# yuhuishi-convect/mojo-bm25

Hardware: AMD Instinct MI355X
Metric: queries/sec + achieved HBM GB/s, 10M-doc CSC index, batch=1024, k=100 (higher is better)
Workload: dtype f32; 1 GPU; c3: 10M docs / 200k vocab, batch=1024, k=100, 8 terms per query; segments=dense, n_docs=10000000, n_terms=200000, nnz=639994696, batch=1024, terms_per_query=8, k=100, tile_docs=2048, parallelism=doc-shard x1, term_lanes=8

## Files before the change

### mojo-bm25_amd/bm25mi/index.py

```python
from __future__ import annotations

import ctypes
from typing import Optional, Tuple

import numpy as np

from . import _capi
from ._capi import check, lib


def _ptr(a: Optional[np.ndarray]):
    return None if a is None else a.ctypes.data_as(ctypes.c_void_p)


def pack_mask(allow) -> np.ndarray:
    a = np.asarray(allow)
    if a.ndim == 1:
        a = a[None, :]
    if a.ndim != 2:
        raise ValueError("allow must be a bool [n_docs] or [M, n_docs] array")
    a = a.astype(bool)
    M, n = a.shape
    W = (n + 31) // 32
    bits = np.zeros((M, W * 32), np.uint8)
# ... 812 lines not shown
        if (d_values.dim() not in (1, 2) or d_values.shape[-1] != self.n_docs
                or not d_values.is_contiguous()):
            raise ValueError(f"d_values must be a contiguous [{self.n_docs}] or "
                             f"[F, {self.n_docs}] tensor (one entry per document)")
        F = 1 if d_values.dim() == 1 else d_values.shape[0]
        if (d_out.dim() != 2 or d_out.shape[1] != W or d_out.element_size() != 4
                or not d_out.is_contiguous()):
            raise ValueError(f"d_out must be a contiguous packed [M, {W}] tensor of 32-bit words")
        M = d_out.shape[0]
        if (d_fields.dim() != 2 or d_fields.shape[0] != M or d_fields.dtype != torch.int32
                or not d_fields.is_contiguous()):
            raise ValueError(f"d_fields must be a contiguous int32 [{M}, C] tensor (one row per "
                             "mask)")
        C = d_fields.shape[1]
        for name, t in (("d_lo", d_lo), ("d_hi", d_hi)):
            if (t.dtype != d_values.dtype or tuple(t.shape) != (M, C) or not t.is_contiguous()):
                raise ValueError(f"{name} must be a contiguous {d_values.dtype} [{M}, {C}] tensor "
                                 "(the values' dtype, the shape of d_fields)")
        Mb = 0
        if d_base is not None:
            if (d_base.dim() != 2 or d_base.shape[1] != W or d_base.element_size() != 4
                    or not d_base.is_contiguous()):
                raise ValueError(f"d_base must be a contiguous packed [1 or M, {W}] tensor of "
                                 "32-bit words")
            Mb = d_base.shape[0]
            if Mb not in (1, M):
                raise ValueError(f"d_base has {Mb} rows, expected 1 or {M}")
        s = getattr(stream, "cuda_stream", stream) or 0
        p = lambda t, n: ctypes.c_void_p(t.data_ptr()) if n else None
        check(lib.bm25_range_masks_device(
            self._h, p(d_values, F and self.n_docs), kinds[d_values.dtype], F, p(d_fields, M * C),
            p(d_lo, M * C), p(d_hi, M * C), C, M, p(d_base, Mb and W), Mb, p(d_out, M and W),
            ctypes.c_void_p(s)))

    def search_boolean(self, queries: np.ndarray, k: int, must=None, any=None, must_not=None,
                       base=None, *, min_match=None, total_hits: bool = False, facets=None,
                       ranges=None):
        q = np.ascontiguousarray(queries, dtype=np.int32)
        if q.ndim != 2:
            raise ValueError("queries must be a 2-D [Q, T] int32 array")
        Q, T = q.shape
        mu, an, mn, _, b, Mb = self._clauses_arg(must, any, must_not, base, rows=Q)
        mm = None if min_match is None else min_match_rows(an, min_match, "query")
        if facets is not None:
            if not isinstance(facets, (tuple, list)) or len(facets) != 2:
                raise ValueError("facets must be a pair (groups, n_groups)")
            fg, G = _facet_groups(facets[0], facets[1], self.n_docs)
        if ranges is not None:
            rv, kind, rf, rlo, rhi = _range_args(*_ranges_arg(ranges), self.n_docs, rows=Q,
                                                 what="query")
        k = int(k)
        docs = np.zeros((Q, max(k, 0)), np.int32)
        scores = np.zeros((Q, max(k, 0)), np.float32)
        if ranges is not None:
            totals = np.zeros(Q, np.int64) if total_hits else None
            counts = np.zeros((Q, G), np.int64) if facets is not None else None
            give = bool(counts is not None and G and fg.size)
            ranged = bool(rv.size and rf.size)
            check(lib.bm25_search_boolean_ranges(
                self._h, _ptr(q), Q, T, k, _ptr(mu), mu.shape[1], _ptr(an), an.shape[1], _ptr(mn),
                mn.shape[1], _ptr(mm), _ptr(b) if Mb else None, Mb, _ptr(fg) if give else None,
                G if give else 0, _ptr(rv) if ranged else None, kind, rv.shape[0] if ranged else 0,
                _ptr(rf) if ranged else None, _ptr(rlo) if ranged else None,
                _ptr(rhi) if ranged else None, rf.shape[1] if ranged else 0, _ptr(docs),
                _ptr(scores), _ptr(totals), _ptr(counts) if give else None))
            out = (docs, scores)
            if total_hits:
                out += (totals,)
            if facets is not None:
                out += (counts,)
            return out
        if facets is not None:
            totals = np.zeros(Q, np.int64) if total_hits else None
            counts = np.zeros((Q, G), np.int64)
            give = bool(G and fg.size)
            check(lib.bm25_search_boolean_facets(
                self._h, _ptr(q), Q, T, k, _ptr(mu), mu.shape[1], _ptr(an), an.shape[1], _ptr(mn),
                mn.shape[1], _ptr(mm), _ptr(b) if Mb else None, Mb, _ptr(fg) if give else None,
                G if give else 0, _ptr(docs), _ptr(scores), _ptr(totals),
                _ptr(counts) if give else None))
            return (docs, scores, totals, counts) if total_hits else (docs, scores, counts)
        if mm is None and not total_hits:
            check(lib.bm25_search_boolean(self._h, _ptr(q), Q, T, k, _ptr(mu), mu.shape[1],
                                          _ptr(an), an.shape[1], _ptr(mn), mn.shape[1],
                                          _ptr(b) if Mb else None, Mb, _ptr(docs), _ptr(scores)))
            return docs, scores
        totals = np.zeros(Q, np.int64) if total_hits else None
        check(lib.bm25_search_boolean_min_match(
            self._h, _ptr(q), Q, T, k, _ptr(mu), mu.shape[1], _ptr(an), an.shape[1], _ptr(mn),
            mn.shape[1], _ptr(mm), _ptr(b) if Mb else None, Mb, _ptr(docs), _ptr(scores),
            _ptr(totals)))
        return (docs, scores, totals) if total_hits else (docs, scores)

    def set_values_f64(self, data64) -> None:
        d = np.ascontiguousarray(data64, dtype=np.float64)
        if d.size < self.nnz:
            raise ValueError("data64 shorter than nnz")
        check(lib.bm25_index_set_values_f64(self._h, _ptr(d)))

    def scores_dense_f64(self, query) -> np.ndarray:
        q = np.ascontiguousarray(np.asarray(query).ravel(), dtype=np.int32)
        out = np.zeros(self.n_docs, np.float64)
        check(lib.bm25_scores_dense_f64(self._h, _ptr(q), q.size, _ptr(out)))
        return out

    def topn_f64(self, query, n: int) -> Tuple[np.ndarray, np.ndarray]:
        q = np.ascontiguousarray(np.asarray(query).ravel(), dtype=np.int32)
        docs = np.zeros(max(int(n), 0), np.int32)
        scores = np.zeros(max(int(n), 0), np.float64)
        check(lib.bm25_topn_f64(self._h, _ptr(q), q.size, int(n), _ptr(docs), _ptr(scores)))
        return docs, scores

    def profile_enable(self, on: bool = True) -> None:
        check(lib.bm25_profile_enable(self._h, int(on)))

    def profile_read(self) -> dict:
        sm = ctypes.c_double()
        sl = ctypes.c_int64()
        tm = ctypes.c_double()
        ns = ctypes.c_int64()
        rs = ctypes.c_int64()
        check(lib.bm25_profile_read(self._h, ctypes.byref(sm), ctypes.byref(sl), ctypes.byref(tm),
                                    ctypes.byref(ns), ctypes.byref(rs)))
        return {"score_ms": sm.value, "score_launches": sl.value, "total_ms": tm.value,
                "searches": ns.value, "rescored_tiles_last": rs.value}

    def set_option(self, name: str, value: int) -> None:
        check(lib.bm25_index_set_option(self._h, name.encode(), int(value)))
        self.__dict__.pop("_bm25_width_ok", None)
        for f in self.__dict__.get("_bm25_forks", []):
            f.set_option(name, value)

    def get_option(self, name: str) -> int:
        v = ctypes.c_int64()
        check(lib.bm25_index_get_option(self._h, name.encode(), ctypes.byref(v)))
        return v.value

    KERNELS = {1: "flat_sample", 2: "flat_rest", 4: "flat_all", 8: "wave_sample",
               16: "wave_rest", 32: "wave_all", 64: "large_k", 128: "bound_keys",
               256: "bound_off", 512: "count_skips", 1024: "rest_split",
               2048: "bound_pool", 4096: "filtered", 8192: "weighted",
               16384: "after"}

    def last_dispatch(self) -> dict:
        km = ctypes.c_uint32()
        tl = ctypes.c_int32()
        bt = (ctypes.c_int32 * 3)()
        sp_ = ctypes.c_int32()
        check(lib.bm25_search_dispatch(self._h, ctypes.byref(km), ctypes.byref(tl), bt,
                                       ctypes.byref(sp_)))
        return {"kernels": {n for b, n in self.KERNELS.items() if km.value & b},
                "tile_skip": bool(km.value & 32768),
                "seg_skip": bool(km.value & 65536),
                "term_lanes": tl.value,
                "band_tiles": {"all": bt[0], "sample": bt[1], "rest": bt[2]},
                "sample_p": sp_.value}

    def search_stats(self) -> dict:
        v = (ctypes.c_int64 * 8)()
        check(lib.bm25_search_counters(self._h, v, 8))
        return {"rescored_tiles": v[0], "fallback_queries": v[1],
                "bound_skipped_tiles": v[2], "bound_skipped_postings": v[3],
                "block_merge_queries": v[4], "large_dense_queries": v[5],
                "bound_dropped_segments": v[6], "bound_dropped_postings": v[7]}


def merge_topk_device(device: int, d_docs, d_scores, W: int, Q: int, k: int, d_out_docs,
                      d_out_scores, stream=None) -> None:
    s = getattr(stream, "cuda_stream", stream) or 0
    check(lib.bm25_merge_topk_device(int(device), ctypes.c_void_p(d_docs.data_ptr()),
                                     ctypes.c_void_p(d_scores.data_ptr()), int(W), int(Q), int(k),
                                     ctypes.c_void_p(d_out_docs.data_ptr()),
                                     ctypes.c_void_p(d_out_scores.data_ptr()),
                                     ctypes.c_void_p(s)))


def merge_sorted_device(device: int, d_docs, d_scores, W: int, Q: int, k: int, rank_stride: int,
                        d_out_docs, d_out_scores, stream=None) -> None:
    s = getattr(stream, "cuda_stream", stream) or 0
    check(lib.bm25_merge_sorted_device(int(device), ctypes.c_void_p(d_docs.data_ptr()),
                                       ctypes.c_void_p(d_scores.data_ptr()), int(W), int(Q),
                                       int(k), int(rank_stride),
                                       ctypes.c_void_p(d_out_docs.data_ptr()),
                                       ctypes.c_void_p(d_out_scores.data_ptr()),
                                       ctypes.c_void_p(s)))


class ShardedIndex:

    def __init__(self, indptr, indices, data, n_docs: int, devices):
        devices = [int(d) for d in devices]
        if not devices:
            raise ValueError("need at least one device")
        indptr = np.asarray(indptr)
        ip_i64 = indptr.dtype == np.int64 or indptr[-1] > np.iinfo(np.int32).max
        ip = np.ascontiguousarray(indptr, dtype=np.int64 if ip_i64 else np.int32)
        ix = np.ascontiguousarray(indices, dtype=np.int32)
        dt = np.ascontiguousarray(data, dtype=np.float32)
        devs = np.asarray(devices, np.int32)
        self.n_docs = int(n_docs)
        self.n_terms = int(ip.size - 1)
        self._h = None
        h = ctypes.c_void_p()
        check(lib.bm25_sharded_create(len(devices), _ptr(devs), self.n_docs, self.n_terms,
                                      int(ip[-1]), _ptr(ip), int(ip_i64), _ptr(ix), _ptr(dt),
                                      ctypes.byref(h)))
        self._h = h

    def shards(self):
        n = ctypes.c_int64()
        check(lib.bm25_sharded_info(self._h, ctypes.byref(n), None, None))
        lo = np.zeros(n.value, np.int64)
        hi = np.zeros(n.value, np.int64)
        check(lib.bm25_sharded_info(self._h, ctypes.byref(n), _ptr(lo), _ptr(hi)))
        return list(zip(lo.tolist(), hi.tolist()))

    def search(self, queries: np.ndarray, k: int) -> Tuple[np.ndarray, np.ndarray]:
        q = np.ascontiguousarray(queries, dtype=np.int32)
        if q.ndim != 2:
            raise ValueError("queries must be a 2-D [Q, T] int32 array")
        Q, T = q.shape
        k = int(k)
        docs = np.zeros((Q, max(k, 0)), np.int32)
        scores = np.zeros((Q, max(k, 0)), np.float32)
        check(lib.bm25_sharded_search(self._h, _ptr(q), Q, T, k, _ptr(docs), _ptr(scores)))
        return docs, scores

    def close(self) -> None:
        if self._h is not None:
            lib.bm25_sharded_destroy(self._h)
            self._h = None

    def __del__(self):
        try:
            self.close()
        except Exception:
            pass


def device_count() -> int:
    return _capi.device_count()
```

### mojo-bm25_amd/csrc/bm25mi_capi.cpp

```cpp
#include "../../include/bm25mi.h"

#include <hip/hip_runtime.h>

#include <algorithm>
#include <cmath>
#include <cstdarg>
#include <cstdio>
#include <cstring>
#include <memory>
#include <mutex>
#include <string>
#include <vector>

#include "bm25mi_host.h"
#include "bm25mi_internal.h"

using namespace bm25mi;

namespace {
thread_local std::string g_err;
}

int bm25mi::fail(int code, const char* fmt, ...) {
  char buf[1024];
// ... 33 lines not shown
  std::vector<void*> p;
  ~IndexArrays() {
    hipSetDevice(device);
    for (void* x : p) hipFree(x);
  }
};

}

struct bm25_index {
  DevIndex ix;
  std::shared_ptr<IndexArrays> arrays;
  hipStream_t stream = nullptr;
  Workspace ws;
  int32_t* d_q = nullptr;
  int32_t* d_docs = nullptr;
  float* d_scores = nullptr;
  int64_t cap_q_elems = 0, cap_out_elems = 0;
  std::mutex mu;
  int prof = 0;
  std::vector<EventPair> ev_pool;
  size_t ev_used = 0;
  double score_ms = 0.0, total_ms = 0.0;
  int64_t score_launches = 0, searches = 0, rescored = 0;
  int64_t device_bytes = 0;
  EventPair* split_ev = nullptr;
  hipEvent_t ws_done = nullptr;
  hipEvent_t ev_split[2] = {nullptr, nullptr};
  hipStream_t ws_stream = nullptr;
  int32_t* d_maxtok = nullptr;
  bool sampled = false;
  int32_t* report_host = nullptr;
  int32_t* report_dev = nullptr;
  int32_t seq = 0, last_bound_seq = -1, seen_seq = -1, weak_until = 0, backoff = 64;
  int64_t last_bound_q = 0;
  int64_t large_fallback = 0;
  LargeArena arena;
  int64_t filtered_dense = 0;
};

static const OptDesc* find_opt(const char* name) {
  for (const OptDesc& d : kOpts)
    if (!strcmp(d.name, name)) return &d;
  for (const OptDesc& d : kOptsMore)
    if (!strcmp(d.name, name)) return &d;
  fail(BM25_EINVAL, "unknown option '%s'", name);
  return nullptr;
}

int bm25mi::set_opt(SearchOpts& o, const char* name, int64_t v) {
  if (!name) return fail(BM25_EINVAL, "NULL option name");
  const OptDesc* d = find_opt(name);
  if (!d) return BM25_EINVAL;
  if (v < d->lo || v > d->hi || (d->kind == kOptPow2 && (v & (v - 1)) != 0)) {
    if (d->msg) return fail(BM25_EINVAL, "%s", d->msg);
    if (d->kind == kOptBool) return fail(BM25_EINVAL, "%s must be 0 or 1", name);
    return fail(BM25_EINVAL, d->kind == kOptPow2 ? "%s must be a power of two in %d..%d"
                                                  : "%s must be in %d..%d", name, d->lo, d->hi);
  }
  o.*d->field = (int)v;
  return BM25_OK;
}

int bm25mi::get_opt(const SearchOpts& o, const char* name, int64_t* v) {
  if (!name || !v) return fail(BM25_EINVAL, "NULL argument");
  const OptDesc* d = find_opt(name);
  if (!d) return BM25_EINVAL;
  *v = o.*d->field;
  return BM25_OK;
}

namespace {

void free_ws(Workspace& ws) {
  hipFree(ws.cand);
  hipFree(ws.theta);
  hipFree(ws.list);
  hipFree(ws.list_cnt);
  hipFree(ws.fb);
  hipFree(ws.cand2);
  hipFree(ws.flag_tiles);
  hipFree(ws.nflag);
  hipFree(ws.queue);
  hipFree(ws.counters);
  hipFree(ws.slow);
  hipFree(ws.wctr);
  hipFree(ws.seg);
  hipFree(ws.qw);
  hipFree(ws.sub);
  hipFree(ws.sub_ipb);
  hipFree(ws.sub_done);
  hipFree(ws.tskip);
  ws = Workspace{};
}

int32_t list_cap_for(const SearchOpts& o, int64_t k) {
  if (o.list_cap > 0) return o.list_cap;
  return (int32_t)std::min<int64_t>(65536, std::max<int64_t>(2048, 64 * k));
}

SearchOpts env_opts() {
  SearchOpts o;
  auto read = [&o](const OptDesc& d) {
    int v = env_int(d.env, o.*d.field);
    if (d.kind == kOptBool) v = v != 0;
    if (d.env_clamp >= 1) v = std::max(d.lo, v);
    if (d.env_clamp >= 2) v = std::min(d.hi, v);
    o.*d.field = v;
  };
  for (const OptDesc& d : kOpts) read(d);
  for (const OptDesc& d : kOptsMore) read(d);
  return o;
}

int ensure_ws(bm25_index* h, int64_t Q, int64_t T, int k, hipStream_t st) {
  Workspace& ws = h->ws;
  const int64_t need_seg = seg_entries(h->ix, std::max(Q, ws.cap_q), T);
  if (Q <= ws.cap_q && k <= ws.cap_k) {
    if (need_seg <= ws.cap_seg) return BM25_OK;
    hipFree(ws.seg);
    ws.seg = nullptr;
    ws.cap_seg = 0;
    HIP_TRY(hipMalloc(&ws.seg, sizeof(uint64_t) * need_seg), "hipMalloc(seg)");
    ws.cap_seg = need_seg;
    return BM25_OK;
  }
  const int64_t q = std::max(Q, ws.cap_q);
  const int64_t kk = std::max<int64_t>(k, ws.cap_k);
  free_ws(ws);
  const int64_t nt = h->ix.ntiles;
  const int64_t mf = maxflag_for((int)kk, nt);
  const int32_t C = list_cap_for(h->ix.opt, kk);
  HIP_TRY(hipMalloc(&ws.cand, sizeof(uint64_t) * q * nt * kTileM), "hipMalloc(cand)");
  HIP_TRY(hipMalloc(&ws.theta, sizeof(uint64_t) * q), "hipMalloc(theta)");
  HIP_TRY(hipMalloc(&ws.list, sizeof(uint64_t) * q * C), "hipMalloc(list)");
  HIP_TRY(hipMalloc(&ws.list_cnt, sizeof(int32_t) * q), "hipMalloc(list_cnt)");
  HIP_TRY(hipMalloc(&ws.fb, sizeof(int32_t) * q), "hipMalloc(fb)");
  HIP_TRY(hipMalloc(&ws.cand2, sizeof(uint64_t) * q * mf * kk), "hipMalloc(cand2)");
  HIP_TRY(hipMalloc(&ws.flag_tiles, sizeof(int32_t) * q * mf), "hipMalloc(flag_tiles)");
  HIP_TRY(hipMalloc(&ws.nflag, sizeof(int32_t) * q), "hipMalloc(nflag)");
  HIP_TRY(hipMalloc(&ws.queue, sizeof(int32_t) * q * mf), "hipMalloc(queue)");
  HIP_TRY(hipMalloc(&ws.counters, sizeof(int32_t) * kCounters), "hipMalloc(counters)");
  HIP_TRY(hipMemsetAsync(ws.counters, 0, sizeof(int32_t) * kCounters, st), "hipMemsetAsync(counters)");
  HIP_TRY(hipMalloc(&ws.slow, sizeof(int32_t) * q), "hipMalloc(slow)");
  HIP_TRY(hipMalloc(&ws.wctr, sizeof(int32_t) * kWctrRegions * kWctrInts), "hipMalloc(wctr)");
  HIP_TRY(hipMemsetAsync(ws.wctr, 0, sizeof(int32_t) * kWctrRegions * kWctrInts, st),
          "hipMemsetAsync(wctr)");
  HIP_TRY(hipMalloc(&ws.qw, sizeof(uint32_t) * q), "hipMalloc(qw)");
  HIP_TRY(hipMalloc(&ws.sub, sizeof(uint32_t) * q * 8), "hipMalloc(sub)");
  HIP_TRY(hipMalloc(&ws.sub_ipb, sizeof(int32_t)), "hipMalloc(sub_ipb)");
  HIP_TRY(hipMalloc(&ws.sub_done, sizeof(int32_t)), "hipMalloc(sub_done)");
  HIP_TRY(hipMemsetAsync(ws.sub_done, 0, sizeof(int32_t), st), "hipMemsetAsync(sub_done)");
  if (h->ix.bmax)
    HIP_TRY(hipMalloc(&ws.tskip, (size_t)std::max<int64_t>(q * tskip_stride(nt), 4)), "hipMalloc(tskip)");
  ws.cap_seg = need_seg;
  if (ws.cap_seg > 0) HIP_TRY(hipMalloc(&ws.seg, sizeof(uint64_t) * ws.cap_seg), "hipMalloc(seg)");
  ws.list_cap = C;
  ws.cap_q = q;
  ws.cap_k = kk;
  return BM25_OK;
}

int ensure_io(bm25_index* h, int64_t q_elems, int64_t out_elems) {
  if (q_elems > h->cap_q_elems) {
    hipFree(h->d_q);
    h->d_q = nullptr;
    h->cap_q_elems = 0;
    HIP_TRY(hipMalloc(&h->d_q, sizeof(int32_t) * std::max<int64_t>(q_elems, 1)), "hipMalloc(queries)");
    h->cap_q_elems = q_elems;
  }
  if (out_elems > h->cap_out_elems) {
    hipFree(h->d_docs);
    hipFree(h->d_scores);
    h->d_docs = nullptr;
    h->d_scores = nullptr;
    h->cap_out_elems = 0;
    HIP_TRY(hipMalloc(&h->d_docs, sizeof(int32_t) * std::max<int64_t>(out_elems, 1)), "hipMalloc(docs)");
    HIP_TRY(hipMalloc(&h->d_scores, sizeof(float) * std::max<int64_t>(out_elems, 1)), "hipMalloc(scores)");
    h->cap_out_elems = out_elems;
  }
  return BM25_OK;
}

void harvest_events(bm25_index* h) {
  if (h->ev_used == 0) return;
  for (size_t i = 0; i < h->ev_used; ++i) {
    float ms1 = 0.f, ms2 = 0.f;
    const bool tot = h->ev_pool[i].with_c;
    hipEventSynchronize(tot ? h->ev_pool[i].c : h->ev_pool[i].b);
    hipEventElapsedTime(&ms1, h->ev_pool[i].a, h->ev_pool[i].b);
    if (tot) hipEventElapsedTime(&ms2, h->ev_pool[i].a, h->ev_pool[i].c);
    h->score_ms += ms1;
    h->total_ms += tot ? ms2 : ms1;
  }
  h->ev_used = 0;
}

EventPair* next_events(bm25_index* h) {
  if (!h->prof) return nullptr;
  if (h->ev_used == h->ev_pool.size()) {
    if (h->ev_pool.size() < 512) {
      EventPair p;
      hipEventCreate(&p.a);
      hipEventCreate(&p.b);
      hipEventCreate(&p.c);
      h->ev_pool.push_back(p);
    } else {
      harvest_events(h);
    }
  }
  EventPair* e = &h->ev_pool[h->ev_used++];
  e->with_c = h->prof >= 2;
  return e;
}

hipError_t record_end(bm25_index* h, EventPair* ev, hipStream_t st) {
  return (ev && ev->with_c) ? hipEventRecord(ev->c, st) : hipSuccess;
}

hipError_t order_ws(bm25_index* h, hipStream_t st) {
  if (h->ws_stream == nullptr || st == h->ws_stream) {
    h->ws_stream = st;
    return hipSuccess;
  }
  if (!h->ws_done) {
    const hipError_t e = hipEventCreateWithFlags(&h->ws_done, hipEventDisableTiming);
    if (e != hipSuccess) return e;
  }
  hipError_t e = hipEventRecord(h->ws_done, h->ws_stream);
  if (e == hipSuccess) e = hipStreamWaitEvent(st, h->ws_done, 0);
  h->ws_stream = st;
  return e;
}

void ws_wait_host(bm25_index* h) {
  if (h->ws_stream) hipStreamSynchronize(h->ws_stream);
}

void choose_theta_source(bm25_index* h) {
  ++h->seq;
  if (h->report_host && h->last_bound_seq >= 0 && h->seen_seq != h->last_bound_seq) {
    const int32_t r = __atomic_load_n(h->report_host + 1, __ATOMIC_ACQUIRE);
    if (r == h->last_bound_seq) {
      h->seen_seq = r;
      const int64_t nf = __atomic_load_n(h->report_host, __ATOMIC_RELAXED);
      if (nf * 16 > h->last_bound_q) {
        h->weak_until = h->seq + h->backoff;
        h->backoff = std::min(2 * h->backoff, 4096);
      } else {
        h->backoff = 64;
      }
    }
  }
  h->ix.bound_weak = h->seq < h->weak_until;
}

void arm_report(bm25_index* h, int P, int64_t Q) {
  h->ws.report = h->report_dev;
  h->ws.seq = h->seq;
  if (h->ix.bound_weak) h->ix.disp.kernels |= kKBoundOff;
  if (P == 0) {
    h->last_bound_seq = h->seq;
    h->last_bound_q = Q;
  }
}

void alloc_report(bm25_index* h) {
  if (hipHostMalloc((void**)&h->report_host, 2 * sizeof(int32_t), hipHostMallocMapped) !=
      hipSuccess) {
    (void)hipGetLastError();
    h->report_host = nullptr;
    return;
  }
  h->report_host[0] = 0;
  h->report_host[1] = -1;
  if (hipHostGetDevicePointer((void**)&h->report_dev, h->report_host, 0) != hipSuccess) {
    (void)hipGetLastError();
    hipHostFree(h->report_host);
    h->report_host = h->report_dev = nullptr;
  }
}

int run_search(bm25_index* h, const int32_t* d_queries, int64_t Q, int64_t T, int k,
               int32_t* d_docs, float* d_scores, hipStream_t st, bool shard = false) {
  if (Q == 0 || k == 0) return BM25_OK;
  if (k > kMaxK) {
    const bool lists = h->ix.opt.large_lists && k <= kLargeListMaxK && k <= h->ix.n_docs &&
                       large_list_supported(h->ix, T, Q) && large_geom(h->ix, k).P > 0;
    if (lists) {
      const int rc = ensure_ws(h, Q, T, 1, st);
      if (rc) return rc;
    }
    if (h->arena.need > h->arena.bytes) {
      if (h->ws_stream) HIP_TRY(hipStreamSynchronize(h->ws_stream), "hipStreamSynchronize");
      hipFree(h->arena.base);
      h->arena.base = nullptr;
      h->arena.bytes = 0;
      HIP_TRY(hipMalloc((void**)&h->arena.base, h->arena.need), "hipMalloc(large-k scratch)");
      h->arena.bytes = h->arena.need;
    }
    h->arena.used = 0;
    h->ws.arena = &h->arena;
    HIP_TRY(order_ws(h, st), "workspace order");
    if (h->ws.counters)
      HIP_TRY(hipMemsetAsync(h->ws.counters, 0, sizeof(int32_t) * kCounters, st), "hipMemsetAsync");
    h->ix.disp = Dispatch{};
    h->ix.disp.sample_p = 1;
// ... 55 lines not shown
    hipFree(h->arena.base);
    h->arena.base = nullptr;
    h->arena.bytes = 0;
    HIP_TRY(hipMalloc((void**)&h->arena.base, h->arena.need), "hipMalloc(filtered scratch)");
    h->arena.bytes = h->arena.need;
  }
  h->arena.used = 0;
  h->ws.arena = &h->arena;
  HIP_TRY(order_ws(h, st), "workspace order");
  h->large_fallback = 0;
  h->ix.disp = Dispatch{};
  h->ix.disp.sample_p = 1;
  h->ws.report = nullptr;
  EventPair* ev = next_events(h);
  if (ev) HIP_TRY(hipEventRecord(ev->a, st), "hipEventRecord");
  int64_t nd = 0;
  if (after) h->ix.disp.kernels |= kKAfter;
  HIP_TRY(launch_search_filtered(h->ix, d_queries, Q, T, k, d_masks, M, d_query_mask, h->ws,
                                 d_docs, d_scores, &nd, st, d_weights, d_after_scores,
                                 d_after_docs),
          after ? "cursor search" : d_weights ? "weighted search" : "filtered search");
  h->filtered_dense = nd;
  if (ev) {
    HIP_TRY(hipEventRecord(ev->b, st), "hipEventRecord");
    HIP_TRY(record_end(h, ev, st), "hipEventRecord");
  }
  if (h->prof) {
    h->score_launches += 1;
    h->searches += 1;
  }
  return BM25_OK;
}

void read_counters(bm25_index* h, int32_t (&cnt)[kCounters]) {
  if (!h->ws.counters) return;
  ws_wait_host(h);
  hipMemcpyAsync(cnt, h->ws.counters, sizeof cnt, hipMemcpyDeviceToHost, h->stream);
  hipStreamSynchronize(h->stream);
}

int check_k(const bm25_index* h, int64_t k, bool shard = false) {
  if (k < 0) return fail(BM25_EINVAL, "negative dimensions are not allowed (top_k=%lld)", (long long)k);
  if (!shard && k > h->ix.n_docs)
    return fail(BM25_EINVAL, "kth(=%lld) out of bounds (%lld)", (long long)(h->ix.n_docs - k),
                (long long)h->ix.n_docs);
  return BM25_OK;
}

int64_t max_token(int64_t mx, const int32_t* ids, int64_t n) {
  for (int64_t i = 0; i < n; ++i) mx = std::max<int64_t>(mx, ids[i]);
  return mx;
}

int check_token_ids(int64_t n_terms, int64_t mx0, const int32_t* ids, int64_t n) {
  const int64_t mx = max_token(mx0, ids, n);
  if (mx >= n_terms)
    return fail(BM25_EINVAL,
                "The maximum token ID in the query (%lld) is higher than the number of tokens in "
                "the index.",
                (long long)mx);
  return BM25_OK;
}

int check_weights(const int32_t* ids, const float* w, int64_t Q, int64_t T) {
  for (int64_t i = 0; i < Q * T; ++i)
    if (ids[i] >= 0 && !std::isfinite(w[i]))
      return fail(BM25_EINVAL, "weights[%lld][%lld] = %g is not finite", (long long)(i / T),
                  (long long)(i % T), (double)w[i]);
  return BM25_OK;
}

struct Enter {
  std::lock_guard<std::mutex> lk;
  int rc;
  explicit Enter(bm25_index* h) : lk(h->mu), rc(BM25_OK) {
    const hipError_t e = hipSetDevice(h->ix.device);
    if (e != hipSuccess) rc = hip_fail(e, "hipSetDevice");
  }
};

struct OwnStream {
  hipStream_t s = nullptr;
  ~OwnStream() {
    if (s) hipStreamDestroy(s);
  }
};

}

extern "C" {

int bm25_abi_version(void) { return BM25MI_ABI_VERSION; }

const char* bm25_last_error(void) { return g_err.c_str(); }

int bm25_device_count(void) {
  int n = 0;
  if (hipGetDeviceCount(&n) != hipSuccess) return 0;
  return n;
}

static int build_index(bm25_index* h, const std::vector<int64_t>& ip, const int32_t* indices,
                       const float* data);

int bm25_index_create(int device, int64_t n_docs, int64_t n_terms, int64_t nnz,
                      const void* indptr, int indptr_is_i64, const int32_t* indices,
                      const float* data, int64_t doc_offset, bm25_index** out) {
  if (!out) return fail(BM25_EINVAL, "out is NULL");
  *out = nullptr;
  if (n_docs < 0 || n_terms < 0 || nnz < 0)
    return fail(BM25_EINVAL, "negative size (n_docs=%lld n_terms=%lld nnz=%lld)",
                (long long)n_docs, (long long)n_terms, (long long)nnz);
  if (n_docs > INT32_MAX) return fail(BM25_EINVAL, "n_docs=%lld exceeds int32 doc ids", (long long)n_docs);
  if (doc_offset < 0 || doc_offset + n_docs > (int64_t)INT32_MAX + 1)
    return fail(BM25_EINVAL, "doc_offset=%lld out of int32 range", (long long)doc_offset);
  if (!indptr || (nnz > 0 && (!indices || !data)))
    return fail(BM25_EINVAL, "NULL CSC array");
  std::vector<int64_t> ip(n_terms + 1);
  for (int64_t t = 0; t <= n_terms; ++t)
    ip[t] = indptr_is_i64 ? ((const int64_t*)indptr)[t] : (int64_t)((const int32_t*)indptr)[t];
  if (ip[0] != 0 || ip[n_terms] != nnz)
    return fail(BM25_EINVAL, "indptr must start at 0 and end at nnz (got %lld..%lld, nnz=%lld)",
                (long long)ip[0], (long long)ip[n_terms], (long long)nnz);
  for (int64_t t = 0; t < n_terms; ++t) {
    if (ip[t + 1] < ip[t]) return fail(BM25_EINVAL, "indptr decreases at column %lld", (long long)t);
    if (ip[t + 1] - ip[t] > n_docs)
      return fail(BM25_EINVAL, "column %lld has more entries than n_docs", (long long)t);
  }
  const int shift = build_tile_shift();
  const int64_t ntiles = (n_docs + (1LL << shift) - 1) >> shift;
  if (ntiles > 65536) return fail(BM25_EINVAL, "n_docs=%lld needs %lld tiles (> 65536)", (long long)n_docs, (long long)ntiles);

  int ndev = 0;
  if (hipGetDeviceCount(&ndev) != hipSuccess || ndev == 0)
    return fail(BM25_EHIP, "no HIP device available");
  if (device < 0 || device >= ndev) return fail(BM25_EINVAL, "device %d out of range (%d visible)", device, ndev);
  HIP_TRY(hipSetDevice(device), "hipSetDevice");

  bm25_index* h = new bm25_index();
  DevIndex& ix = h->ix;
  ix.opt = env_opts();
  ix.device = device;
  ix.n_docs = n_docs;
  ix.n_terms = n_terms;
  ix.nnz = nnz;
  ix.doc_offset = doc_offset;
  ix.tile_shift = shift;
  ix.ntiles = ntiles;
  const int rc = build_index(h, ip, indices, data);
  if (rc == BM25_OK) {
    h->arrays = std::make_shared<IndexArrays>();
    h->arrays->device = device;
    h->arrays->p = {ix.indptr, ix.rel, ix.tl_ptr, ix.tl_tile, ix.tl_start, ix.ldoc, ix.val, ix.bmax,
                    ix.bpool, ix.tmask};
    *out = h;
  } else {
    bm25_index_destroy(h);
  }
  return rc;
}

static int build_index(bm25_index* h, const std::vector<int64_t>& ip, const int32_t* indices,
                       const float* data) {
  DevIndex& ix = h->ix;
  const int64_t n_terms = ix.n_terms, nnz = ix.nnz, ntiles = ix.ntiles;
  HIP_TRY(hipStreamCreateWithFlags(&h->stream, hipStreamNonBlocking), "hipStreamCreate");
  std::vector<int64_t> cnt;
  HostCall c(h->stream);
  auto own = [&c](auto** p, int64_t bytes, const char* what) {
    if (c.ok()) c.run(hipMalloc(p, (size_t)bytes), what);
  };
  alloc_report(h);
  const int64_t rel_elems = n_terms * (ntiles + 1);
  {
    const char* m = getenv("BM25_SEGMENTS");
    size_t free_b = 0, total_b = 0;
    if (hipMemGetInfo(&free_b, &total_b) != hipSuccess) total_b = 0;
    const int64_t rel_bytes = rel_elems * 4;
    if (m && !strcmp(m, "sparse")) ix.sparse = true;
    else if (m && !strcmp(m, "dense")) ix.sparse = false;
    else ix.sparse = rel_bytes > 2 * 6 * std::max<int64_t>(nnz, 1) &&
                     rel_bytes > (int64_t)(total_b / 8);
  }
  own(&ix.indptr, sizeof(int64_t) * (n_terms + 1), "hipMalloc(indptr)");
  if (!ix.sparse) own(&ix.rel, sizeof(uint32_t) * std::max<int64_t>(rel_elems, 1), "hipMalloc(rel)");
  own(&ix.ldoc, sizeof(uint16_t) * (nnz + kPostingPad), "hipMalloc(ldoc)");
  own(&ix.val, sizeof(float) * (nnz + kPostingPad), "hipMalloc(val)");
  if (c.ok()) c.run(hipMemsetAsync(ix.ldoc + nnz, 0, sizeof(uint16_t) * kPostingPad, h->stream), "hipMemset");
  if (c.ok()) c.run(hipMemsetAsync(ix.val + nnz, 0, sizeof(float) * kPostingPad, h->stream), "hipMemset");
  int32_t* d_indices = c.alloc<int32_t>(nnz, "hipMalloc(indices)");
  int32_t* d_err = c.alloc<int32_t>(1, "hipMalloc(err)");
  h->device_bytes = (int64_t)(sizeof(int64_t) * (n_terms + 1) +
                              (ix.sparse ? 0 : sizeof(uint32_t) * rel_elems) +
                              (sizeof(uint16_t) + sizeof(float)) * nnz);
  if (c.ok()) c.run(hipMemsetAsync(d_err, 0, sizeof(int32_t), h->stream), "hipMemset");
  c.upload_to(ix.indptr, ip.data(), n_terms + 1, "H2D indptr");
  c.upload_to(d_indices, indices, nnz, "H2D indices");
  c.upload_to(ix.val, data, nnz, "H2D data");
  if (!ix.sparse) {
    if (c.ok()) c.run(launch_build_tables(ix, d_indices, d_err, h->stream), "build_tables launch");
  } else {
    int64_t* d_cnt = c.alloc<int64_t>(n_terms, "hipMalloc(cnt)");
    cnt.assign(n_terms + 1, 0);
    if (c.ok()) c.run(launch_count_tiles(ix, d_indices, d_cnt, d_err, h->stream), "count_tiles");
    c.download(cnt.data() + 1, d_cnt, n_terms, "count_tiles");
    if (c.ok()) c.run(hipStreamSynchronize(h->stream), "count_tiles");
    for (int64_t t = 0; t < n_terms; ++t) cnt[t + 1] += cnt[t];
    ix.n_pairs = cnt[n_terms];
    own(&ix.tl_ptr, sizeof(int64_t) * (n_terms + 1), "hipMalloc(tl_ptr)");
    own(&ix.tl_tile, sizeof(uint16_t) * std::max<int64_t>(ix.n_pairs, 1), "hipMalloc(tl_tile)");
    own(&ix.tl_start, sizeof(uint32_t) * std::max<int64_t>(ix.n_pairs, 1), "hipMalloc(tl_start)");
    c.upload_to(ix.tl_ptr, cnt.data(), n_terms + 1, "H2D tl_ptr");
    if (c.ok()) c.run(launch_fill_tiles(ix, d_indices, h->stream), "fill_tiles launch");
    if (c.ok()) c.run(hipStreamSynchronize(h->stream), "fill_tiles");
    h->device_bytes += (int64_t)(sizeof(int64_t) * (n_terms + 1) +
                                 (sizeof(uint16_t) + sizeof(uint32_t)) * ix.n_pairs);
  }
  ix.nonneg = true;
  for (int64_t p = 0; p < nnz && ix.nonneg; ++p)
    ix.nonneg = data[p] == 0.0f || data[p] >= 1.17549435e-38f;
  if (c.ok() && !ix.sparse && ix.nonneg && n_terms > 0 && ntiles > 0) {
    if (hipMalloc(&ix.bmax, sizeof(uint16_t) * n_terms * bmax_stride(ntiles)) == hipSuccess) {
      c.run(launch_build_bmax(ix, h->stream), "build_bmax launch");
      h->device_bytes += (int64_t)(sizeof(uint16_t) * n_terms * bmax_stride(ntiles));
      const int64_t ps = bmax_stride((ntiles + kPool - 1) / kPool);
      if (c.ok() && hipMalloc(&ix.bpool, sizeof(uint16_t) * n_terms * ps) == hipSuccess) {
        ix.pstride = ps;
        c.run(launch_pool_bounds(ix.bmax, n_terms, bmax_stride(ntiles), ix.bpool, ps, h->stream),
              "pool_bounds launch");
        h->device_bytes += (int64_t)(sizeof(uint16_t) * n_terms * ps);
      } else {
        (void)hipGetLastError();
        ix.bpool = nullptr;
      }
      if (c.ok() && ix.opt.tile_mask &&
          hipMalloc(&ix.tmask, sizeof(uint32_t) * n_terms * bmax_stride(ntiles)) == hipSuccess) {
        c.run(launch_build_tmask(ix, h->stream), "build_tmask launch");
        h->device_bytes += (int64_t)(sizeof(uint32_t) * n_terms * bmax_stride(ntiles));
      } else {
        (void)hipGetLastError();
        ix.tmask = nullptr;
      }
    } else {
      (void)hipGetLastError();
      ix.bmax = nullptr;
    }
  }
  int32_t herr = 0;
  c.download(&herr, d_err, 1, "D2H err");
  const int rc = c.finish("build sync");
  if (rc) return rc;
  if (herr)
    return fail(BM25_EINVAL,
                "indices must be sorted, unique and in [0, n_docs) within every column "
                "(canonical CSC)");
  return BM25_OK;
}

int bm25_index_destroy(bm25_index* h) {
  if (!h) return BM25_OK;
  hipSetDevice(h->ix.device);
  if (h->stream) hipStreamSynchronize(h->stream);
  if (h->ws_stream) hipDeviceSynchronize();
  for (auto& p : h->ev_pool) {
    hipEventDestroy(p.a);
    hipEventDestroy(p.b);
    hipEventDestroy(p.c);
  }
  if (h->ws_done) hipEventDestroy(h->ws_done);
  for (hipEvent_t e : h->ev_split)
    if (e) hipEventDestroy(e);
  free_ws(h->ws);
  hipFree(h->arena.base);
  hipFree(h->d_q);
  hipFree(h->d_docs);
  hipFree(h->d_scores);
  hipFree(h->d_maxtok);
  if (h->report_host) hipHostFree(h->report_host);
  if (h->arrays) {
    h->arrays.reset();
  } else {
    for (void* x : {(void*)h->ix.indptr, (void*)h->ix.rel, (void*)h->ix.tl_ptr,
                    (void*)h->ix.tl_tile, (void*)h->ix.tl_start, (void*)h->ix.ldoc,
                    (void*)h->ix.val, (void*)h->ix.bmax, (void*)h->ix.bpool,
                    (void*)h->ix.tmask})
      hipFree(x);
  }
  hipFree(h->ix.wbpool);
  if (h->stream) hipStreamDestroy(h->stream);
  delete h;
  return BM25_OK;
}

static int pool_world(bm25_index* h);

int bm25_index_fork(bm25_index* base, bm25_index** out) {
  if (!out) return fail(BM25_EINVAL, "out is NULL");
  *out = nullptr;
  if (!base || !base->arrays) return fail(BM25_EINVAL, "NULL or unbuilt index");
  std::lock_guard<std::mutex> lk(base->mu);
  HIP_TRY(hipSetDevice(base->ix.device), "hipSetDevice");
  bm25_index* h = new bm25_index();
  h->ix = base->ix;
  h->ix.disp = Dispatch{};
  h->ix.wbpool = nullptr;
  h->arrays = base->arrays;
  h->device_bytes = base->device_bytes;
  const hipError_t e = hipStreamCreateWithFlags(&h->stream, hipStreamNonBlocking);
  if (e != hipSuccess) {
    bm25_index_destroy(h);
    return hip_fail(e, "hipStreamCreate");
  }
  alloc_report(h);
  if (h->ix.wbmax) {
    const int rc = pool_world(h);
    if (rc) {
      bm25_index_destroy(h);
      return rc;
    }
  }
  *out = h;
  return BM25_OK;
}

int bm25_index_info(const bm25_index* h, int64_t* n_docs, int64_t* n_terms, int64_t* nnz,
                    int32_t* tile_docs, int64_t* n_tiles, int64_t* device_bytes) {
  if (!h) return fail(BM25_EINVAL, "NULL index");
  if (n_docs) *n_docs = h->ix.n_docs;
  if (n_terms) *n_terms = h->ix.n_terms;
  if (nnz) *nnz = h->ix.nnz;
  if (tile_docs) *tile_docs = 1 << h->ix.tile_shift;
  if (n_tiles) *n_tiles = h->ix.ntiles;
  if (device_bytes) *device_bytes = h->device_bytes;
  return BM25_OK;
}

int bm25_index_segments(const bm25_index* h, int32_t* sparse, int64_t* n_pairs) {
  if (!h) return fail(BM25_EINVAL, "NULL index");
  if (sparse) *sparse = h->ix.sparse ? 1 : 0;
  if (n_pairs) *n_pairs = h->ix.n_pairs;
  return BM25_OK;
}

int bm25_index_bounds(const bm25_index* h, int32_t* has_bounds, int64_t* bytes) {
  if (!h) return fail(BM25_EINVAL, "NULL index");
  const bool on = h->ix.bmax != nullptr;
  if (has_bounds) *has_bounds = on ? 1 : 0;
  if (bytes) *bytes = on ? (int64_t)sizeof(uint16_t) * h->ix.n_terms * bmax_stride(h->ix.ntiles) : 0;
  return BM25_OK;
}

int bm25_search(bm25_index* h, const int32_t* queries, int64_t Q, int64_t T, int32_t k,
                int32_t* out_docs, float* out_scores) {
  if (!h) return fail(BM25_EINVAL, "NULL index");
  if (Q < 0 || T < 0) return fail(BM25_EINVAL, "negative query shape");
  int rc = check_k(h, k);
  if (rc) return rc;
  if (Q == 0 || k == 0) return BM25_OK;
  if (T > 0 && !queries) return fail(BM25_EINVAL, "NULL queries");
  if (!out_docs || !out_scores) return fail(BM25_EINVAL, "NULL output");
  rc = check_token_ids(h->ix.n_terms, 0, queries, Q * T);
  if (rc) return rc;
  Enter in(h);
  if (in.rc) return in.rc;
  rc = ensure_io(h, Q * T, Q * (int64_t)k);
  if (rc) return rc;
  HostCall c(h->stream);
  c.upload_to(h->d_q, queries, Q * T, "H2D queries");
  if (c.ok()) c.hold(run_search(h, h->d_q, Q, T, k, h->d_docs, h->d_scores, h->stream));
  c.download(out_docs, h->d_docs, Q * k, "D2H docs");
  c.download(out_scores, h->d_scores, Q * k, "D2H scores");
  return c.finish("search sync");
}

int bm25_search_device(bm25_index* h, const int32_t* d_queries, int64_t Q, int64_t T, int32_t k,
                       int32_t* d_docs, float* d_scores, void* stream) {
  if (!h) return fail(BM25_EINVAL, "NULL index");
  if (Q < 0 || T < 0) return fail(BM25_EINVAL, "negative query shape");
  int rc = check_k(h, k);
  if (rc) return rc;
  if (Q == 0 || k == 0) return BM25_OK;
  Enter in(h);
  if (in.rc) return in.rc;
  return run_search(h, d_queries, Q, T, k, d_docs, d_scores, (hipStream_t)stream);
}

int bm25_search_filtered(bm25_index* h, const int32_t* queries, int64_t Q, int64_t T, int32_t k,
                         const uint32_t* masks, int64_t M, const int32_t* query_mask,
                         int32_t* out_docs, float* out_scores) {
  if (!h) return fail(BM25_EINVAL, "NULL index");
  if (Q < 0 || T < 0 || M < 0) return fail(BM25_EINVAL, "negative query or mask shape");
  int rc = check_k(h, k);
  if (rc) return rc;
  if (Q == 0 || k == 0) return BM25_OK;
  if (T > 0 && !queries) return fail(BM25_EINVAL, "NULL queries");
  if (M > 0 && !masks) return fail(BM25_EINVAL, "NULL masks");
  if (M == 0 && !query_mask)
    return fail(BM25_EINVAL, "no masks: query_mask must name -1 (no filter) for every query");
  if (!out_docs || !out_scores) return fail(BM25_EINVAL, "NULL output");
  rc = check_token_ids(h->ix.n_terms, 0, queries, Q * T);
  if (rc) return rc;
  if (query_mask)
    for (int64_t i = 0; i < Q; ++i)
      if (query_mask[i] < -1 || query_mask[i] >= M)
        return fail(BM25_EINVAL, "query_mask[%lld] = %d is outside [-1, %lld)", (long long)i,
                    query_mask[i], (long long)M);
  Enter in(h);
  if (in.rc) return in.rc;
  rc = ensure_io(h, Q * T, Q * (int64_t)k);
  if (rc) return rc;
  const int64_t W = (h->ix.n_docs + 31) >> 5;
  HostCall c(h->stream);
  uint32_t* d_masks = M > 0 ? c.alloc<uint32_t>(M * W) : nullptr;
  int32_t* d_qm = query_mask ? c.alloc<int32_t>(Q) : nullptr;
  c.upload_to(d_masks, masks, M * W);
  if (query_mask) c.upload_to(d_qm, query_mask, Q);
  c.upload_to(h->d_q, queries, Q * T);
  if (!c.ok()) return c.finish("filtered search staging");
  c.hold(run_filtered(h, h->d_q, Q, T, k, d_masks, M, d_qm, h->d_docs, h->d_scores, h->stream));
  c.download(out_docs, h->d_docs, Q * k);
  c.download(out_scores, h->d_scores, Q * k);
  return c.finish("filtered search");
}

int bm25_search_filtered_device(bm25_index* h, const int32_t* d_queries, int64_t Q, int64_t T,
                                int32_t k, const uint32_t* d_masks, int64_t M,
                                const int32_t* d_query_mask, int32_t* d_docs, float* d_scores,
                                void* stream) {
  if (!h) return fail(BM25_EINVAL, "NULL index");
  if (Q < 0 || T < 0 || M < 0) return fail(BM25_EINVAL, "negative query or mask shape");
  int rc = check_k(h, k);
  if (rc) return rc;
  if (Q == 0 || k == 0) return BM25_OK;
  Enter in(h);
  if (in.rc) return in.rc;
  return run_filtered(h, d_queries, Q, T, k, d_masks, M, d_query_mask, d_docs, d_scores,
                      (hipStream_t)stream);
}
// ... 951 lines not shown
  c.upload_to(d_qq, queries, Q * T);
  c.upload_to(d_ww, weights, Q * T);
  c.upload_to(d_dd, docs, Q * C);
  if (c.ok()) c.run(launch_score_docs(h->ix, d_qq, Q, T, d_dd, C, d_out, h->stream, d_ww));
  c.download(out_scores, d_out, Q * C);
  return c.finish("score_docs_weighted");
}

int bm25_score_docs_weighted_device(bm25_index* h, const int32_t* d_queries,
                                    const float* d_weights, int64_t Q, int64_t T,
                                    const int32_t* d_docs, int64_t C, float* d_scores,
                                    void* stream) {
  if (!h) return fail(BM25_EINVAL, "NULL index");
  if (Q < 0 || T < 0 || C < 0) return fail(BM25_EINVAL, "negative query or candidate shape");
  if (Q == 0 || C == 0) return BM25_OK;
  if (T > 0 && (!d_queries || !d_weights)) return fail(BM25_EINVAL, "NULL queries or weights");
  if (!d_docs || !d_scores) return fail(BM25_EINVAL, "NULL docs or output");
  Enter in(h);
  if (in.rc) return in.rc;
  HIP_TRY(launch_score_docs(h->ix, d_queries, Q, T, d_docs, C, d_scores, (hipStream_t)stream,
                            T > 0 ? d_weights : nullptr),
          "score_docs_weighted launch");
  return BM25_OK;
}

int bm25_index_set_values_f64(bm25_index* h, const double* data64) {
  if (!h || (h->ix.nnz > 0 && !data64)) return fail(BM25_EINVAL, "NULL argument");
  if (!h->arrays) return fail(BM25_EINVAL, "unbuilt index");
  Enter in(h);
  if (in.rc) return in.rc;
  if (!h->ix.val64) {
    HIP_TRY(hipMalloc(&h->ix.val64, sizeof(double) * std::max<int64_t>(h->ix.nnz, 1)),
            "hipMalloc(val64)");
    h->arrays->p.push_back(h->ix.val64);
  }
  HostCall c(h->stream);
  c.upload_to(h->ix.val64, data64, h->ix.nnz, "H2D val64");
  return c.finish("val64 sync");
}

static double* dense_f64_query(bm25_index* h, HostCall& c, const int32_t* query, int64_t T) {
  if (T < 0) c.hold(fail(BM25_EINVAL, "negative query length"));
  else if (T > 0 && !query) c.hold(fail(BM25_EINVAL, "NULL query"));
  else if (!h->ix.val64)
    c.hold(fail(BM25_EINVAL, "no float64 values: bm25_index_set_values_f64 first"));
  else c.hold(check_token_ids(h->ix.n_terms, 0, query, T));
  int32_t* d_q = c.alloc<int32_t>(T, "hipMalloc(query)");
  double* d_out = c.alloc<double>(h->ix.n_docs, "hipMalloc(dense)");
  c.upload_to(d_q, query, T, "H2D query");
  if (c.ok())
    c.run(launch_dense_f64(h->ix, h->ix.val64, d_q, T, d_out, h->stream), "dense f64 launch");
  return d_out;
}

int bm25_scores_dense_f64(bm25_index* h, const int32_t* query, int64_t T, double* out_scores) {
  if (!h || !out_scores) return fail(BM25_EINVAL, "NULL argument");
  Enter in(h);
  if (in.rc) return in.rc;
  HostCall c(h->stream);
  const double* d_out = dense_f64_query(h, c, query, T);
  c.download(out_scores, d_out, h->ix.n_docs);
  return c.finish("scores_dense_f64");
}

int bm25_topn_f64(bm25_index* h, const int32_t* query, int64_t T, int64_t n, int32_t* out_docs,
                  double* out_scores) {
  if (!h) return fail(BM25_EINVAL, "NULL index");
  if (n < 0 || n > h->ix.n_docs)
    return fail(BM25_EINVAL, "n=%lld must be in 0..n_docs (%lld)", (long long)n,
                (long long)h->ix.n_docs);
  if (n > 0 && (!out_docs || !out_scores)) return fail(BM25_EINVAL, "NULL output");
  if (n == 0) return BM25_OK;
  Enter in(h);
  if (in.rc) return in.rc;
  HostCall c(h->stream);
  const double* d_out = dense_f64_query(h, c, query, T);
  void* scratch = c.alloc<char>((int64_t)topn_f64_scratch_bytes(h->ix.n_docs));
  int32_t* d_docs = c.alloc<int32_t>(n);
  double* d_sc = c.alloc<double>(n);
  if (c.ok()) c.run(launch_topn_f64(d_out, h->ix.n_docs, n, scratch, d_docs, d_sc, h->stream));
  c.download(out_docs, d_docs, n);
  c.download(out_scores, d_sc, n);
  return c.finish("topn_f64");
}

int bm25_merge_topk_device(int device, const int32_t* d_docs, const float* d_scores, int64_t W,
                           int64_t Q, int32_t k, int32_t* d_out_docs, float* d_out_scores,
                           void* stream) {
  if (W < 1 || Q < 0 || k < 0) return fail(BM25_EINVAL, "bad merge shape W=%lld Q=%lld k=%d", (long long)W, (long long)Q, k);
  HIP_TRY(hipSetDevice(device), "hipSetDevice");
  HIP_TRY(launch_merge_lists(d_docs, d_scores, W, Q, k, Q * (int64_t)k, false, d_out_docs, d_out_scores, (hipStream_t)stream), "merge_lists launch");
  return BM25_OK;
}

int bm25_merge_sorted_device(int device, const int32_t* d_docs, const float* d_scores, int64_t W,
                             int64_t Q, int32_t k, int64_t rank_stride, int32_t* d_out_docs,
                             float* d_out_scores, void* stream) {
  if (W < 1 || Q < 0 || k < 0 || rank_stride < Q * (int64_t)k)
    return fail(BM25_EINVAL, "bad merge shape W=%lld Q=%lld k=%d stride=%lld", (long long)W,
                (long long)Q, k, (long long)rank_stride);
  HIP_TRY(hipSetDevice(device), "hipSetDevice");
  HIP_TRY(launch_merge_lists(d_docs, d_scores, W, Q, k, rank_stride, true, d_out_docs,
                             d_out_scores, (hipStream_t)stream),
          "merge_sorted launch");
  return BM25_OK;
}

int bm25_profile_enable(bm25_index* h, int on) {
  if (!h) return fail(BM25_EINVAL, "NULL index");
  std::lock_guard<std::mutex> lk(h->mu);
  hipSetDevice(h->ix.device);
  harvest_events(h);
  h->prof = on < 0 ? 0 : (on > 2 ? 2 : on);
  h->score_ms = h->total_ms = 0.0;
  h->score_launches = h->searches = h->rescored = 0;
  return BM25_OK;
}

int bm25_profile_read(bm25_index* h, double* score_ms_total, int64_t* score_launches,
                      double* total_ms, int64_t* searches, int64_t* rescored_tiles) {
  if (!h) return fail(BM25_EINVAL, "NULL index");
  std::lock_guard<std::mutex> lk(h->mu);
  hipSetDevice(h->ix.device);
  harvest_events(h);
  int32_t cnt[kCounters] = {};
  read_counters(h, cnt);
  if (score_ms_total) *score_ms_total = h->score_ms;
  if (score_launches) *score_launches = h->score_launches;
  if (total_ms) *total_ms = h->total_ms;
  if (searches) *searches = h->searches;
  if (rescored_tiles) *rescored_tiles = cnt[3];
  return BM25_OK;
}

int bm25_search_stats(bm25_index* h, int64_t* rescored_tiles, int64_t* fallback_queries) {
  return bm25_search_stats_ex(h, rescored_tiles, fallback_queries, nullptr);
}

int bm25_search_stats_ex(bm25_index* h, int64_t* rescored_tiles, int64_t* fallback_queries,
                         int64_t* bound_skipped) {
  if (!h) return fail(BM25_EINVAL, "NULL index");
  Enter in(h);
  if (in.rc) return in.rc;
  int32_t cnt[kCounters] = {};
  read_counters(h, cnt);
  if (rescored_tiles) *rescored_tiles = cnt[3];
  if (fallback_queries) *fallback_queries = cnt[2];
  if (bound_skipped) *bound_skipped = (h->ix.disp.kernels & kKCountSkips) ? cnt[5] : -1;
  return BM25_OK;
}

int bm25_search_counters(bm25_index* h, int64_t* out, int32_t n) {
  if (!h || !out) return fail(BM25_EINVAL, "NULL argument");
  if (n < 1 || n > 8) return fail(BM25_EINVAL, "n=%d must be in 1..8", n);
  Enter in(h);
  if (in.rc) return in.rc;
  int32_t cnt[kCounters] = {};
  read_counters(h, cnt);
  uint64_t post = 0;
  std::memcpy(&post, cnt + 6, sizeof post);
  const bool counted = (h->ix.disp.kernels & kKCountSkips) != 0;
  uint64_t dpost = 0;
  std::memcpy(&dpost, cnt + 10, sizeof dpost);
  const int64_t v[8] = {cnt[3], cnt[2], counted ? cnt[5] : -1, counted ? (int64_t)post : -1,
                        cnt[4], h->large_fallback, counted ? cnt[8] : -1,
                        counted ? (int64_t)dpost : -1};
  for (int i = 0; i < n; ++i) out[i] = v[i];
  return BM25_OK;
}

int bm25_index_set_option(bm25_index* h, const char* name, int64_t value) {
  if (!h) return fail(BM25_EINVAL, "NULL index");
  std::lock_guard<std::mutex> lk(h->mu);
  const int old_cap = h->ix.opt.list_cap;
  const int rc = set_opt(h->ix.opt, name, value);
  if (rc) return rc;
  if (h->ix.opt.list_cap != old_cap && h->ws.cap_q > 0) {
    hipSetDevice(h->ix.device);
    ws_wait_host(h);
    free_ws(h->ws);
  }
  return BM25_OK;
}

int bm25_index_get_option(const bm25_index* h, const char* name, int64_t* value) {
  if (!h) return fail(BM25_EINVAL, "NULL index");
  bm25_index* m = const_cast<bm25_index*>(h);
  std::lock_guard<std::mutex> lk(m->mu);
  return get_opt(h->ix.opt, name, value);
}

int bm25_search_dispatch(bm25_index* h, uint32_t* kernels, int32_t* term_lanes,
                         int32_t* band_tiles, int32_t* sample_p) {
  if (!h) return fail(BM25_EINVAL, "NULL index");
  std::lock_guard<std::mutex> lk(h->mu);
  const Dispatch& d = h->ix.disp;
  if (kernels) *kernels = d.kernels;
  if (term_lanes) *term_lanes = d.term_lanes;
  if (band_tiles)
    for (int i = 0; i < 3; ++i) band_tiles[i] = d.band_tiles[i];
  if (sample_p) *sample_p = d.sample_p;
  return BM25_OK;
}

}

struct bm25_sharded {
  std::vector<bm25_index*> shards;
  std::vector<int64_t> lo, hi;
  std::vector<hipEvent_t> sampled;
  std::vector<hipEvent_t> keyed;
  std::vector<hipEvent_t> done;
  std::vector<uint64_t*> keys;
  std::vector<uint64_t*> all_keys;
  int64_t cap_keys = 0;
  int64_t n_docs = 0, n_terms = 0, shard_docs_max = 0;
  int32_t* g_docs = nullptr;
  float* g_scores = nullptr;
  int32_t* m_docs = nullptr;
  float* m_scores = nullptr;
  int64_t cap_g = 0, cap_m = 0;
  std::mutex mu;
};

namespace {

int sharded_free(bm25_sharded* s) {
  if (!s) return BM25_OK;
  if (!s->shards.empty() && s->shards[0]) {
    hipSetDevice(s->shards[0]->ix.device);
    hipFree(s->g_docs);
    hipFree(s->g_scores);
    hipFree(s->m_docs);
    hipFree(s->m_scores);
  }
  for (size_t i = 0; i < s->shards.size(); ++i) {
    if (!s->shards[i]) continue;
    hipSetDevice(s->shards[i]->ix.device);
    hipStreamSynchronize(s->shards[i]->stream);
    for (auto* v : {&s->sampled, &s->keyed, &s->done})
      if (i < v->size() && (*v)[i]) hipEventDestroy((*v)[i]);
    if (i < s->keys.size()) hipFree(s->keys[i]);
    if (i < s->all_keys.size()) hipFree(s->all_keys[i]);
    bm25_index_destroy(s->shards[i]);
  }
  delete s;
  return BM25_OK;
}

struct DrainShards {
  bm25_sharded* s;
  ~DrainShards() {
    for (size_t r = 0; s && r < s->shards.size(); ++r) {
      hipSetDevice(s->shards[r]->ix.device);
      hipStreamSynchronize(s->shards[r]->stream);
    }
  }
};

}

extern "C" {

int bm25_sharded_create(int n_dev, const int* devices, int64_t n_docs, int64_t n_terms,
                        int64_t nnz, const void* indptr, int indptr_is_i64,
                        const int32_t* indices, const float* data, bm25_sharded** out) {
  if (!out) return fail(BM25_EINVAL, "out is NULL");
  *out = nullptr;
  if (n_dev < 1 || !devices) return fail(BM25_EINVAL, "need at least one device");
  if (n_docs < 0 || n_terms < 0 || nnz < 0) return fail(BM25_EINVAL, "negative size");
  if (!indptr || (nnz > 0 && (!indices || !data))) return fail(BM25_EINVAL, "NULL CSC array");
  std::vector<int64_t> ip(n_terms + 1);
  for (int64_t t = 0; t <= n_terms; ++t)
    ip[t] = indptr_is_i64 ? ((const int64_t*)indptr)[t] : (int64_t)((const int32_t*)indptr)[t];
  if (ip[0] != 0 || ip[n_terms] != nnz)
    return fail(BM25_EINVAL, "indptr must start at 0 and end at nnz");
  for (int64_t t = 0; t < n_terms; ++t)
    if (ip[t + 1] < ip[t]) return fail(BM25_EINVAL, "indptr decreases at column %lld", (long long)t);
  bm25_sharded* s = new bm25_sharded();
  s->n_docs = n_docs;
  s->n_terms = n_terms;
  const int64_t align = 2048;
  auto bound = [&](int64_t r) -> int64_t {
    if (r >= n_dev) return n_docs;
    const int64_t x = n_docs * r / n_dev;
    return std::min(n_docs, (x + align / 2) / align * align);
  };
  std::vector<int64_t> sip(n_terms + 1);
  std::vector<int32_t> six;
  std::vector<float> sdt;
  for (int r = 0; r < n_dev; ++r) {
    const int64_t lo = bound(r), hi = bound(r + 1);
    sip[0] = 0;
    for (int64_t t = 0; t < n_terms; ++t) {
      const int32_t* b = indices + ip[t];
      const int32_t* e = indices + ip[t + 1];
      const int32_t* p0 = std::lower_bound(b, e, (int32_t)std::min<int64_t>(lo, INT32_MAX));
      const int32_t* p1 = std::lower_bound(p0, e, (int32_t)std::min<int64_t>(hi, INT32_MAX));
      sip[t + 1] = sip[t] + (p1 - p0);
    }
    six.resize(std::max<int64_t>(sip[n_terms], 1));
    sdt.resize(std::max<int64_t>(sip[n_terms], 1));
    for (int64_t t = 0; t < n_terms; ++t) {
      const int32_t* b = indices + ip[t];
      const int32_t* e = indices + ip[t + 1];
      const int32_t* p0 = std::lower_bound(b, e, (int32_t)std::min<int64_t>(lo, INT32_MAX));
      for (int64_t i = 0; i < sip[t + 1] - sip[t]; ++i) {
        six[sip[t] + i] = p0[i] - (int32_t)lo;
        sdt[sip[t] + i] = data[(p0 - indices) + i];
      }
    }
    bm25_index* h = nullptr;
    const int rc = bm25_index_create(devices[r], hi - lo, n_terms, sip[n_terms], sip.data(), 1,
                                     six.data(), sdt.data(), lo, &h);
    if (rc) {
      const std::string msg = g_err;
      sharded_free(s);
      return fail(rc, "shard %d (device %d): %s", r, devices[r], msg.c_str());
    }
// ... 155 lines not shown
```

### mojo-bm25_amd/csrc/bm25mi_host.h

```cpp
#pragma once
#include <hip/hip_runtime.h>

#include <algorithm>
#include <cstdint>
#include <vector>

#include "../../include/bm25mi.h"
#include "bm25mi_internal.h"

namespace bm25mi {

int fail(int code, const char* fmt, ...);
int hip_fail(hipError_t e, const char* what);

class HostCall {
 public:
  explicit HostCall(hipStream_t st) : st_(st) {}
  HostCall(const HostCall&) = delete;
  HostCall& operator=(const HostCall&) = delete;
  ~HostCall() {
    if (!finished_) hipStreamSynchronize(st_);
    for (void* p : bufs_) hipFree(p);
  }

  bool ok() const { return rc_ == BM25_OK && err_ == hipSuccess; }
  void run(hipError_t e, const char* what = nullptr) {
    if (ok() && e != hipSuccess) {
      err_ = e;
      what_ = what;
    }
  }
  void hold(int rc) {
    if (rc_ == BM25_OK) rc_ = rc;
  }
  template <class T>
  T* alloc(int64_t n, const char* what = nullptr) {
    void* p = nullptr;
    if (ok()) run(hipMalloc(&p, sizeof(T) * (size_t)std::max<int64_t>(n, 1)), what);
    if (p) bufs_.push_back(p);
    return (T*)p;
  }
  template <class T>
  void upload_to(T* dst, const T* src, int64_t n, const char* what = nullptr) {
    if (ok() && n > 0)
      run(hipMemcpyAsync(dst, src, sizeof(T) * (size_t)n, hipMemcpyHostToDevice, st_), what);
  }
  template <class T>
  T* upload(const T* src, int64_t n, const char* what = nullptr) {
    if (n <= 0) return nullptr;
    T* d = alloc<T>(n, what);
    upload_to(d, src, n, what);
    return d;
  }
  template <class T>
  void download(T* dst, const T* src, int64_t n, const char* what = nullptr) {
    if (ok() && n > 0)
      run(hipMemcpyAsync(dst, src, sizeof(T) * (size_t)n, hipMemcpyDeviceToHost, st_), what);
  }
  int finish(const char* what) {
    const hipError_t es = hipStreamSynchronize(st_);
    finished_ = true;
    if (rc_) return rc_;
    run(es);
    return err_ == hipSuccess ? BM25_OK : hip_fail(err_, what_ ? what_ : what);
  }

 private:
  hipStream_t st_;
  std::vector<void*> bufs_;
  hipError_t err_ = hipSuccess;
  const char* what_ = nullptr;
  int rc_ = BM25_OK;
  bool finished_ = false;
};

enum OptKind { kOptBool, kOptRange, kOptPow2 };
struct OptDesc {
  const char* name;
  const char* env;
  int SearchOpts::*field;
  OptKind kind;
  int lo, hi;
  int env_clamp;
  const char* msg;
};
inline constexpr OptDesc kOpts[] = {
    {"flat", "BM25_FLAT", &SearchOpts::flat, kOptBool, 0, 1, 0, nullptr},
    {"flat_bw", "BM25_FLAT_BW", &SearchOpts::flat_bw, kOptPow2, 0, 8, 0,
     "flat_bw must be 0, 1, 2, 4 or 8"},
    {"items_per_wave", "BM25_ITEMS_PER_WAVE", &SearchOpts::items_per_wave, kOptRange, 1, 1024, 0,
     nullptr},
    {"sample_p", "BM25_SAMPLE_P", &SearchOpts::sample_p, kOptPow2, 1, 64, 0, nullptr},
    {"list_cap", "BM25_LIST_CAP", &SearchOpts::list_cap, kOptRange, 0, 1 << 20, 0,
     "list_cap must be in 0..2^20"},
    {"claim_ch", "BM25_CLAIM_CH", &SearchOpts::claim_ch, kOptRange, 1, 64, 0, nullptr},
    {"claim_m", "BM25_CLAIM_M", &SearchOpts::claim_m, kOptRange, 1, kClaimM, 0, nullptr},
    {"tile_bound", "BM25_TILE_BOUND", &SearchOpts::tile_bound, kOptBool, 0, 1, 0, nullptr},
    {"theta_bound", "BM25_THETA_BOUND", &SearchOpts::theta_bound, kOptBool, 0, 1, 0, nullptr},
    {"grid_pct", "BM25_GRID_PCT", &SearchOpts::grid_pct, kOptRange, 1, 100, 2, nullptr},
    {"count_skips", "BM25_COUNT_SKIPS", &SearchOpts::count_skips, kOptBool, 0, 1, 0, nullptr},
    {"large_lists", "BM25_LARGE_LISTS", &SearchOpts::large_lists, kOptBool, 0, 1, 0, nullptr},
    {"rest_split", "BM25_REST_SPLIT", &SearchOpts::rest_split, kOptBool, 0, 1, 0, nullptr},
    {"bound_pool", "BM25_BOUND_POOL", &SearchOpts::bound_pool, kOptBool, 0, 1, 0, nullptr},
    {"filter_tiles", "BM25_FILTER_TILES", &SearchOpts::filter_tiles, kOptBool, 0, 1, 0, nullptr},
    {"bool_chunk", "BM25_BOOL_CHUNK", &SearchOpts::bool_chunk, kOptRange, 0, 1 << 30, 1,
     "bool_chunk must be in 0..2^30"},
};
inline constexpr OptDesc kOptsMore[] = {
    {"tile_mask", "BM25_TILE_MASK", &SearchOpts::tile_mask, kOptBool, 0, 1, 0, nullptr},
    {"seg_skip", "BM25_SEG_SKIP", &SearchOpts::seg_skip, kOptBool, 0, 1, 0, nullptr},
};

int set_opt(SearchOpts& o, const char* name, int64_t v);
int get_opt(const SearchOpts& o, const char* name, int64_t* v);

}
```

### mojo-bm25_amd/csrc/bm25mi_internal.h

```cpp
#pragma once
#include <stdint.h>
#include <hip/hip_runtime.h>

#include <algorithm>
#include <vector>

namespace bm25mi {

__host__ __device__ inline uint32_t score_key(float s) {
  uint32_t u;
  __builtin_memcpy(&u, &s, 4);
  return (u & 0x80000000u) ? ~u : (u | 0x80000000u);
}
__host__ __device__ inline float key_score(uint32_t k) {
  uint32_t u = (k & 0x80000000u) ? (k & 0x7FFFFFFFu) : ~k;
  float s;
  __builtin_memcpy(&s, &u, 4);
  return s;
}
__host__ __device__ inline uint64_t make_key(float s, uint32_t doc) {
  return ((uint64_t)score_key(s) << 32) | (uint64_t)(0xFFFFFFFFu - doc);
}

constexpr int kTileM = 4;
constexpr int kLargeM = 8;
constexpr int kSplitM = 3;
constexpr int kSplitItemsPerWave = 48;
constexpr int kMaxK = 4096;
constexpr int kMergeP = 8192;
constexpr int64_t kPostingPad = 64;
constexpr int kDefaultTileShift = 11;

constexpr int kClaimM = 8;
constexpr int kCtrStride = 64;
constexpr int kSampleGroup = 8;
constexpr int kWctrInts = 8 * kClaimM * kCtrStride;
constexpr int kDoneOff = 32;
constexpr int kWctrRegions = 3;

struct SearchOpts {
  int flat = 1;
  int flat_bw = 0;
  int items_per_wave = 4;
  int sample_p = 8;
  int list_cap = 0;
  int claim_ch = 1;
  int claim_m = 4;
  int tile_bound = 1;
  int theta_bound = 1;
  int count_skips = 0;
  int grid_pct = 100;
  int large_lists = 1;
  int rest_split = 0;
  int bound_pool = 1;
  int filter_tiles = 1;
  int bool_chunk = 0;
  int tile_mask = 1;
  int seg_skip = 1;
};

enum {
  kKFlatSample = 1, kKFlatRest = 2, kKFlatAll = 4,
  kKWaveSample = 8, kKWaveRest = 16, kKWaveAll = 32,
  kKLarge = 64,
  kKBound = 128,
  kKBoundOff = 256,
  kKCountSkips = 512,
  kKRestSplit = 1024,
  kKBoundPool = 2048,
  kKFiltered = 4096,
  kKWeighted = 8192,
  kKAfter = 16384,
  kKTileSkip = 32768,
  kKSegSkip = 65536,
};
struct Dispatch {
  uint32_t kernels = 0;
  int32_t term_lanes = 0;
  int32_t band_tiles[3] = {0, 0, 0};
  int32_t sample_p = 0;
};

__host__ __device__ inline int64_t bmax_stride(int64_t ntiles) { return (ntiles + 3) & ~(int64_t)3; }

__host__ __device__ inline int64_t tskip_stride(int64_t ntiles) { return (ntiles + 3) & ~(int64_t)3; }

struct DevIndex {
  int device = 0;
  int64_t n_docs = 0, n_terms = 0, nnz = 0, doc_offset = 0;
  int tile_shift = kDefaultTileShift;
  bool nonneg = false;
  int64_t ntiles = 0;
  int64_t* indptr = nullptr;
  bool sparse = false;
  uint32_t* rel = nullptr;
  int64_t* tl_ptr = nullptr;
  uint16_t* tl_tile = nullptr;
  uint32_t* tl_start = nullptr;
  int64_t n_pairs = 0;
  uint16_t* ldoc = nullptr;
  float* val = nullptr;
  double* val64 = nullptr;
  uint16_t* bmax = nullptr;
  uint32_t* tmask = nullptr;
  uint16_t* bpool = nullptr;
  int64_t pstride = 0;
  bool bound_weak = false;
  const uint16_t* wbmax = nullptr;
  int32_t wW = 0;
  int64_t wstride = 0;
  int64_t wtiles = 0;
  uint16_t* wbpool = nullptr;
  int64_t wpstride = 0;
  int64_t wgroups = 0;
  SearchOpts opt;
  mutable Dispatch disp;
};

constexpr int kCounters = 12;

struct LargeArena {
  char* base = nullptr;
  size_t bytes = 0;
  size_t used = 0;
  size_t need = 0;
  int64_t budget = 0;
};

struct Scratch {
  hipStream_t st;
  std::vector<void*> ptrs;
  LargeArena* ar;
  size_t start, total = 0;
  explicit Scratch(hipStream_t s, LargeArena* a = nullptr)
      : st(s), ar(a), start(a ? a->used : 0) {}
  template <class T>
  hipError_t get(T** p, int64_t n) {
    *p = nullptr;
    const size_t size = (sizeof(T) * (size_t)std::max<int64_t>(n, 1) + 255) & ~(size_t)255;
    total += size;
    if (ar && ar->base && ar->used + size <= ar->bytes) {
      *p = reinterpret_cast<T*>(ar->base + ar->used);
      ar->used += size;
      return hipSuccess;
    }
    const hipError_t e = hipMallocAsync((void**)p, size, st);
    if (e == hipSuccess) ptrs.push_back((void*)*p);
    return e;
  }
  ~Scratch() {
    if (ar) {
      ar->need = std::max(ar->need, start + total);
      ar->used = start;
    }
    for (void* p : ptrs) hipFreeAsync(p, st);
  }
};

struct Workspace {
  int64_t cap_q = 0, cap_k = 0;
  LargeArena* arena = nullptr;
  uint64_t* cand = nullptr;
  uint64_t* theta = nullptr;
  uint64_t* list = nullptr;
  int32_t* list_cnt = nullptr;
  int32_t list_cap = 0;
  int32_t* fb = nullptr;
  uint64_t* cand2 = nullptr;
  int32_t* flag_tiles = nullptr;
  int32_t* nflag = nullptr;
  int32_t* queue = nullptr;
  int32_t* counters = nullptr;
  int32_t* slow = nullptr;
  uint64_t* slots = nullptr;
  int32_t* slot_cnt = nullptr;
  int32_t slot_cap = 0;
  int32_t* wctr = nullptr;
  int32_t* report = nullptr;
  int32_t seq = 0;
  uint32_t* qw = nullptr;
  uint32_t* sub = nullptr;
  int32_t* sub_ipb = nullptr;
  int32_t* sub_done = nullptr;
  uint8_t* tskip = nullptr;
  uint64_t* seg = nullptr;
  int64_t cap_seg = 0;
};

inline int64_t maxflag_for(int k, int64_t ntiles) {
  const int64_t m = (k + kTileM - 1) / kTileM;
  return m < ntiles ? m : (ntiles > 0 ? ntiles : 1);
}

struct SampleGeom {
  int P, m;
  int64_t S;
  int G;
};
SampleGeom sample_geom(int64_t ntiles, int k, int W, int pmax);
SampleGeom search_geom(const DevIndex& ix, int64_t ntiles, int k, int W, int64_t T);
constexpr int64_t kBoundMaxTiles = 30720;
constexpr int64_t kBoundTilesPerK = 16;
constexpr int64_t kPool = 4;
constexpr int64_t kPoolGroupsPerK = 8;
#ifndef BM25_BOUND_TERMS
#define BM25_BOUND_TERMS 16
#endif
constexpr int64_t kBoundMaxTerms = BM25_BOUND_TERMS;

hipError_t launch_build_tables(const DevIndex& ix, const int32_t* d_indices,
                               int32_t* d_err, hipStream_t stream);
hipError_t launch_build_bmax(const DevIndex& ix, hipStream_t stream);
hipError_t launch_build_tmask(const DevIndex& ix, hipStream_t stream);
hipError_t launch_pool_bounds(const uint16_t* in, int64_t rows, int64_t in_stride, uint16_t* out,
                              int64_t out_stride, hipStream_t stream);
hipError_t launch_count_tiles(const DevIndex& ix, const int32_t* d_indices, int64_t* d_cnt,
                              int32_t* d_err, hipStream_t stream);
hipError_t launch_fill_tiles(const DevIndex& ix, const int32_t* d_indices, hipStream_t stream);
int64_t seg_entries(const DevIndex& ix, int64_t Q, int64_t T);
SampleGeom shard_geom_world(const DevIndex& ix, int k, int64_t T, bool world);
hipError_t launch_score(const DevIndex& ix, const int32_t* d_queries, int64_t Q, int64_t T,
                        int k, const Workspace& ws, hipStream_t stream, bool world = false);
hipError_t launch_sample(const DevIndex& ix, const int32_t* d_queries, int64_t Q, int64_t T,
                         const SampleGeom& g, uint64_t* keys, const Workspace& ws,
                         hipStream_t stream);
hipError_t launch_finish(const DevIndex& ix, const int32_t* d_queries, int64_t Q, int64_t T,
                         int k, const SampleGeom& g, int W, const uint64_t* all_keys,
                         const Workspace& ws, hipStream_t stream,
                         hipStream_t rest_stream = nullptr, hipEvent_t join = nullptr,
                         hipEvent_t rest_timing = nullptr);
hipError_t launch_select(const DevIndex& ix, const int32_t* d_queries,
                         int64_t Q, int64_t T, int k, int P, const Workspace& ws,
                         int32_t* d_docs, float* d_scores, hipStream_t stream, bool unsorted = false);
hipError_t launch_scores_dense(const DevIndex& ix, const int32_t* d_query,
                               int64_t T, float* d_out, hipStream_t stream);
hipError_t launch_score_docs(const DevIndex& ix, const int32_t* d_queries, int64_t Q, int64_t T,
                             const int32_t* d_docs, int64_t C, float* d_out, hipStream_t stream,
                             const float* d_weights = nullptr);
hipError_t launch_merge_lists(const int32_t* d_docs, const float* d_scores,
                              int64_t W, int64_t Q, int k, int64_t rank_stride, bool sorted,
                              int32_t* d_out_docs, float* d_out_scores, hipStream_t stream);

hipError_t launch_scores_batch(const DevIndex& ix, const int32_t* d_queries, int64_t G, int64_t T,
                               int64_t stride, float* d_out, hipStream_t stream,
                               const float* d_weights = nullptr);

hipError_t launch_search_large(const DevIndex& ix, const int32_t* d_queries, int64_t Q, int64_t T,
                               int k, int32_t* d_docs, float* d_scores, hipStream_t stream,
                               LargeArena* arena = nullptr, int64_t budget = 0);
hipError_t launch_sample_large(const DevIndex& ix, const int32_t* d_queries, int64_t Q, int64_t T,
                               const SampleGeom& g, uint64_t* keys, const Workspace& ws,
                               hipStream_t stream);
hipError_t launch_rest_lists(const DevIndex& ix, const int32_t* d_queries, int64_t Q, int64_t T,
                             const SampleGeom& g, const Workspace& ws, hipStream_t stream);
bool large_list_supported(const DevIndex& ix, int64_t T, int64_t Q);

constexpr int64_t kLargeListMaxK = 131072;
SampleGeom large_geom(const DevIndex& ix, int64_t k);
hipError_t launch_search_large_lists(const DevIndex& ix, const int32_t* d_queries, int64_t Q,
                                     int64_t T, int k, const Workspace& ws, int32_t* d_docs,
                                     float* d_scores, int64_t* n_fallback, hipStream_t stream);

hipError_t launch_merge_large(const int32_t* d_docs, const float* d_scores, int64_t W, int64_t Q,
                              int k, int64_t rank_stride, int32_t* d_out_docs,
                              float* d_out_scores, hipStream_t stream);

hipError_t launch_filter_census(const DevIndex& ix, const uint32_t* d_masks, int64_t M,
                                int32_t* d_census, uint32_t* d_total, hipStream_t stream);
hipError_t launch_filter_pass_a(const DevIndex& ix, const int32_t* d_queries, int64_t Q, int64_t T,
                                const uint32_t* d_masks, const int32_t* d_query_mask,
                                const int32_t* d_census, uint64_t* d_cand, int32_t* d_skipped,
                                hipStream_t stream, const float* d_weights = nullptr,
                                const uint64_t* d_ckey = nullptr);
hipError_t launch_filter_pass_b(const DevIndex& ix, const int32_t* d_queries, int64_t Q, int64_t T,
                                const uint32_t* d_masks, const int32_t* d_query_mask,
                                const uint64_t* d_cand, const uint64_t* d_theta, uint64_t* d_list,
                                int32_t* d_list_cnt, int32_t C, int32_t* d_rescored,
                                hipStream_t stream, const float* d_weights = nullptr,
                                const uint64_t* d_ckey = nullptr);
hipError_t launch_search_filtered_dense(const DevIndex& ix, const int32_t* d_queries, int64_t T,
                                        int k, const uint32_t* d_masks,
                                        const int32_t* d_query_mask, const uint32_t* d_total,
                                        const int32_t* d_ids, int64_t nq, int32_t* d_docs,
                                        float* d_scores, hipStream_t stream, LargeArena* arena,
                                        const float* d_weights = nullptr,
                                        const uint64_t* d_ckey = nullptr);
hipError_t launch_search_filtered(const DevIndex& ix, const int32_t* d_queries, int64_t Q,
                                  int64_t T, int k, const uint32_t* d_masks, int64_t M,
                                  const int32_t* d_query_mask, const Workspace& ws,
                                  int32_t* d_docs, float* d_scores, int64_t* n_dense,
                                  hipStream_t stream, const float* d_weights = nullptr,
                                  const float* d_after_scores = nullptr,
                                  const int32_t* d_after_docs = nullptr);

hipError_t launch_term_masks(const DevIndex& ix, const int32_t* d_must, int64_t A,
                             const int32_t* d_any, int64_t B, const int32_t* d_must_not, int64_t N,
                             int64_t M, const uint32_t* d_base, int64_t Mb, uint32_t* d_out,
                             hipStream_t stream, const int32_t* d_min_match = nullptr);

hipError_t launch_mask_count(const DevIndex& ix, const uint32_t* d_masks, int64_t M,
                             int64_t* d_counts, hipStream_t stream);

constexpr int64_t kFacetBins = 8192;
constexpr int64_t kFacetMaxRows = 64;
constexpr int64_t kFacetMinChunk = 8192;
constexpr int64_t kFacetMaxChunk = 65536;
constexpr int64_t kFacetChunkStep = 1024;
constexpr int64_t kFacetGlobalChunk = 16384;
int64_t facet_rows(int64_t G);
int64_t facet_chunk_docs(int64_t G, int64_t M);
hipError_t launch_mask_facets(const DevIndex& ix, const uint32_t* d_masks, int64_t M,
                              const int32_t* d_groups, int64_t G, int64_t* d_counts,
                              hipStream_t stream);

enum { kFieldI32 = 0, kFieldF32 = 1, kFieldI64 = 2 };
constexpr int64_t kRangeRows = 64;
constexpr int64_t kRangeSpanDocs = 256;
constexpr int64_t kRangeChunkDocs = 4096;
constexpr int64_t kRangeRegClauses = 8;
hipError_t launch_range_masks(const DevIndex& ix, const void* d_values, int kind, int64_t F,
                              const int32_t* d_fields, const void* d_lo, const void* d_hi,
                              int64_t C, int64_t M, const uint32_t* d_base, int64_t Mb,
                              uint32_t* d_out, hipStream_t stream);

hipError_t launch_max_token(const int32_t* d_queries, int64_t n, int32_t* d_out,
                            hipStream_t stream);

bool tile_shift_supported(int s);
int build_tile_shift();

size_t radix_sort_scratch_bytes(int64_t n);
hipError_t radix_sort_pairs(uint64_t* keys, uint32_t* vals, uint64_t* keys_alt, uint32_t* vals_alt,
                            int64_t n, int key_bits_lo, int key_bits_hi, bool descending,
                            int val_bits_hi, void* scratch, bool* result_in_alt, hipStream_t st);
hipError_t radix_sort_rows_desc(uint64_t* keys, uint64_t* keys_alt, uint32_t* rows,
                                uint32_t* rows_alt, int64_t G, int64_t n, void* scratch,
                                bool* result_in_alt, hipStream_t st);
size_t exclusive_scan_scratch_bytes(int64_t n);
hipError_t exclusive_scan_u64(const unsigned long long* in, int64_t* out, int64_t n, void* scratch,
                              hipStream_t st);

hipError_t launch_dense_f64(const DevIndex& ix, const double* val64, const int32_t* d_query,
                            int64_t T, double* d_out, hipStream_t st);
size_t topn_f64_scratch_bytes(int64_t n_docs);
hipError_t launch_topn_f64(const double* d_scores, int64_t n_docs, int64_t n, void* scratch,
                           int32_t* d_docs, double* d_out_scores, hipStream_t st);

enum { kLucene = 0, kBm25Py = 1 };
hipError_t build_scores(int64_t n_docs, int64_t n_terms, int64_t n, const int32_t* d_docs,
                        const int32_t* d_terms, const float* d_tfs, const int32_t* d_doc_len,
                        double avgdl, double k1, double b, int method, const float* d_idf,
                        int64_t* d_indptr, int32_t* d_indices, float* d_data, double* d_data64,
                        int32_t* d_err, hipStream_t stream);

}
```

### mojo-bm25_amd/csrc/bm25mi_kernels.hip

```cpp
#include "bm25mi_internal.h"

#include <map>
#include <mutex>
#include <cstdio>
#include <cstdlib>
#include <vector>

namespace bm25mi {

enum Phase { kAll = 0, kSample = 1, kRest = 2 };

constexpr int kJ = 8;
constexpr int kWaves = 4;
constexpr int kGroup = 64;

struct IndexArgs {
  const int64_t* indptr;
  const uint32_t* rel;
  const uint16_t* ldoc;
  const float* val;
  int64_t V, ntiles, n_docs, nnz;
  int64_t doc_offset;
  int32_t nonneg;
  int32_t sparse;
  const int64_t* tl_ptr;
  const uint16_t* tl_tile;
  const uint32_t* tl_start;
  const uint64_t* seg;
  int64_t seg_zero;
  const uint8_t* tskip;
  int64_t tskip_stride;
};

static IndexArgs args_of(const DevIndex& ix) {
  return IndexArgs{ix.indptr, ix.rel, ix.ldoc, ix.val, ix.n_terms, ix.ntiles, ix.n_docs,
                   ix.nnz, ix.doc_offset, ix.nonneg ? 1 : 0, ix.sparse ? 1 : 0, ix.tl_ptr,
                   ix.tl_tile, ix.tl_start, nullptr, 0, nullptr, 0};
}

__device__ __forceinline__ void segment(const IndexArgs& a, int64_t term, int64_t tile,
                                        uint32_t& r0, uint32_t& r1) {
  if (!a.sparse) {
    const uint32_t* r = a.rel + term * (a.ntiles + 1) + tile;
    r0 = r[0];
    r1 = r[1];
    return;
  }
  const int64_t b = a.tl_ptr[term], e = a.tl_ptr[term + 1];
  int64_t lo = b, hi = e;
  while (lo < hi) {
    const int64_t mid = (lo + hi) >> 1;
    if ((int64_t)a.tl_tile[mid] < tile) lo = mid + 1;
    else hi = mid;
  }
  const uint32_t df = (uint32_t)(a.indptr[term + 1] - a.indptr[term]);
  const uint32_t at = lo < e ? a.tl_start[lo] : df;
  r0 = r1 = at;
  if (lo < e && (int64_t)a.tl_tile[lo] == tile) r1 = lo + 1 < e ? a.tl_start[lo + 1] : df;
}

__host__ __device__ inline int64_t sample_tile(int64_t si, int64_t P, int64_t G) {
  return (si / G) * G * P + si % G;
}
__host__ __device__ inline int64_t sample_count(int64_t ntiles, int64_t P, int64_t G) {
  const int64_t r = ntiles % (G * P);
  return (ntiles / (G * P)) * G + (r < G ? r : G);
}

struct Stage {
  const uint64_t* cand;
  uint64_t* cand_out;
  int64_t cstride;
  int64_t nt;
  int32_t P;
  int32_t G;
  int32_t M;
  const uint64_t* theta;
  const uint64_t* list;
  const int32_t* list_cnt;
  int32_t C;
  const uint64_t* sample_keys;
  uint64_t* cand_mirror;
  int64_t sample_stride;
  const int32_t* qmap;
  const int32_t* nq_dev;
  int32_t nq_host;
  int32_t* fb;
  int32_t* fb_cnt;
  int32_t ctr_region;
  bool remap;
  bool unsorted;
  bool split;
};

__device__ __forceinline__ int lane_id() { return (int)(threadIdx.x & 63); }

__device__ __forceinline__ uint32_t lane_u32(uint32_t v, int l) {
  return (uint32_t)__builtin_amdgcn_readlane((int)v, l);
}
__device__ __forceinline__ int64_t lane_i64(int64_t v, int l) {
  const uint32_t lo = lane_u32((uint32_t)v, l), hi = lane_u32((uint32_t)((uint64_t)v >> 32), l);
  return (int64_t)(((uint64_t)hi << 32) | lo);
}
__device__ __forceinline__ int uniform(int v) { return __builtin_amdgcn_readfirstlane(v); }
__device__ __forceinline__ float lane_f32(float v, int l) {
  return __uint_as_float(lane_u32(__float_as_uint(v), l));
}

__device__ __forceinline__ uint32_t wave_max_u32(uint32_t v) {
  v = max(v, (uint32_t)__builtin_amdgcn_mov_dpp((int)v, 0xB1, 0xF, 0xF, false));
  v = max(v, (uint32_t)__builtin_amdgcn_mov_dpp((int)v, 0x4E, 0xF, 0xF, false));
  v = max(v, (uint32_t)__builtin_amdgcn_mov_dpp((int)v, 0x141, 0xF, 0xF, false));
  v = max(v, (uint32_t)__builtin_amdgcn_mov_dpp((int)v, 0x140, 0xF, 0xF, false));
  const uint32_t a = __builtin_amdgcn_readlane(v, 0), b = __builtin_amdgcn_readlane(v, 16);
  const uint32_t c = __builtin_amdgcn_readlane(v, 32), d = __builtin_amdgcn_readlane(v, 48);
  return max(max(a, b), max(c, d));
}

__device__ __forceinline__ uint32_t wave_sum_u32(uint32_t v) {
  v += (uint32_t)__builtin_amdgcn_mov_dpp((int)v, 0xB1, 0xF, 0xF, false);
  v += (uint32_t)__builtin_amdgcn_mov_dpp((int)v, 0x4E, 0xF, 0xF, false);
  v += (uint32_t)__builtin_amdgcn_mov_dpp((int)v, 0x141, 0xF, 0xF, false);
  v += (uint32_t)__builtin_amdgcn_mov_dpp((int)v, 0x140, 0xF, 0xF, false);
  return (uint32_t)__builtin_amdgcn_readlane((int)v, 0) + (uint32_t)__builtin_amdgcn_readlane((int)v, 16) +
         (uint32_t)__builtin_amdgcn_readlane((int)v, 32) + (uint32_t)__builtin_amdgcn_readlane((int)v, 48);
}

template <int TL>
__device__ __forceinline__ uint32_t seg_sum_u32(uint32_t v) {
  if (TL >= 1) v += (uint32_t)__builtin_amdgcn_mov_dpp((int)v, 0xB1, 0xF, 0xF, false);
  if (TL >= 2) v += (uint32_t)__builtin_amdgcn_mov_dpp((int)v, 0x4E, 0xF, 0xF, false);
  if (TL >= 3) v += (uint32_t)__builtin_amdgcn_mov_dpp((int)v, 0x141, 0xF, 0xF, false);
  if (TL >= 4) v += (uint32_t)__builtin_amdgcn_mov_dpp((int)v, 0x140, 0xF, 0xF, false);
  if (TL >= 5) v += (uint32_t)__shfl_xor((int)v, 16, 64);
  if (TL >= 6) v += (uint32_t)__shfl_xor((int)v, 32, 64);
  return v;
}
template <int TL>
__device__ __forceinline__ float seg_sum_f32(float v) {
  if (TL >= 1) v += __int_as_float(__builtin_amdgcn_mov_dpp(__float_as_int(v), 0xB1, 0xF, 0xF, false));
  if (TL >= 2) v += __int_as_float(__builtin_amdgcn_mov_dpp(__float_as_int(v), 0x4E, 0xF, 0xF, false));
  if (TL >= 3) v += __int_as_float(__builtin_amdgcn_mov_dpp(__float_as_int(v), 0x141, 0xF, 0xF, false));
  if (TL >= 4) v += __int_as_float(__builtin_amdgcn_mov_dpp(__float_as_int(v), 0x140, 0xF, 0xF, false));
  if (TL >= 5) v += __shfl_xor(v, 16, 64);
  if (TL >= 6) v += __shfl_xor(v, 32, 64);
  return v;
}

__device__ __forceinline__ uint32_t wave_or_u32(uint32_t v) {
  v |= (uint32_t)__builtin_amdgcn_mov_dpp((int)v, 0xB1, 0xF, 0xF, false);
  v |= (uint32_t)__builtin_amdgcn_mov_dpp((int)v, 0x4E, 0xF, 0xF, false);
  v |= (uint32_t)__builtin_amdgcn_mov_dpp((int)v, 0x141, 0xF, 0xF, false);
  v |= (uint32_t)__builtin_amdgcn_mov_dpp((int)v, 0x140, 0xF, 0xF, false);
  return (uint32_t)__builtin_amdgcn_readlane((int)v, 0) | (uint32_t)__builtin_amdgcn_readlane((int)v, 16) |
         (uint32_t)__builtin_amdgcn_readlane((int)v, 32) | (uint32_t)__builtin_amdgcn_readlane((int)v, 48);
}

__device__ __forceinline__ uint32_t wave_incl_scan(uint32_t x) {
  const int lane = lane_id();
#pragma unroll
  for (int o = 1; o < 64; o <<= 1) {
    const uint32_t y = (uint32_t)__shfl_up((int)x, o, 64);
    if (lane >= o) x += y;
  }
  return x;
}

__device__ __forceinline__ void lds_add(float* p, float v) {
  __hip_atomic_fetch_add(p, v, __ATOMIC_RELAXED, __HIP_MEMORY_SCOPE_WORKGROUP);
}

__device__ __forceinline__ float mul_rn(float w, float v) {
#pragma clang fp contract(off)
  return w * v;
}

template <int S, bool WT = false>
__device__ __forceinline__ void add_group(const IndexArgs& a, int64_t beg, uint32_t len, float wt,
                                          int ng, float* acc) {
  const int lane = lane_id();
  const uint32_t incl = wave_incl_scan(len);
  const uint32_t start = incl - len;
  const int64_t delta = beg - (int64_t)start;
// ... 527 lines not shown
    }
    const uint32_t wm = wave_max_u32(__float_as_uint(m));
    const int64_t last = min<int64_t>(base + (int64_t)(i + 1) * per * 256 - 1, n_docs - 1);
    const uint64_t key = wm == 0u ? 0ull
                         : ((uint64_t)score_key(__uint_as_float(wm)) << 32) |
                               (uint64_t)(0xFFFFFFFFu - (uint32_t)last - idoff);
    if (lane == (uint32_t)i) out[i] = key;
  }
  zero_acc<S>(acc);
}

template <int S>
__device__ __forceinline__ void best1_pos(float* acc, int64_t tile, uint32_t idoff,
                                          uint64_t* __restrict__ out, uint64_t* mirror) {
  constexpr int E4 = (1 << S) / 256;
  float4* a4 = reinterpret_cast<float4*>(acc);
  const uint32_t lane = lane_id();
  float m = 0.f;
#pragma unroll
  for (int j = 0; j < E4; ++j) {
    const float4 f = a4[j * 64 + lane];
    m = fmaxf(m, fmaxf(fmaxf(f.x, f.y), fmaxf(f.z, f.w)));
  }
  const uint32_t wm = wave_max_u32(__float_as_uint(m));
  uint64_t key = 0ull;
  if (wm != 0u) {
    const float fm = __uint_as_float(wm);
    uint32_t bd = 0xFFFFFFFFu;
#pragma unroll
    for (int j = E4 - 1; j >= 0; --j) {
      const float4 f = a4[j * 64 + lane];
      bd = f.w == fm ? entry_doc(4 * j + 3, lane) : bd;
      bd = f.z == fm ? entry_doc(4 * j + 2, lane) : bd;
      bd = f.y == fm ? entry_doc(4 * j + 1, lane) : bd;
      bd = f.x == fm ? entry_doc(4 * j + 0, lane) : bd;
    }
    const uint32_t doc = 0xFFFFFFFFu - wave_max_u32(0xFFFFFFFFu - bd);
    key = ((uint64_t)score_key(fm) << 32) |
          (uint64_t)(0xFFFFFFFFu - (uint32_t)((tile << S) + doc) - idoff);
  }
  zero_acc<S>(acc);
  if (lane == 0) *out = key;
  if (lane == 1 && mirror) *mirror = key;
}
template <int S, int PH>
__global__ __launch_bounds__(64 * kWaves) void score_wave_kernel(
    IndexArgs a, const int32_t* __restrict__ queries, int32_t T, Stage sg,
    const uint64_t* __restrict__ theta, uint64_t* __restrict__ cand, uint64_t* __restrict__ list,
    int32_t* __restrict__ list_cnt, int32_t C) {
  constexpr int D = 1 << S;
  __shared__ __attribute__((aligned(16))) float acc_all[kWaves * D];
  const int wave = uniform((int)(threadIdx.x >> 6));
  float* acc = acc_all + wave * D;
  const int64_t nq = sg.nq_dev ? (int64_t)*sg.nq_dev : (int64_t)sg.nq_host;
  const int P = sg.P;
  const int64_t nt = PH == kSample ? sample_count(a.ntiles, P, sg.G) : a.ntiles;
  const int64_t nitems = nt * nq;
  const int64_t per = (nitems + 7) >> 3;
  const int64_t grp = blockIdx.x & 7;
  const int64_t lo = grp * per;
  const int64_t hi = min(nitems, lo + per);
  const int64_t stride = (int64_t)(gridDim.x >> 3) * kWaves;
  int64_t it = lo + (int64_t)(blockIdx.x >> 3) * kWaves + wave;
  if (it >= hi) return;
  zero_acc<S>(acc);
  for (; it < hi; it += stride) {
    const int64_t ti = it / nq;
    const int64_t qi = it - ti * nq;
    const int64_t q = sg.qmap ? (int64_t)sg.qmap[qi] : qi;
    const int64_t tile = tile_of<PH>(ti, P, sg.G);
    add_item<S>(a, tile, queries + q * T, T, acc);
    float fv[D / 64];
    take_entries<S>(acc, fv);
    if (PH == kRest)
      emit_above<S>(fv, tile, a.n_docs, theta[qi], list + qi * C, list_cnt + qi, C);
    else
      select_top<S>(fv, tile, a.n_docs, PH == kSample ? sg.M : kTileM,
                    PH == kSample ? (uint32_t)a.doc_offset : 0u,
                    sg.cand_out + qi * sg.cstride + ti * (PH == kSample ? sg.M : kTileM));
  }
}
#ifndef BM25_QW
#define BM25_QW 4
#endif
constexpr int kQW = BM25_QW;
#ifndef BM25_FR
#define BM25_FR 10
#endif
#ifndef BM25_FR_S
#define BM25_FR_S 8
#endif

#ifndef BM25_FLAT_WPE
#define BM25_FLAT_WPE 5
#endif

#ifndef BM25_CLAMP
#define BM25_CLAMP 2
#endif

#ifndef BM25_TRACE
#define BM25_TRACE 0
#endif
#if BM25_TRACE
constexpr int kTraceWaves = 1 << 14;
__device__ uint64_t g_bm25_trace[4 * kTraceWaves];
#endif

__device__ __forceinline__ uint32_t scan64(uint32_t x) {
  x += (uint32_t)__builtin_amdgcn_update_dpp(0, (int)x, 0x111, 0xF, 0xF, true);
  x += (uint32_t)__builtin_amdgcn_update_dpp(0, (int)x, 0x112, 0xF, 0xF, true);
  x += (uint32_t)__builtin_amdgcn_update_dpp(0, (int)x, 0x114, 0xF, 0xF, true);
  x += (uint32_t)__builtin_amdgcn_update_dpp(0, (int)x, 0x118, 0xF, 0xF, true);
  x += (uint32_t)__builtin_amdgcn_update_dpp(0, (int)x, 0x142, 0xA, 0xF, false);
  x += (uint32_t)__builtin_amdgcn_update_dpp(0, (int)x, 0x143, 0xC, 0xF, false);
  return x;
}

struct FlatCur {
  int32_t rit, end, b, q, qb, bw;
};

struct FlatDesc {
  uint32_t ip, r0, r1;
  uint32_t aux;
};

__device__ __forceinline__ float f16_bits_to_float(uint16_t h) {
  _Float16 x;
  __builtin_memcpy(&x, &h, 2);
  return (float)x;
}

constexpr uint32_t kRowNewTile = 1u << 17;
constexpr uint32_t kRowParity = 1u << 24;
constexpr uint32_t kRowDead = 1u << 25;
__device__ __forceinline__ uint32_t row_lo(uint32_t w) { return w & 1u; }
__device__ __forceinline__ uint32_t row_n0(uint32_t w) { return (w >> 1) & 0xFFu; }
__device__ __forceinline__ uint32_t row_n1(uint32_t w) { return (w >> 9) & 0xFFu; }
__device__ __forceinline__ uint32_t row_tile(uint32_t w) { return (w >> 18) & 0x3Fu; }

struct FlatTab {
  uint32_t base;
  uint32_t w;
  uint32_t last;
};

struct FlatCtx {
  int32_t q, b;
  uint64_t th;
};

constexpr uint32_t kNoTile = 0xFFFFFFFFu;
template <int TL>
__device__ __forceinline__ FlatTab flat_chunk(uint32_t sb, uint32_t sl, uint32_t incl,
                                              uint32_t excl, uint32_t total, uint32_t j0,
                                              uint32_t prev, uint32_t par) {
  const uint32_t lane = lane_id();
  const uint32_t j = j0 + lane;
  int pos = 0;
#pragma unroll
  for (int step = 32; step >= 1; step >>= 1) {
    const uint32_t x = (uint32_t)__shfl((int)incl, pos + step - 1, 64);
    if (x <= j) pos += step;
  }
  const uint32_t e = (uint32_t)__shfl((int)excl, pos, 64);
  const uint32_t b = (uint32_t)__shfl((int)sb, pos, 64);
  const uint32_t l = (uint32_t)__shfl((int)sl, pos, 64);
  const bool in = j < total;
  FlatTab t;
  const uint32_t k = j - e;
  t.base = (in && l != 0u) ? ((b & ~1u) + 128u * k) * 2u : 0u;
  const uint32_t rlo = k == 0u ? (b & 1u) : 0u;
  const uint32_t rhi = min(128u, (b & 1u) + l - 128u * k);
  const uint32_t masks = (in && l != 0u) ? (rlo | ((((rhi + 1u) >> 1) - rlo) << 1) | ((rhi >> 1) << 9))
                                         : 0u;
  const uint32_t tile = (uint32_t)pos >> TL;
  uint32_t tp = (uint32_t)__shfl_up((int)tile, 1, 64);
  if (lane == 0u) tp = prev;
  const uint32_t top1 = masks != 0u ? (((rhi + 1u) >> 1) - 1u) : 0u;
  t.w = masks | ((in && tile != tp) ? kRowNewTile : 0u) | (tile << 18) | (par ? kRowParity : 0u) |
        (top1 << 26);
  t.last = lane_u32(tile, 63);
  return t;
}

__host__ __device__ inline int flat_tl(int64_t T) {
  return T <= 8 ? 3 : (T <= 16 ? 4 : (T <= 32 ? 5 : 6));
}

template <int S, int PH, int SM, bool SP, int TL>
__global__ __launch_bounds__(64) __attribute__((amdgpu_waves_per_eu(BM25_FLAT_WPE, BM25_FLAT_WPE))) void score_flat_kernel(
    IndexArgs a, const int32_t* __restrict__ queries, int32_t T, int32_t P, int32_t G,
    int32_t nq_host, const int32_t* __restrict__ nq_dev, const int32_t* __restrict__ qmap,
    const uint64_t* __restrict__ theta, uint64_t* __restrict__ cand, int64_t cstride,
    uint64_t* __restrict__ list, int32_t* __restrict__ list_cnt, int32_t C,
    int32_t* __restrict__ wctr, int32_t claim_ch, int32_t claim_m,
    const uint64_t* __restrict__ skeys, int64_t sstride, int32_t BW, uint64_t* mirror,
    int32_t* __restrict__ stats, int32_t* __restrict__ slot_cnt,
    const uint32_t* __restrict__ sub, const int32_t* __restrict__ sub_ipb) {
  constexpr int D = 1 << S;
  constexpr bool kSplit = PH == kRest && SM == kSplitM;
  constexpr int kFR = PH == kSample ? BM25_FR_S : BM25_FR;
  constexpr uint32_t TT = 1u << TL;
  constexpr uint32_t kTileMask = (64u >> TL) - 1u;
  __shared__ __attribute__((aligned(16))) float acc[D + 64];
  constexpr bool kCross = PH == kRest && SM == kLargeM;
  __shared__ uint16_t xl[kCross ? kCrossCap : 1];
  const uint32_t lane = lane_id();
  const uint32_t trash = ((uint32_t)D + lane) * 4u;
  const int32_t nq = (PH == kAll && nq_dev) ? uniform(*nq_dev) : nq_host;
  const int32_t nt = PH == kSample ? (int32_t)sample_count(a.ntiles, P, G) : (int32_t)a.ntiles;
  const int32_t nb = (nt + BW - 1) / BW;
  const int32_t ipb = kSplit ? uniform(*sub_ipb) : nq;
  const int64_t nitems = (int64_t)nb * ipb;
  const int64_t per = (nitems + 7) >> 3;
  const int grp = (int)(blockIdx.x & 7);
  const uint32_t lo = (uint32_t)(grp * per);
  const int32_t ngi = (int32_t)max<int64_t>(0, min<int64_t>(nitems, lo + per) - lo);
  if (ngi == 0) return;
  const int32_t cm = (int32_t)(blockIdx.x >> 3) % claim_m;
  int32_t* ctr = wctr + (grp * kClaimM + cm) * kCtrStride;
  auto finish = [&]() {
    const int32_t g8 = (int32_t)(gridDim.x >> 3);
    const int32_t sharers = g8 / claim_m + (cm < g8 % claim_m ? 1 : 0);
    int32_t old = 0;
    if (lane == 0) old = atomicAdd(ctr + kDoneOff, 1);
    if (uniform(old) == sharers - 1 && lane == 0) {
      ctr[0] = 0;
      ctr[kDoneOff] = 0;
    }
  };
#if BM25_CLAMP == 2
  const PostingRsrc pr = posting_rsrc_pairs(a);
#else
  const PostingRsrc pr = posting_rsrc(a);
#endif
#if BM25_TRACE
  const uint64_t tr_t0 = wall_clock64();
  uint32_t tr_items = 0, tr_rows = 0;
#endif
  const uint32_t lt = lane & (TT - 1u), li = lane >> TL;
  const int64_t nbp = (a.ntiles + 7) >> 3;

  auto dec = [&](FlatCur& c, uint32_t it) {
    const uint32_t band = it / (uint32_t)ipb;
    const uint32_t e = uniform((int)sub[it - band * (uint32_t)ipb]);
    c.q = (int32_t)(e & 0xFFFFFu);
    c.qb = c.q;
    c.b = (int32_t)(band * (uint32_t)BW + ((e >> 20) & 63u));
    c.bw = min((int32_t)(e >> 26), nt - c.b);
  };
  auto claim = [&]() -> int32_t {
    int32_t v = 0;
    if (lane == 0) v = atomicAdd(ctr, 1);
    return v;
  };
  int32_t pending = claim();
  auto batch_row = [&](int32_t q) -> int32_t {
    return (PH == kAll && qmap) ? uniform(qmap[q]) : q;
  };
  auto next = [&](FlatCur c) -> FlatCur {
    if (c.rit >= ngi) return c;
    if (c.rit + 1 < c.end) {
      ++c.rit;
      if constexpr (kSplit) {
        dec(c, lo + (uint32_t)c.rit);
        return c;
      }
      if (++c.q == nq) {
        c.q = 0;
        c.b += BW;
        c.bw = min(BW, nt - c.b);
      }
      c.qb = batch_row(c.q);
      return c;
    }
    const int64_t bb = ((int64_t)uniform(pending) * claim_m + cm) * claim_ch;
    if (bb >= ngi) {
      c.rit = c.end = ngi;
      return c;
    }
    pending = claim();
    FlatCur n;
    n.rit = (int32_t)bb;
    n.end = (int32_t)min<int64_t>(ngi, bb + claim_ch);
    const uint32_t it = lo + (uint32_t)bb;
    if constexpr (kSplit) {
      dec(n, it);
      return n;
    }
    const uint32_t band = it / (uint32_t)nq;
    n.q = (int32_t)(it - band * (uint32_t)nq);
    n.qb = batch_row(n.q);
    n.b = (int32_t)band * BW;
    n.bw = min(BW, nt - n.b);
    return n;
  };
  auto terms_of = [&](const FlatCur& c) -> int32_t {
    return queries[(int64_t)c.qb * T + (int)min(lt, (uint32_t)(T - 1))];
  };
  constexpr bool kBits = PH == kRest && TL == 3 && SM != kLargeM;
  const bool skipping = PH == kRest && skeys != nullptr && G == kSampleGroup &&
                        !(kBits && a.tskip != nullptr);
  const uint32_t lgG = (uint32_t)__builtin_ctz((unsigned)G), lgP = (uint32_t)__builtin_ctz((unsigned)P);
  auto load_bdesc = [&](const FlatCur& c, int32_t tm) -> FlatDesc {
    FlatDesc d;
    const int32_t term = tm;
    const bool ok = (int)lt < T && (int)li < c.bw && term >= 0 && term < a.V;
    const int64_t tt = ok ? term : 0;
    const int64_t tile = ok ? (int64_t)tile_of32<PH>((uint32_t)(c.b + li), (uint32_t)P,
                                                      (uint32_t)G)
                            : 0;
    if constexpr (SP) {
      const uint64_t e = a.seg[ok ? ((int64_t)c.qb * nbp + (tile >> 3)) * (8 * TT) + lt * 8 + (tile & 7)
                                  : a.seg_zero];
      d.ip = 0u;
      d.r0 = (uint32_t)e;
      d.r1 = (uint32_t)e + (uint32_t)(e >> 32);
    } else {
      const uint32_t* r = a.rel + tt * (a.ntiles + 1) + tile;
      d.ip = (uint32_t)a.indptr[tt];
      d.r0 = r[0];
      d.r1 = *(ok ? r + 1 : r);
    }
    d.aux = 0u;
    if (kBits && a.tskip != nullptr) {
      const uint32_t t32 = (uint32_t)c.b + li;
      if ((int)li < c.bw)
        d.aux = ((uint32_t)a.tskip[(int64_t)c.q * a.tskip_stride + t32] >> lt) & 1u;
    } else if (skipping) {
      const uint32_t t32 = (uint32_t)tile;
      const int64_t si = (int64_t)(((t32 >> (lgG + lgP)) << lgG) | (t32 & (uint32_t)(G - 1)));
      d.aux = reinterpret_cast<const uint32_t*>(skeys)[2 * ((int64_t)c.q * sstride +
                                                              min<int64_t>(si, sstride - 1)) + 1];
    }
    return d;
  };
  auto th_positive = [&](uint64_t th) -> bool {
    return (uint32_t)(th >> 32) > score_key(0.f);
  };

  uint32_t nbound = 0;
  constexpr bool kCountPost = PH == kRest && SM == 2;
  uint32_t npost = 0;
  uint32_t ndrop = 0, ndpost = 0;
  uint32_t iSb = 0, iSl = 0, iIncl = 0, iExcl = 0;
  uint32_t iTotal = 0, iR = 0, iJ0 = 0, iPrev = kNoTile, iCur = 0;
  int32_t ctxV = 0, iPar = 0;
  FlatCur nx, nx2;
  FlatDesc dN;
  uint64_t thN = 0ull;
  int32_t tmN2 = 0;
  auto enter_item = [&]() {
#if BM25_TRACE
    ++tr_items;
#endif
    const bool th_pos = PH == kRest && th_positive(thN);
    const uint32_t t32 = (uint32_t)nx.b + li;
    const bool smp = skipping && ((t32 >> lgG) & (uint32_t)(P - 1)) == 0u;
    bool skip = smp && th_pos && dN.aux < (uint32_t)(thN >> 32);
    if constexpr (PH == kRest) {
      if (kBits && a.tskip != nullptr) {
        const bool drop = dN.aux != 0u;
        if constexpr (kCountPost) {
          const bool cut = seg_sum_u32<TL>(dN.aux) == TT;
          const uint32_t sl = dN.r1 - dN.r0;
          const uint32_t tp = seg_sum_u32<TL>(sl);
          const bool cnt = cut && !skip && lt == 0u && (int)li < nx.bw;
          nbound += (uint32_t)__popcll(__ballot(cnt));
          npost += wave_sum_u32(cnt ? tp : 0u);
          const bool dcnt = drop && !cut && !skip && sl != 0u;
          ndrop += (uint32_t)__popcll(__ballot(dcnt));
          ndpost += wave_sum_u32(dcnt ? sl : 0u);
        }
        skip = skip || drop;
      }
    }
    iSb = dN.ip + dN.r0;
    iSl = skip ? 0u : dN.r1 - dN.r0;
    uint32_t nr = iSl == 0u ? 0u : ((iSb & 1u) + iSl + 127u) >> 7;
    if ((PH == kAll || (PH == kRest && !th_pos)) && lt == 0u && (int)li < nx.bw)
      nr = max(nr, 1u);
    if constexpr (PH == kSample) {
      const uint32_t tr = seg_sum_u32<TL>(nr);
      if (lt == 0u && (int)li < nx.bw && tr == 0u) {
        uint64_t* out = cand + (int64_t)nx.q * cstride + (int64_t)(nx.b + (int32_t)li) * SM;
#pragma unroll
        for (int i = 0; i < SM; ++i) out[i] = 0ull;
        if (SM == 1 && mirror) mirror[out - cand] = 0ull;
      }
    }
    iIncl = scan64(nr);
    iExcl = iIncl - nr;
    iTotal = lane_u32(iIncl, 63);
    uint32_t R = max(iTotal, (uint32_t)kFR);
    if ((R & 63u) != 0u && (R & 63u) < (uint32_t)kFR) R += (uint32_t)kFR - (R & 63u);
    iR = R;
    iJ0 = 0;
    iPrev = kNoTile;
    {
      const int32_t c4 = (int32_t)lane - 4 * iPar;
      ctxV = c4 == 0 ? nx.q : c4 == 1 ? nx.b : c4 == 2 ? (int32_t)(uint32_t)thN
           : c4 == 3 ? (int32_t)(uint32_t)(thN >> 32) : ctxV;
    }
    iCur = (uint32_t)iPar;
    iPar ^= 1;
    FlatCur nx3 = next(nx2);
    dN = load_bdesc(nx2, tmN2);
    thN = PH == kRest ? theta[nx2.q] : 0ull;
    tmN2 = terms_of(nx3);
    nx = nx2;
    nx2 = nx3;
  };

  FlatCur c0;
  c0.rit = -1;
  c0.end = 0;
  c0.b = c0.q = c0.qb = 0;
  c0.bw = 1;
  nx = next(c0);
  if (nx.rit >= ngi) {
    finish();
    return;
  }
  dN = load_bdesc(nx, terms_of(nx));
  thN = PH == kRest ? theta[nx.q] : 0ull;
  nx2 = next(nx);
  tmN2 = terms_of(nx2);
  for (int j = 0; j < D / 256; ++j)
    reinterpret_cast<float4*>(acc)[j * 64 + lane] = make_float4(0.f, 0.f, 0.f, 0.f);
  acc[D + lane] = -__builtin_inff();

  bool items_left = true;
  FlatTab tI;
  uint32_t nI = 0, il = 0;
  auto next_chunk = [&]() {
    if (iJ0 + 64u < iR) {
      iJ0 += 64u;
      iPrev = tI.last;
    } else if (items_left && nx.rit < ngi) {
      enter_item();
    } else {
      items_left = false;
      tI.base = 0u;
      tI.w = kRowDead;
      nI = 0x7FFFFFFFu;
      il = 0;
      return;
    }
    tI = flat_chunk<TL>(iSb, iSl, iIncl, iExcl, iTotal, iJ0, iPrev, iCur);
    nI = min(64u, iR - iJ0);
    il = 0;
  };
  enter_item();
  tI = flat_chunk<TL>(iSb, iSl, iIncl, iExcl, iTotal, 0u, iPrev, iCur);
  nI = min(64u, iR);
  il = 0;

  uint32_t ldR[kFR], wR[kFR];
  float v0R[kFR], v1R[kFR];
  auto issue = [&](int s) {
    if (il == nI) next_chunk();
    const uint32_t base = lane_u32(tI.base, (int)il);
    wR[s] = lane_u32(tI.w, (int)il);
#if BM25_CLAMP == 2
    const int li2 = (int)min(lane, wR[s] >> 26);
    ldR[s] = bm25_sload_b32(pr.ldoc, li2, 0, (int)base, 0);
    const bm25_v2u v = bm25_sload_b64(pr.val, li2, 0, (int)(base * 2u), 0);
    v0R[s] = __uint_as_float(v[0]);
    v1R[s] = __uint_as_float(v[1]);
#else
#if BM25_CLAMP
    const uint32_t wv = wR[s];
    const uint32_t top = max(row_lo(wv) + row_n0(wv), row_n1(wv));
    const uint32_t t4 = (top > 0u ? top - 1u : 0u) * 4u;
    const uint32_t lo4 = min(lane * 4u, t4), lo8 = min(lane * 8u, 2u * t4);
#else
    const uint32_t lo4 = lane * 4u, lo8 = lane * 8u;
#endif
    ldR[s] = __builtin_amdgcn_raw_buffer_load_b32(pr.ldoc, (int)lo4, (int)base, 0);
    const auto v = __builtin_amdgcn_raw_buffer_load_b64(pr.val, (int)lo8, (int)(base * 2u), 0);
    v0R[s] = __uint_as_float((uint32_t)v[0]);
    v1R[s] = __uint_as_float((uint32_t)v[1]);
#endif
    ++il;
  };
#pragma unroll
  for (int s = 0; s < kFR; ++s) issue(s);

  FlatCtx ctxE{0, 0, 0ull};
  uint32_t curTi = kNoTile;
  float hmax = 0.f;
  bool done = false;
  float thS = 0.f;
  int32_t ncross = 0;

  auto epilogue = [&]() {
    const int32_t ti = ctxE.b + (int32_t)curTi;
    const int64_t tile = tile_of32<PH>((uint32_t)ti, (uint32_t)P, (uint32_t)G);
    if constexpr (kCross) {
      const int64_t si = (int64_t)ctxE.q * a.ntiles + tile;
      if (ncross == 0)
        zero_acc<S>(acc);
      else if (ncross <= kCrossCap)
        emit_cross<S>(acc, xl, ncross, tile, a.n_docs, ctxE.th, cand + si * cstride,
                      (int32_t)cstride, slot_cnt + si, list + (int64_t)ctxE.q * C,
                      list_cnt + ctxE.q, C);
      else
        emit_rest_slot<S>(acc, tile, a.n_docs, ctxE.th, cand + si * cstride, (int32_t)cstride,
                          slot_cnt + si, list + (int64_t)ctxE.q * C, list_cnt + ctxE.q, C);
    } else if constexpr (PH == kRest) {
      const bool flagged = a.nonneg && th_positive(ctxE.th);
      if (flagged && __ballot(hmax >= key_score((uint32_t)(ctxE.th >> 32))) == 0) {
        zero_acc<S>(acc);
      } else {
        emit_rest<S>(acc, tile, a.n_docs, ctxE.th, list + (int64_t)ctxE.q * C,
                     list_cnt + ctxE.q, C);
      }
      hmax = 0.f;
    } else if constexpr (PH == kAll) {
      select_top_lds<S>(acc, tile, a.n_docs, kTileM, cand + (int64_t)ctxE.q * cstride + tile * kTileM);
    } else {
      uint64_t* out = cand + (int64_t)ctxE.q * cstride + (int64_t)ti * SM;
      if constexpr (SM == 1) {
        if (a.nonneg) {
          const uint32_t wm = wave_max_u32(__float_as_uint(hmax));
          const uint32_t last = (uint32_t)min<int64_t>((tile << S) + D - 1, a.n_docs - 1);
          const uint64_t key = wm == 0u ? 0ull
                               : ((uint64_t)score_key(__uint_as_float(wm)) << 32) |
                                     (uint64_t)(0xFFFFFFFFu - last - (uint32_t)a.doc_offset);
          zero_acc<S>(acc);
          if (lane == 0) *out = key;
          if (lane == 1 && mirror) mirror[out - cand] = key;
          hmax = 0.f;
        } else {
          best1_pos<S>(acc, tile, (uint32_t)a.doc_offset, out, mirror ? mirror + (out - cand) : nullptr);
        }
      } else if (SM == kLargeM || a.nonneg) {
        best_slices_pos<S, SM>(acc, tile, a.n_docs, (uint32_t)a.doc_offset, out);
      } else {
        best_dense<S, SM, true>(acc, tile, a.n_docs, (uint32_t)a.doc_offset, out);
      }
    }
  };

  uint32_t sc0, sc1, wC;
  float ac0, ac1, xc0, xc1;
  auto lds_at = [&](uint32_t off) -> float& {
    return *reinterpret_cast<float*>(reinterpret_cast<char*>(acc) + off);
  };
  auto prepare = [&](int s) {
    wC = wR[s];
    const bool m0 = lane - row_lo(wC) < row_n0(wC), m1 = lane < row_n1(wC);
    sc0 = m0 ? (ldR[s] & 0xFFFFu) : trash;
    sc1 = m1 ? (ldR[s] >> 16) : trash;
    ac0 = v0R[s];
    ac1 = v1R[s];
    xc0 = lds_at(sc0);
    xc1 = lds_at(sc1);
  };
  prepare(0);

  auto step = [&](int s) {
    issue(s);
    if (wC & kRowNewTile) {
      if (curTi != kNoTile) epilogue();
      curTi = row_tile(wC) & kTileMask;
      const int32_t pPar = (wC & kRowParity) ? 1 : 0;
      ctxE.q = __builtin_amdgcn_readlane(ctxV, 4 * pPar);
      ctxE.b = __builtin_amdgcn_readlane(ctxV, 4 * pPar + 1);
      ctxE.th = ((uint64_t)(uint32_t)__builtin_amdgcn_readlane(ctxV, 4 * pPar + 3) << 32) |
                (uint32_t)__builtin_amdgcn_readlane(ctxV, 4 * pPar + 2);
      xc0 = sc0 == trash ? xc0 : 0.f;
      xc1 = sc1 == trash ? xc1 : 0.f;
      if constexpr (kCross) {
        thS = key_score((uint32_t)(ctxE.th >> 32));
        ncross = th_positive(ctxE.th) ? 0 : kCrossCap + 1;
      }
    }
    const float y0 = xc0 + ac0, y1 = xc1 + ac1;
    lds_at(sc0) = y0;
    lds_at(sc1) = y1;
    if constexpr (kCross) {
      const uint64_t m0 = __ballot(y0 >= thS);
      const uint64_t m1 = __ballot(y1 >= thS);
      if ((m0 | m1) != 0ull) {
        const int32_t n0 = (int32_t)__popcll(m0), n1 = (int32_t)__popcll(m1);
        if (ncross + n0 + n1 <= kCrossCap) {
          const uint32_t b0 = __builtin_amdgcn_mbcnt_hi((uint32_t)(m0 >> 32),
                                                        __builtin_amdgcn_mbcnt_lo((uint32_t)m0, 0u));
          const uint32_t b1 = __builtin_amdgcn_mbcnt_hi((uint32_t)(m1 >> 32),
                                                        __builtin_amdgcn_mbcnt_lo((uint32_t)m1, 0u));
          if ((m0 >> lane) & 1ull) xl[ncross + (int32_t)b0] = (uint16_t)sc0;
          if ((m1 >> lane) & 1ull) xl[ncross + n0 + (int32_t)b1] = (uint16_t)sc1;
        }
        ncross += n0 + n1;
      }
    } else if (PH == kRest || (PH == kSample && SM == 1)) {
      hmax = fmaxf(hmax, fmaxf(y0, y1));
    }
    done = (wC & kRowDead) != 0u;
    prepare((s + 1) % kFR);
  };

  while (!done) {
#pragma unroll
    for (int s = 0; s < kFR; ++s) step(s);
#if BM25_TRACE
    tr_rows += kFR;
#endif
  }
#if BM25_TRACE
  if (PH == kRest && lane == 0 && blockIdx.x < kTraceWaves) {
    uint64_t* tr = g_bm25_trace + 4 * blockIdx.x;
    tr[0] = tr_t0;
    tr[1] = wall_clock64();
    tr[2] = tr_items;
    tr[3] = tr_rows;
  }
#endif
  if (curTi != kNoTile) epilogue();
  if (kCountPost && stats != nullptr) {
    const uint32_t nb = nbound;
    if (lane == 0 && nb != 0u) atomicAdd(stats, (int32_t)nb);
    const uint32_t np = npost;
    if (lane == 0 && np != 0u)
      atomicAdd(reinterpret_cast<unsigned long long*>(stats + 1), (unsigned long long)np);
    const uint32_t nd = ndrop;
    if (lane == 0 && nd != 0u) atomicAdd(stats + 3, (int32_t)nd);
    const uint32_t ndp = ndpost;
    if (lane == 0 && ndp != 0u)
      atomicAdd(reinterpret_cast<unsigned long long*>(stats + 5), (unsigned long long)ndp);
  }
  finish();
}

constexpr int kRescoreNT = 256;

__device__ __forceinline__ void bitonic_sort_desc(uint64_t* keys, int n) {
  for (int size = 2; size <= n; size <<= 1) {
    for (int stride = size >> 1; stride > 0; stride >>= 1) {
      const int ls = __builtin_ctz((unsigned)stride);
      for (int i = threadIdx.x; i < (n >> 1); i += blockDim.x) {
        const int lo = ((i >> ls) << (ls + 1)) + (i & (stride - 1));
        const int hi = lo + stride;
        const bool desc = (lo & size) == 0;
        const uint64_t x = keys[lo], y = keys[hi];
        if ((x < y) == desc) {
          keys[lo] = y;
          keys[hi] = x;
        }
      }
      __syncthreads();
    }
  }
}

template <int S>
__device__ void rescore_tile(const IndexArgs& a, const int32_t* __restrict__ queries, int32_t T,
                             int32_t k, int64_t q, int64_t tile, uint64_t* out, float* acc,
                             uint64_t* keys) {
  constexpr int D = 1 << S;
  if (threadIdx.x < 64) {
    zero_acc<S>(acc);
    add_item<S>(a, tile, queries + q * T, T, acc);
  }
  __syncthreads();
  for (int i = threadIdx.x; i < D; i += blockDim.x) {
    const int64_t doc = (tile << S) + i;
    keys[i] = doc < a.n_docs ? make_key(acc[i], (uint32_t)doc) : 0ull;
  }
  __syncthreads();
  bitonic_sort_desc(keys, D);
  for (int i = threadIdx.x; i < k; i += blockDim.x) out[i] = i < D ? keys[i] : 0ull;
}

template <int S>
__global__ __launch_bounds__(kRescoreNT) void rescore_kernel(IndexArgs a,
                                                             const int32_t* __restrict__ queries,
                                                             int32_t T, int32_t k, int64_t maxflag,
                                                             Stage sg, Workspace ws) {
  constexpr int D = 1 << S;
  __shared__ __attribute__((aligned(16))) float acc[D];
  __shared__ uint64_t keys[D];
  __shared__ int32_t s_item;
  const int32_t n_items = ws.counters[0];
  for (;;) {
    __syncthreads();
    if (threadIdx.x == 0) s_item = atomicAdd(&ws.counters[1], 1);
    __syncthreads();
    const int32_t it = s_item;
    if (it >= n_items) break;
    const int32_t code = ws.queue[it];
    const int64_t qi = code / maxflag;
    const int64_t q = sg.qmap ? (int64_t)sg.qmap[qi] : qi;
    const int64_t tile = sample_tile(ws.flag_tiles[code], sg.P, sg.G);
    rescore_tile<S>(a, queries, T, k, q, tile, ws.cand2 + (int64_t)code * k, acc, keys);
  }
}

template <int S>
__global__ __launch_bounds__(64) void scores_dense_kernel(IndexArgs a,
                                                          const int32_t* __restrict__ query,
                                                          int32_t T, float* __restrict__ out) {
  constexpr int D = 1 << S, E = D / 64;
  __shared__ __attribute__((aligned(16))) float acc[D];
  const int64_t tile = blockIdx.x;
  zero_acc<S>(acc);
  add_item<S>(a, tile, query, T, acc);
  float fv[E];
  take_entries<S>(acc, fv);
  const int64_t base = tile << S;
  const uint32_t lane = lane_id();
  if (base + D <= a.n_docs) {
#pragma unroll
    for (int j = 0; j < E / 4; ++j)
      *reinterpret_cast<float4*>(out + base + entry_doc(4 * j, lane)) =
          make_float4(fv[4 * j], fv[4 * j + 1], fv[4 * j + 2], fv[4 * j + 3]);
  } else {
#pragma unroll
    for (int e = 0; e < E; ++e)
      if (base + entry_doc(e, lane) < a.n_docs) out[base + entry_doc(e, lane)] = fv[e];
  }
}

template <int S, bool WT = false>
__global__ __launch_bounds__(64) void scores_batch_kernel(IndexArgs a,
                                                          const int32_t* __restrict__ queries,
                                                          int32_t T, int64_t stride,
                                                          float* __restrict__ out,
                                                          const float* __restrict__ weights) {
  constexpr int D = 1 << S, E = D / 64;
  __shared__ __attribute__((aligned(16))) float acc[D];
  const int64_t tile = blockIdx.x, g = blockIdx.y;
  zero_acc<S>(acc);
  add_item<S, WT>(a, tile, queries + g * T, T, acc, WT ? weights + g * T : nullptr);
  float fv[E];
  take_entries<S>(acc, fv);
  float* row = out + g * stride + (tile << S);
  const uint32_t lane = lane_id();
#pragma unroll
  for (int j = 0; j < E / 4; ++j)
    *reinterpret_cast<float4*>(row + entry_doc(4 * j, lane)) =
        make_float4(fv[4 * j], fv[4 * j + 1], fv[4 * j + 2], fv[4 * j + 3]);
}

__global__ __launch_bounds__(256) void build_tables_kernel(
    const int64_t* __restrict__ indptr, const int32_t* __restrict__ indices, int64_t V,
    int64_t n_docs, int S, int64_t ntiles, uint32_t* __restrict__ rel,
    uint16_t* __restrict__ ldoc, int32_t* __restrict__ err) {
  const int lane = lane_id();
  const int64_t waves = (int64_t)gridDim.x * (blockDim.x >> 6);
  const uint32_t mask = (1u << S) - 1u;
  for (int64_t t = (int64_t)blockIdx.x * (blockDim.x >> 6) + (threadIdx.x >> 6); t < V;
       t += waves) {
    const int64_t a0 = indptr[t], a1 = indptr[t + 1];
    const int64_t df = a1 - a0;
    uint32_t* row = rel + t * (ntiles + 1);
    const bool heavy = df * 4 >= ntiles;
    for (int64_t p = a0 + lane; p < a1; p += 64) {
      const int32_t d = indices[p];
      const int32_t dp = p > a0 ? indices[p - 1] : -1;
      const bool ok = d >= 0 && (int64_t)d < n_docs && d > dp;
      if (!ok) atomicOr(err, 1);
      ldoc[p] = (uint16_t)(((uint32_t)d & mask) << 2);
      if (heavy && ok) {
        const int64_t tp = dp >= 0 ? ((int64_t)dp >> S) : -1;
        const int64_t tc = (int64_t)d >> S;
        for (int64_t j = tp + 1; j <= tc; ++j) row[j] = (uint32_t)(p - a0);
      }
    }
    if (heavy) {
      int64_t last = -1;
      if (df > 0) {
        const int32_t dl = indices[a1 - 1];
        last = (dl >= 0 && (int64_t)dl < n_docs) ? ((int64_t)dl >> S) : ntiles - 1;
      }
      for (int64_t j = last + 1 + lane; j <= ntiles; j += 64) row[j] = (uint32_t)df;
    } else {
      for (int64_t j = lane; j <= ntiles; j += 64) {
        const int64_t target = j << S;
        int64_t lo = 0, hi = df;
        while (lo < hi) {
          const int64_t mid = (lo + hi) >> 1;
          if ((int64_t)indices[a0 + mid] < target) lo = mid + 1;
          else hi = mid;
        }
        row[j] = (uint32_t)lo;
      }
    }
  }
}

__global__ __launch_bounds__(256) void build_bmax_kernel(const int64_t* __restrict__ indptr,
                                                         const uint32_t* __restrict__ rel,
                                                         const float* __restrict__ val, int64_t V,
                                                         int64_t ntiles,
                                                         uint16_t* __restrict__ bmax) {
  const int64_t bs = bmax_stride(ntiles);
  for (int64_t t = blockIdx.x; t < V; t += gridDim.x) {
    const int64_t ip = indptr[t];
    const uint32_t* r = rel + t * (ntiles + 1);
    for (int64_t j = ntiles + threadIdx.x; j < bs; j += blockDim.x) bmax[t * bs + j] = 0;
    for (int64_t j = threadIdx.x; j < ntiles; j += blockDim.x) {
      float m = 0.f;
      for (int64_t p = ip + r[j]; p < ip + r[j + 1]; ++p) m = fmaxf(m, val[p]);
      _Float16 h = (_Float16)m;
      uint16_t u;
      __builtin_memcpy(&u, &h, 2);
      if ((float)h > m) --u;
      bmax[t * bs + j] = u;
    }
  }
}

__global__ __launch_bounds__(256) void build_tmask_kernel(const int64_t* __restrict__ indptr,
                                                          const uint32_t* __restrict__ rel,
                                                          const uint16_t* __restrict__ ldoc,
                                                          int64_t V, int64_t ntiles, int S,
                                                          uint32_t* __restrict__ tmask) {
  const int64_t bs = bmax_stride(ntiles);
  for (int64_t t = blockIdx.x; t < V; t += gridDim.x) {
    const int64_t ip = indptr[t];
    const uint32_t* r = rel + t * (ntiles + 1);
    for (int64_t j = ntiles + threadIdx.x; j < bs; j += blockDim.x) tmask[t * bs + j] = 0u;
    for (int64_t j = threadIdx.x; j < ntiles; j += blockDim.x) {
      uint32_t m = 0u;
      for (int64_t p = ip + r[j]; p < ip + r[j + 1]; ++p) m |= 1u << ((uint32_t)ldoc[p] >> (S - 3));
      tmask[t * bs + j] = m;
    }
  }
}

constexpr int kSkipNT = 256;
constexpr int kSkipTerms = 8;
inline int skip_npt(int64_t ntiles) {
  const int64_t bs = bmax_stride(ntiles);
  return bs >= 4 * kSkipNT ? 4 : (bs >= 2 * kSkipNT ? 2 : 1);
}
constexpr uint32_t kSkipBias = 0x80000000u - 1048472u;
template <int N> struct alignas(2 * N) SkipB { uint16_t v[N]; };
template <int N> struct alignas(4 * N) SkipM { uint32_t v[N]; };
template <int N> struct alignas(N) SkipO { uint8_t v[N]; };
template <int N>
__global__ __launch_bounds__(kSkipNT) void tile_skip_kernel(
    const uint16_t* __restrict__ bmax, const uint32_t* __restrict__ tmask, int64_t V,
    int64_t ntiles, const int32_t* __restrict__ queries, int32_t T, int64_t Q,
    const uint64_t* __restrict__ theta, uint8_t* __restrict__ tskip, int32_t seg) {
  const int64_t bs = bmax_stride(ntiles);
  const int64_t nch = (bs + kSkipNT * N - 1) / (kSkipNT * N);
  for (int64_t it = blockIdx.x; it < Q * nch; it += gridDim.x) {
    const int64_t q = it / nch;
    const int64_t t0 = ((it - q * nch) * kSkipNT + threadIdx.x) * N;
    if (t0 >= bs) continue;
    const uint32_t thk = (uint32_t)(theta[q] >> 32);
    SkipO<N> out;
#pragma unroll
    for (int i = 0; i < N; ++i) out.v[i] = 0;
    if (thk > score_key(0.f) && t0 < ntiles) {
      SkipB<N> bb[kSkipTerms];
      SkipM<N> mm[kSkipTerms];
      uint32_t okm = 0u;
#pragma unroll
      for (int t = 0; t < kSkipTerms; ++t) {
#pragma unroll
        for (int i = 0; i < N; ++i) {
          bb[t].v[i] = 0;
          mm[t].v[i] = 0u;
        }
        if (t < T) {
          const int32_t term = queries[q * T + t];
          if (term >= 0 && term < V) {
            okm |= 1u << t;
            bb[t] = *reinterpret_cast<const SkipB<N>*>(bmax + term * bs + t0);
            if (tmask != nullptr) mm[t] = *reinterpret_cast<const SkipM<N>*>(tmask + term * bs + t0);
          }
        }
      }
      const float th = key_score(thk);
      const float K = 1048576.f / th;
#pragma unroll
      for (int i = 0; i < N; ++i) {
        if (t0 + i >= ntiles) break;
        float ub[kSkipTerms];
        uint32_t mk[kSkipTerms];
#pragma unroll
        for (int t = 0; t < kSkipTerms; ++t) {
          ub[t] = ((okm >> t) & 1u) ? f16_bits_to_float((uint16_t)(bb[t].v[i] + 1u)) : 0.f;
          mk[t] = mm[t].v[i];
        }
        const float sum = ((ub[0] + ub[1]) + (ub[2] + ub[3])) + ((ub[4] + ub[5]) + (ub[6] + ub[7]));
        uint32_t byte = sum * 1.0001f < th ? 0xFFu : 0u;
        if (byte == 0u && tmask != nullptr) {
          uint32_t c[kSkipTerms];
#pragma unroll
          for (int t = 0; t < kSkipTerms; ++t)
            c[t] = mk[t] != 0u ? (uint32_t)ceilf(fminf(ub[t] * K, 2097152.f)) + 1u : 0u;
          uint32_t L = 0u;
#pragma unroll
          for (int s = 31; s >= 0; --s) {
            uint32_t acc = kSkipBias;
#pragma unroll
            for (int t = 0; t < kSkipTerms; ++t) acc += __umul24((mk[t] >> s) & 1u, c[t]);
            L = __builtin_amdgcn_alignbit(L, acc, 31);
          }
          if (L == 0u) {
            byte = 0xFFu;
          } else if (seg) {
#pragma unroll
            for (int t = 0; t < kSkipTerms; ++t) byte |= (mk[t] & L) == 0u ? 1u << t : 0u;
          }
        }
        out.v[i] = (uint8_t)byte;
      }
    }
    *reinterpret_cast<SkipO<N>*>(tskip + q * bs + t0) = out;
  }
}

__global__ __launch_bounds__(256) void pool_bounds_kernel(const uint16_t* __restrict__ in,
                                                          int64_t rows, int64_t in_stride,
                                                          uint16_t* __restrict__ out,
                                                          int64_t out_stride) {
  const int64_t n = rows * out_stride;
  for (int64_t e = (int64_t)blockIdx.x * 256 + threadIdx.x; e < n; e += (int64_t)gridDim.x * 256) {
    const int64_t r = e / out_stride, g = e - r * out_stride;
    uint16_t m = 0;
    for (int64_t j = g * kPool; j < min<int64_t>((g + 1) * kPool, in_stride); ++j)
      m = max(m, in[r * in_stride + j]);
    out[e] = m;
  }
}

constexpr int kBoundNT = 256;

__device__ __forceinline__ void block_kth_u16(const uint64_t* lbq, int32_t nq4, uint32_t k,
                                              uint32_t* hist, uint32_t* sh, uint32_t& v,
                                              uint32_t& need) {
  const uint32_t lane = lane_id();
  uint32_t hi = 0u, nd = k;
#pragma unroll
  for (int pass = 0; pass < 2; ++pass) {
    for (int i = (int)threadIdx.x; i < 256; i += kBoundNT) hist[i] = 0u;
    __syncthreads();
    for (int32_t g = (int32_t)threadIdx.x; g < nq4; g += kBoundNT) {
      const uint64_t x = lbq[g];
#pragma unroll
      for (int u = 0; u < 4; ++u) {
        const uint32_t val = (uint32_t)(x >> (16 * u)) & 0xFFFFu;
        if (pass == 0) atomicAdd(&hist[val >> 8], 1u);
        else if ((val >> 8) == hi) atomicAdd(&hist[val & 255u], 1u);
      }
    }
    __syncthreads();
    if (threadIdx.x < 64) {
      uint32_t c[4], t = 0u;
#pragma unroll
      for (int j = 0; j < 4; ++j) {
        c[j] = hist[255 - 4 * (int)lane - j];
        t += c[j];
      }
      uint32_t above = wave_incl_scan(t) - t;
      uint32_t bin1 = 0u, rk = 0u;
#pragma unroll
      for (int j = 0; j < 4; ++j) {
        if (above < nd && nd <= above + c[j]) {
          bin1 = 256u - 4u * lane - (uint32_t)j;
          rk = nd - above;
        }
        above += c[j];
      }
      bin1 = wave_max_u32(bin1);
      rk = wave_max_u32(rk);
      if (lane == 0) {
        sh[0] = bin1;
        sh[1] = rk;
      }
    }
    __syncthreads();
    const uint32_t b = sh[0] - 1u;
    nd = sh[1];
    hi = pass == 0 ? b : hi;
    v = pass == 0 ? (b << 8) : (v | b);
    __syncthreads();
  }
  need = nd;
}

__device__ void split_table(const IndexArgs& a, const int32_t* __restrict__ queries, int32_t T,
                            int64_t q, int32_t nq, int32_t bwmax, uint32_t* __restrict__ qw,
                            uint32_t* __restrict__ sub, int32_t* __restrict__ sub_ipb,
                            int32_t* __restrict__ sub_done, uint32_t* sh ) {
  __shared__ int32_t s_last;
  if (threadIdx.x == 0) {
    const int32_t* qt = queries + q * T;
    uint64_t w = 0;
    for (int i = 0; i < T; ++i) {
      const int32_t t = qt[i];
      bool dup = t < 0 || (int64_t)t >= a.V;
      for (int j = 0; j < i && !dup; ++j) dup = qt[j] == t;
      if (!dup) w += (uint64_t)(a.indptr[t + 1] - a.indptr[t]);
    }
    qw[q] = (uint32_t)min<uint64_t>(w, 0xFFFFFFFFull);
    __threadfence();
    s_last = atomicAdd(sub_done, 1) == nq - 1;
  }
  __syncthreads();
  if (!s_last) return;
  __threadfence();
  const uint32_t lane = lane_id(), wv = threadIdx.x >> 6;
  uint64_t tw = 0;
  for (int32_t i = (int32_t)threadIdx.x; i < nq; i += kBoundNT) tw += __hip_atomic_load(qw + i, __ATOMIC_RELAXED, __HIP_MEMORY_SCOPE_AGENT);
  uint32_t tw32 = (uint32_t)min<uint64_t>(tw, 0xFFFFFFFFull);
  tw32 = wave_sum_u32(tw32);
  if (lane == 0) sh[2 + wv] = tw32;
  __syncthreads();
  uint64_t tot = 0;
#pragma unroll
  for (int i = 0; i < kBoundNT / 64; ++i) tot += sh[2 + i];
  const double lim = 1.25 * (double)tot / (double)nq;
  const int32_t per = (nq + kBoundNT - 1) / kBoundNT;
  const int32_t q0 = (int32_t)threadIdx.x * per;
  uint32_t fsum = 0u;
  for (int32_t i = q0; i < min(nq, q0 + per); ++i) {
    const double w = (double)__hip_atomic_load(qw + i, __ATOMIC_RELAXED, __HIP_MEMORY_SCOPE_AGENT);
    uint32_t f = 1u;
    while ((int32_t)f < bwmax && w > lim * (double)f) f <<= 1;
    fsum += f;
  }
  const uint32_t incl = wave_incl_scan(fsum);
  __syncthreads();
  if (lane == 63) sh[2 + wv] = incl;
  __syncthreads();
  uint32_t base = incl - fsum;
  for (int i = 0; i < (int)wv; ++i) base += sh[2 + i];
  for (int32_t i = q0; i < min(nq, q0 + per); ++i) {
    const double w = (double)__hip_atomic_load(qw + i, __ATOMIC_RELAXED, __HIP_MEMORY_SCOPE_AGENT);
    uint32_t f = 1u;
    while ((int32_t)f < bwmax && w > lim * (double)f) f <<= 1;
    const uint32_t width = (uint32_t)bwmax / f;
    for (uint32_t j = 0; j < f; ++j) sub[base + j] = (uint32_t)i | ((j * width) << 20) | (width << 26);
    base += f;
  }
  if (threadIdx.x == kBoundNT - 1) {
    *sub_ipb = (int32_t)base;
    *sub_done = 0;
  }
}

typedef unsigned short bm25_us4 __attribute__((ext_vector_type(4)));
template <int TMAX, int GPI>
__device__ __forceinline__ void bound_rows(const IndexArgs& a, const uint16_t* __restrict__ bmax,
                                           const int32_t* __restrict__ qt, int32_t T, int64_t bs,
                                           int32_t gpr, int32_t nq4, int64_t rrank, bool world,
                                           uint64_t* lbq) {
  const uint64_t* row[TMAX];
  bool has[TMAX];
#pragma unroll
  for (int i = 0; i < TMAX; ++i) {
    const int32_t t = i < T ? __builtin_amdgcn_readfirstlane(qt[i]) : -1;
    has[i] = t >= 0 && (int64_t)t < a.V;
    row[i] = reinterpret_cast<const uint64_t*>(bmax + (has[i] ? (int64_t)t * bs : 0));
  }
  for (int32_t g0 = (int32_t)threadIdx.x; g0 < nq4; g0 += GPI * kBoundNT) {
    int64_t o[GPI];
#pragma unroll
    for (int j = 0; j < GPI; ++j) {
      const int32_t g = g0 + j * kBoundNT;
      const int32_t w = world ? g / gpr : 0;
// ... 1165 lines not shown
    key[j] = i < cnt ? y : 0ull;
  }
  uint32_t kept = 0;
  const uint64_t kth = wave_kth_key<R>(key, k, kept);
  __builtin_amdgcn_fence(__ATOMIC_ACQ_REL, "wavefront");
  uint32_t base = 0u;
#pragma unroll
  for (int j = 0; j < R; ++j) {
    const bool keep = key[j] != 0ull && key[j] >= kth;
    const uint64_t b = __ballot(keep);
    if (keep)
      kb[base + __builtin_amdgcn_mbcnt_hi((uint32_t)(b >> 32),
                                          __builtin_amdgcn_mbcnt_lo((uint32_t)b, 0u))] = key[j];
    base += (uint32_t)__popcll(b);
  }
  wave_sort_write(kb, kept, next_pow2(kept > 1u ? kept : 2u), k, doc_offset, q, docs, scores);
}

__global__ __launch_bounds__(64 * kQW) void merge_sorted_kernel(
    const int32_t* __restrict__ in_docs, const float* __restrict__ in_scores, int32_t W,
    int64_t Q, int32_t k, int64_t rstride, int32_t* __restrict__ docs,
    float* __restrict__ scores) {
  __shared__ uint64_t buf[kQW][kMergeSortedCap];
  const int wave = (int)(threadIdx.x >> 6);
  const int64_t q = (int64_t)blockIdx.x * kQW + wave;
  if (q >= Q) return;
  uint64_t* kb = buf[wave];
  const uint32_t lane = lane_id();
  uint32_t cnt = 0u;
  const int nc = (k + 63) >> 6;
  const int ncol = W * nc;
  int cw = 0, cc = 0;
  for (int b0 = 0; b0 < ncol; b0 += 8) {
    float sv[8];
    int32_t dv[8];
    int w = cw, c = cc;
#pragma unroll
    for (int u = 0; u < 8; ++u) {
      const int j = c * 64 + (int)lane;
      const bool in = b0 + u < ncol && j < k;
      const int64_t off = in ? (int64_t)w * rstride + q * k + j : q * k;
      const float sy = in_scores[off];
      const int32_t dy = in_docs[off];
      sv[u] = in ? sy : 0.f;
      dv[u] = in ? dy : -1;
      if (++c == nc) {
        c = 0;
        ++w;
      }
    }
    cw = w;
    cc = c;
#pragma unroll
    for (int u = 0; u < 8; ++u) {
      const bool nz = dv[u] >= 0;
      const uint64_t b = __ballot(nz);
      if (nz)
        kb[cnt + __builtin_amdgcn_mbcnt_hi((uint32_t)(b >> 32),
                                           __builtin_amdgcn_mbcnt_lo((uint32_t)b, 0u))] =
            make_key(sv[u], (uint32_t)dv[u]);
      cnt += (uint32_t)__popcll(b);
    }
  }
  if (k <= 128 && cnt > 256u) {
    uint64_t smp[2];
#pragma unroll
    for (int j = 0; j < 2; ++j) smp[j] = kb[(((uint32_t)j * 64u + lane) * cnt) >> 7];
    wave_sort_regs<2>(smp);
    const int r = min(127, max(0, (int)((4u * (uint32_t)k * 64u) / cnt)));
    const uint64_t t1 = __shfl(r >= 64 ? smp[1] : smp[0], r & 63, 64);
    uint64_t key[kMergeSortedCap / 64];
    uint32_t c = 0u;
#pragma unroll
    for (int j = 0; j < kMergeSortedCap / 64; ++j) {
      const uint32_t i = (uint32_t)j * 64u + lane;
      const uint64_t y = kb[i < cnt ? i : 0u];
      key[j] = i < cnt ? y : 0ull;
      c += key[j] != 0ull && key[j] >= t1;
    }
    c = wave_sum_u32(c);
    if (t1 != 0ull && c >= (uint32_t)k && c <= 512u) {
      __builtin_amdgcn_fence(__ATOMIC_ACQ_REL, "wavefront");
      uint32_t base = 0u;
#pragma unroll
      for (int j = 0; j < kMergeSortedCap / 64; ++j) {
        const bool keep = key[j] != 0ull && key[j] >= t1;
        const uint64_t b = __ballot(keep);
        if (keep)
          kb[base + __builtin_amdgcn_mbcnt_hi((uint32_t)(b >> 32),
                                              __builtin_amdgcn_mbcnt_lo((uint32_t)b, 0u))] = key[j];
        base += (uint32_t)__popcll(b);
      }
      __builtin_amdgcn_fence(__ATOMIC_RELEASE, "wavefront");
      if (base <= 256u)
        regs_sort_write<4>(kb, base, k, 0, q, docs, scores);
      else
        regs_sort_write<8>(kb, base, k, 0, q, docs, scores);
      return;
    }
  }

  if (cnt <= 512u) {
    sort_write_any<8>(kb, cnt, k, 0, q, docs, scores);
    return;
  }
  __builtin_amdgcn_fence(__ATOMIC_RELEASE, "wavefront");
  lds_merge_one<kMergeSortedCap / 64>(kb, cnt, k, 0, q, docs, scores);
}

#ifndef BM25_TILE_SHIFT
#define BM25_TILE_SHIFT 11
#endif
static_assert(BM25_TILE_SHIFT == 11 || BM25_TILE_SHIFT == 12, "2048- or 4096-doc tiles");
bool tile_shift_supported(int s) { return s == BM25_TILE_SHIFT; }
int build_tile_shift() { return BM25_TILE_SHIFT; }

hipError_t launch_build_tables(const DevIndex& ix, const int32_t* d_indices, int32_t* d_err,
                               hipStream_t stream) {
  if (ix.n_terms == 0) return hipSuccess;
  int64_t blocks = (ix.n_terms + 3) / 4;
  if (blocks > 65536) blocks = 65536;
  hipLaunchKernelGGL(build_tables_kernel, dim3((unsigned)blocks), dim3(256), 0, stream,
                     ix.indptr, d_indices, ix.n_terms, ix.n_docs, ix.tile_shift, ix.ntiles,
                     ix.rel, ix.ldoc, d_err);
  return hipGetLastError();
}

hipError_t launch_pool_bounds(const uint16_t* in, int64_t rows, int64_t in_stride, uint16_t* out,
                              int64_t out_stride, hipStream_t stream) {
  if (rows <= 0 || out_stride <= 0) return hipSuccess;
  const int64_t n = rows * out_stride;
  const unsigned blocks = (unsigned)std::min<int64_t>((n + 255) / 256, 65536);
  hipLaunchKernelGGL(pool_bounds_kernel, dim3(blocks), dim3(256), 0, stream, in, rows, in_stride,
                     out, out_stride);
  return hipGetLastError();
}

hipError_t launch_build_bmax(const DevIndex& ix, hipStream_t stream) {
  if (ix.n_terms == 0 || ix.ntiles == 0 || !ix.bmax || ix.sparse) return hipSuccess;
  const int64_t blocks = std::min<int64_t>(ix.n_terms, 65536);
  hipLaunchKernelGGL(build_bmax_kernel, dim3((unsigned)blocks), dim3(256), 0, stream, ix.indptr,
                     ix.rel, ix.val, ix.n_terms, ix.ntiles, ix.bmax);
  return hipGetLastError();
}

hipError_t launch_build_tmask(const DevIndex& ix, hipStream_t stream) {
  if (ix.n_terms == 0 || ix.ntiles == 0 || !ix.tmask || ix.sparse) return hipSuccess;
  const int64_t blocks = std::min<int64_t>(ix.n_terms, 65536);
  hipLaunchKernelGGL(build_tmask_kernel, dim3((unsigned)blocks), dim3(256), 0, stream, ix.indptr,
                     ix.rel, ix.ldoc, ix.n_terms, ix.ntiles, ix.tile_shift, ix.tmask);
  return hipGetLastError();
}

hipError_t launch_count_tiles(const DevIndex& ix, const int32_t* d_indices, int64_t* d_cnt,
                              int32_t* d_err, hipStream_t stream) {
  if (ix.n_terms == 0) return hipSuccess;
  const int64_t blocks = std::min<int64_t>((ix.n_terms + 3) / 4, 65536);
  hipLaunchKernelGGL(count_tiles_kernel, dim3((unsigned)blocks), dim3(256), 0, stream, ix.indptr,
                     d_indices, ix.n_terms, ix.n_docs, ix.tile_shift, ix.ldoc, d_cnt, d_err);
  return hipGetLastError();
}

hipError_t launch_fill_tiles(const DevIndex& ix, const int32_t* d_indices, hipStream_t stream) {
  if (ix.n_terms == 0) return hipSuccess;
  const int64_t blocks = std::min<int64_t>((ix.n_terms + 3) / 4, 65536);
  hipLaunchKernelGGL(fill_tiles_kernel, dim3((unsigned)blocks), dim3(256), 0, stream, ix.indptr,
                     d_indices, ix.n_terms, ix.tile_shift, ix.tl_ptr, ix.tl_tile, ix.tl_start);
  return hipGetLastError();
}

SampleGeom sample_geom(int64_t ntiles, int k, int W, int pmax) {
  for (int P = 64; P >= 2; P >>= 1) {
    if (P > pmax || ntiles < 2 * P) continue;
    const int G = ntiles >= 4 * kSampleGroup * P ? kSampleGroup : 1;
    const int64_t nS = sample_count(ntiles, P, G);
    for (int m = 1; m <= kTileM; m <<= 1)
      if (nS * m * W >= 2 * (int64_t)k) return SampleGeom{P, m, nS * m, G};
  }
  return SampleGeom{1, 0, 0, 1};
}

SampleGeom search_geom(const DevIndex& ix, int64_t ntiles, int k, int W, int64_t T) {
  const SampleGeom g = sample_geom(ntiles, k, W, ix.opt.sample_p);
  const bool bounds = ix.ntiles == 0 || (ix.bmax != nullptr && ix.nonneg && !ix.sparse);
  if (g.P > 1 && ix.opt.theta_bound && !ix.bound_weak && bounds && k >= 1 && T >= 1 &&
      T <= kBoundMaxTerms &&
      ntiles <= kBoundMaxTiles && ntiles * std::max(W, 1) >= kBoundTilesPerK * (int64_t)k)
    return SampleGeom{0, 1, g.S, 1};
  return g;
}

SampleGeom shard_geom_world(const DevIndex& ix, int k, int64_t T, bool world) {
  if (world && ix.wbmax != nullptr) {
    const SampleGeom g = search_geom(ix, ix.wtiles, k, 1, T);
    if (g.P == 0) return g;
  }
  return search_geom(ix, ix.ntiles, k, 1, T);
}

static int device_cus(int dev) {
  static std::mutex mu;
  static std::map<int, int> cache;
  std::lock_guard<std::mutex> lk(mu);
  const auto it = cache.find(dev);
  if (it != cache.end()) return it->second;
  int cus = 0;
  if (hipDeviceGetAttribute(&cus, hipDeviceAttributeMultiprocessorCount, dev) != hipSuccess || cus <= 0)
    cus = 256;
  cache[dev] = cus;
  return cus;
}

template <class K>
static int persistent_grid(K kernel, int block) {
  static std::mutex mu;
  static std::map<std::pair<const void*, int>, int> cache;
  int dev = 0;
  hipGetDevice(&dev);
  std::lock_guard<std::mutex> lk(mu);
  const auto key = std::make_pair((const void*)kernel, dev);
  const auto it = cache.find(key);
  if (it != cache.end()) return it->second;
  int occ = 0;
  const int cus = device_cus(dev);
  hipOccupancyMaxActiveBlocksPerMultiprocessor(&occ, kernel, block, 0);
  const int g = ((cus * (occ > 0 ? occ : 1) + 7) / 8) * 8;
  cache[key] = g;
  return g;
}

static bool use_flat(const DevIndex& ix, int64_t T, int64_t Q) {
  return ix.opt.flat && T >= 1 && T <= 64 && (ix.nnz + kPostingPad) * 4 < 0xFFFFFFF0ll &&
         ix.ntiles * Q < 0x7FFFFFFFll;
}

static int32_t flat_band(const SearchOpts& o, int64_t nt, int64_t nq, int grid, int bwmax,
                         bool fallback) {
  if (o.flat_bw > 0) return std::min(o.flat_bw, bwmax);
  if (fallback) return 1;
  int32_t bw = bwmax;
  while (bw > 1 && ((nt + bw - 1) / bw) * nq < (int64_t)o.items_per_wave * grid) bw >>= 1;
  return bw;
}

int flat_term_lanes(int64_t T) { return 1 << flat_tl(T); }

template <int S, int PH, int SM, int TL>
static void launch_flat(const DevIndex& ix, const int32_t* q, int64_t T, int64_t Qb,
                        const Stage& sg, const Workspace& ws, hipStream_t st) {
  int32_t* wctr = ws.wctr + (int64_t)sg.ctr_region * kWctrInts;
  constexpr bool kSlots = PH == kRest && SM == kLargeM;
  const bool skip = PH == kRest && sg.sample_keys != nullptr && sg.M == 1 && sg.G == kSampleGroup;
  IndexArgs a = args_of(ix);
  if (PH == kRest && !skip && !kSlots && TL == 3 && ix.opt.tile_bound && ix.bmax != nullptr &&
      ws.tskip != nullptr) {
    a.tskip = ws.tskip;
    a.tskip_stride = tskip_stride(ix.ntiles);
    const uint32_t* tmask = ix.opt.tile_mask ? ix.tmask : (const uint32_t*)nullptr;
    const bool seg = ix.opt.seg_skip && tmask != nullptr;
    ix.disp.kernels |= kKTileSkip | (seg ? kKSegSkip : 0);
    auto pre = [&](auto kern, int npt) {
      const int64_t per = (int64_t)kSkipNT * npt;
      const int64_t items = sg.nq_host * ((a.tskip_stride + per - 1) / per);
      const int grid = (int)std::min<int64_t>(items, persistent_grid(kern, kSkipNT));
      hipLaunchKernelGGL(kern, dim3((unsigned)grid), dim3(kSkipNT), 0, st, ix.bmax, tmask,
                         ix.n_terms, ix.ntiles, q, (int32_t)T, (int64_t)sg.nq_host, ws.theta,
                         ws.tskip, (int32_t)seg);
    };
    switch (skip_npt(ix.ntiles)) {
      case 4: pre(tile_skip_kernel<4>, 4); break;
      case 2: pre(tile_skip_kernel<2>, 2); break;
      default: pre(tile_skip_kernel<1>, 1); break;
    }
  }
  a.seg = ws.seg;
  a.seg_zero = Qb * ((ix.ntiles + 7) >> 3) * 8 * (1 << TL);
  const int64_t nt = PH == kSample ? sample_count(ix.ntiles, sg.P, sg.G) : ix.ntiles;
  auto go = [&](auto kern) {
    int grid = persistent_grid(kern, 64);
    if (ix.opt.grid_pct < 100) grid = std::max(8, grid * ix.opt.grid_pct / 100 / 8 * 8);
    if (sg.nq_dev) grid = std::min(grid, 8 * kFallbackBlocks);
    const int claim_m = std::max(1, std::min(ix.opt.claim_m, grid / 8));
    const int bw = SM == kSplitM ? (64 >> TL)
                                 : flat_band(ix.opt, nt, sg.nq_host, grid, 64 >> TL, sg.nq_dev != nullptr);
    ix.disp.kernels |= PH == kSample ? kKFlatSample : (PH == kRest ? kKFlatRest : kKFlatAll);
    if (PH == kRest && SM == 2) ix.disp.kernels |= kKCountSkips;
    ix.disp.term_lanes = 1 << TL;
    ix.disp.band_tiles[PH] = bw;
    hipLaunchKernelGGL(kern, dim3((unsigned)grid), dim3(64), 0, st, a, q, (int32_t)T, sg.P,
                       sg.G, sg.nq_host, sg.nq_dev, sg.qmap, ws.theta,
                       kSlots ? ws.slots : sg.cand_out, kSlots ? (int64_t)ws.slot_cap : sg.cstride,
                       ws.list, ws.list_cnt, ws.list_cap, wctr, ix.opt.claim_ch, claim_m,
                       skip ? sg.sample_keys : nullptr, sg.sample_stride, bw,
                       PH == kSample && SM == 1 ? sg.cand_mirror : nullptr,
                       PH == kRest ? ws.counters + 5 : nullptr, kSlots ? ws.slot_cnt : nullptr,
                       SM == kSplitM ? ws.sub : nullptr, SM == kSplitM ? ws.sub_ipb : nullptr);
  };
  if (ix.sparse)
    go(score_flat_kernel<S, PH, SM, true, TL>);
  else
    go(score_flat_kernel<S, PH, SM, false, TL>);
}

template <int S, int PH, int SM>
static void launch_flat_tl(const DevIndex& ix, const int32_t* q, int64_t T, int64_t Qb,
                           const Stage& sg, const Workspace& ws, hipStream_t st) {
  switch (flat_tl(T)) {
    case 3: launch_flat<S, PH, SM, 3>(ix, q, T, Qb, sg, ws, st); break;
    case 4: launch_flat<S, PH, SM, 4>(ix, q, T, Qb, sg, ws, st); break;
    case 5: launch_flat<S, PH, SM, 5>(ix, q, T, Qb, sg, ws, st); break;
    default: launch_flat<S, PH, SM, 6>(ix, q, T, Qb, sg, ws, st); break;
  }
}

template <int S, int PH>
static void launch_phase(const DevIndex& ix, const int32_t* q, int64_t T, int64_t Qb,
                         const Stage& sg, const Workspace& ws, hipStream_t st) {
  if (use_flat(ix, T, Qb)) {
    if constexpr (PH == kSample) {
      if (sg.M == 2) return launch_flat_tl<S, PH, 2>(ix, q, T, Qb, sg, ws, st);
      if (sg.M == kTileM) return launch_flat_tl<S, PH, kTileM>(ix, q, T, Qb, sg, ws, st);
      if (sg.M == kLargeM) return launch_flat_tl<S, PH, kLargeM>(ix, q, T, Qb, sg, ws, st);
    }
    if constexpr (PH == kRest) {
      if (sg.M == kLargeM && ws.slots != nullptr)
        return launch_flat_tl<S, PH, kLargeM>(ix, q, T, Qb, sg, ws, st);
      if (ix.opt.count_skips)
        return launch_flat_tl<S, PH, 2>(ix, q, T, Qb, sg, ws, st);
      if (sg.split && ws.sub != nullptr && flat_tl(T) == 3)
        return launch_flat_tl<S, PH, kSplitM>(ix, q, T, Qb, sg, ws, st);
    }
    return launch_flat_tl<S, PH, 1>(ix, q, T, Qb, sg, ws, st);
  }
  int32_t* wctr = ws.wctr + (int64_t)sg.ctr_region * kWctrInts;
  (void)wctr;
  ix.disp.kernels |= PH == kSample ? kKWaveSample : (PH == kRest ? kKWaveRest : kKWaveAll);
  int grid = persistent_grid(score_wave_kernel<S, PH>, 64 * kWaves);
  if (sg.nq_dev) grid = std::min(grid, 8 * kFallbackBlocks);
  hipLaunchKernelGGL((score_wave_kernel<S, PH>), dim3((unsigned)grid), dim3(64 * kWaves), 0, st,
                     args_of(ix), q, (int32_t)T, sg, ws.theta, sg.cand_out, ws.list, ws.list_cnt,
                     ws.list_cap);
}

__global__ __launch_bounds__(256) void seg_table_kernel(IndexArgs a,
                                                        const int32_t* __restrict__ queries,
                                                        int64_t Q, int32_t T, int32_t TT,
                                                        uint64_t* __restrict__ seg) {
  const int64_t w = (int64_t)blockIdx.x * 4 + (threadIdx.x >> 6);
  if (w >= Q * T) return;
  const int64_t q = w / T;
  const int pos = (int)(w - q * T);
  const int32_t term = queries[q * T + pos];
  if (term < 0 || term >= a.V) return;
  const int64_t nbp = (a.ntiles + 7) >> 3;
  const int64_t b = a.tl_ptr[term], e = a.tl_ptr[term + 1];
  const int64_t ip = a.indptr[term];
  const uint32_t df = (uint32_t)(a.indptr[term + 1] - ip);
  uint64_t* row = seg + q * nbp * 8 * TT;
  for (int64_t i = b + lane_id(); i < e; i += 64) {
    const uint32_t tile = a.tl_tile[i];
    const uint32_t st = a.tl_start[i];
    const uint32_t nx = i + 1 < e ? a.tl_start[i + 1] : df;
    row[(int64_t)(tile >> 3) * 8 * TT + pos * 8 + (tile & 7)] =
        (uint64_t)(uint32_t)(ip + st) | ((uint64_t)(nx - st) << 32);
  }
}

__global__ __launch_bounds__(256) void max_token_kernel(const int32_t* __restrict__ q, int64_t n,
                                                        int32_t* __restrict__ out) {
  int32_t m = 0;
  for (int64_t i = (int64_t)blockIdx.x * 256 + threadIdx.x; i < n; i += (int64_t)gridDim.x * 256)
    m = max(m, q[i]);
  m = (int32_t)wave_max_u32((uint32_t)max(m, 0));
  if (lane_id() == 0 && m > 0) atomicMax(out, m);
}

hipError_t launch_max_token(const int32_t* d_queries, int64_t n, int32_t* d_out,
                            hipStream_t stream) {
  hipMemsetAsync(d_out, 0, sizeof(int32_t), stream);
  if (n > 0) {
    const int64_t blocks = std::min<int64_t>((n + 255) / 256, 1024);
    hipLaunchKernelGGL(max_token_kernel, dim3((unsigned)blocks), dim3(256), 0, stream, d_queries,
                       n, d_out);
  }
  return hipGetLastError();
}

int64_t seg_entries(const DevIndex& ix, int64_t Q, int64_t T) {
  if (!ix.sparse || !use_flat(ix, T, Q)) return 0;
  return Q * ((ix.ntiles + 7) >> 3) * 8 * flat_term_lanes(T) + 64;
}

static void launch_seg_table(const DevIndex& ix, const int32_t* q, int64_t Q, int64_t T,
                             const Workspace& ws, hipStream_t st) {
  hipMemsetAsync(ws.seg, 0, sizeof(uint64_t) * seg_entries(ix, Q, T), st);
  const int64_t waves = Q * T;
  hipLaunchKernelGGL(seg_table_kernel, dim3((unsigned)((waves + 3) / 4)), dim3(256), 0, st,
                     args_of(ix), q, Q, (int32_t)T, (int32_t)flat_term_lanes(T), ws.seg);
}

static Stage main_stage(const DevIndex& ix, int64_t Q, int P, const Workspace& ws) {
  Stage sg{};
  sg.cand = ws.cand;
  sg.cand_out = ws.cand;
  sg.cstride = ix.ntiles * kTileM;
  sg.P = P;
  sg.G = 1;
  sg.nt = P != 1 ? 0 : ix.ntiles;
  sg.nq_host = (int32_t)Q;
  if (P != 1) {
    sg.theta = ws.theta;
    sg.list = ws.list;
    sg.list_cnt = ws.list_cnt;
    sg.C = ws.list_cap;
    sg.fb = ws.fb;
    sg.fb_cnt = ws.counters + 2;
  }
  return sg;
}

static Stage fallback_stage(const DevIndex& ix, int64_t Q, const Workspace& ws) {
  Stage sg{};
  sg.cand = ws.cand;
  sg.cand_out = ws.cand;
  sg.cstride = ix.ntiles * kTileM;
  sg.P = 1;
  sg.G = 1;
  sg.nt = ix.ntiles;
  sg.qmap = ws.fb;
  sg.nq_dev = ws.counters + 2;
  sg.nq_host = (int32_t)Q;
  return sg;
}

template <int S_>
static void sample_s(const DevIndex& ix, const int32_t* q, int64_t Q, int64_t T,
                     const SampleGeom& g, uint64_t* keys, const Workspace& ws, hipStream_t st) {
  if (sample_count(ix.ntiles, g.P, g.G) * g.m < g.S)
    hipMemsetAsync(keys, 0, sizeof(uint64_t) * Q * g.S, st);
  if (seg_entries(ix, Q, T) > 0) launch_seg_table(ix, q, Q, T, ws, st);
  Stage sg = main_stage(ix, Q, g.P, ws);
  sg.ctr_region = 0;
  sg.M = g.m;
  sg.G = g.G;
  sg.cand_out = keys;
  sg.cand_mirror = keys != ws.cand ? ws.cand : nullptr;
  sg.cstride = g.S;
  launch_phase<S_, kSample>(ix, q, T, Q, sg, ws, st);
}

// ... 559 lines not shown
```

Before: 491,100 queries/s.

## Add per-row (128-posting) skip masks for heavy terms in tile-bound pruning

At build time, terms with multi-row tiles are flagged and a per-tile, per-128-posting-row mask of which doc sub-segments each row touches is stored. The tile_skip kernel now writes a 16-bit row word per term instead of a byte per tile. The score_flat REST kernel uses that word to load only the rows that intersect the surviving segment mask, picking them with a k-th-set-bit lookup. The aim is to cut posting reads inside tiles that survive the tile bound. In exchange the tskip buffer is 16x larger, up to 256 MB of row masks are kept on the device, and both kernels do extra per-tile work.

```diff
diff --git a/mojo-bm25_amd/bm25mi/index.py b/mojo-bm25_amd/bm25mi/index.py
--- a/mojo-bm25_amd/bm25mi/index.py
+++ b/mojo-bm25_amd/bm25mi/index.py
@@ -988,17 +988,19 @@
         return {"kernels": {n for b, n in self.KERNELS.items() if km.value & b},
                 "tile_skip": bool(km.value & 32768),
                 "seg_skip": bool(km.value & 65536),
+                "row_skip": bool(km.value & 131072),
                 "term_lanes": tl.value,
                 "band_tiles": {"all": bt[0], "sample": bt[1], "rest": bt[2]},
                 "sample_p": sp_.value}
 
     def search_stats(self) -> dict:
-        v = (ctypes.c_int64 * 8)()
-        check(lib.bm25_search_counters(self._h, v, 8))
+        v = (ctypes.c_int64 * 10)()
+        check(lib.bm25_search_counters(self._h, v, 10))
         return {"rescored_tiles": v[0], "fallback_queries": v[1],
                 "bound_skipped_tiles": v[2], "bound_skipped_postings": v[3],
                 "block_merge_queries": v[4], "large_dense_queries": v[5],
-                "bound_dropped_segments": v[6], "bound_dropped_postings": v[7]}
+                "bound_dropped_segments": v[6], "bound_dropped_postings": v[7],
+                "bound_dropped_rows": v[8], "bound_dropped_row_postings": v[9]}
 
 
 def merge_topk_device(device: int, d_docs, d_scores, W: int, Q: int, k: int, d_out_docs,
diff --git a/mojo-bm25_amd/csrc/bm25mi_capi.cpp b/mojo-bm25_amd/csrc/bm25mi_capi.cpp
--- a/mojo-bm25_amd/csrc/bm25mi_capi.cpp
+++ b/mojo-bm25_amd/csrc/bm25mi_capi.cpp
@@ -209,7 +209,8 @@
   HIP_TRY(hipMalloc(&ws.sub_done, sizeof(int32_t)), "hipMalloc(sub_done)");
   HIP_TRY(hipMemsetAsync(ws.sub_done, 0, sizeof(int32_t), st), "hipMemsetAsync(sub_done)");
   if (h->ix.bmax)
-    HIP_TRY(hipMalloc(&ws.tskip, (size_t)std::max<int64_t>(q * tskip_stride(nt), 4)), "hipMalloc(tskip)");
+    HIP_TRY(hipMalloc(&ws.tskip, sizeof(uint16_t) * 8 * (size_t)std::max<int64_t>(q * tskip_stride(nt), 1)),
+            "hipMalloc(tskip)");
   ws.cap_seg = need_seg;
   if (ws.cap_seg > 0) HIP_TRY(hipMalloc(&ws.seg, sizeof(uint64_t) * ws.cap_seg), "hipMalloc(seg)");
   ws.list_cap = C;
@@ -571,12 +572,53 @@
     h->arrays = std::make_shared<IndexArrays>();
     h->arrays->device = device;
     h->arrays->p = {ix.indptr, ix.rel, ix.tl_ptr, ix.tl_tile, ix.tl_start, ix.ldoc, ix.val, ix.bmax,
-                    ix.bpool, ix.tmask};
+                    ix.bpool, ix.tmask, ix.hslot, ix.rowmask};
     *out = h;
   } else {
     bm25_index_destroy(h);
   }
   return rc;
+}
+
+static void build_row_masks(bm25_index* h, HostCall& c, const std::vector<int64_t>& ip) {
+  DevIndex& ix = h->ix;
+  const int64_t V = ix.n_terms;
+  const int64_t slot_bytes = (int64_t)sizeof(uint32_t) * kRowEntries * ix.ntiles;
+  const int64_t max_slots = ((int64_t)ix.opt.row_mask_kb << 10) / slot_bytes;
+  if (max_slots <= 0) return;
+  int32_t* d_heavy = c.alloc<int32_t>(V, "hipMalloc(heavy)");
+  std::vector<int32_t> heavy(V, 0);
+  if (c.ok()) c.run(launch_heavy_terms(ix, d_heavy, h->stream), "heavy_terms launch");
+  c.download(heavy.data(), d_heavy, V, "D2H heavy");
+  if (c.ok()) c.run(hipStreamSynchronize(h->stream), "heavy_terms");
+  if (!c.ok()) return;
+  std::vector<int32_t> hterm;
+  for (int64_t t = 0; t < V; ++t)
+    if (heavy[t]) hterm.push_back((int32_t)t);
+  std::stable_sort(hterm.begin(), hterm.end(), [&ip](int32_t x, int32_t y) {
+    return ip[x + 1] - ip[x] > ip[y + 1] - ip[y];
+  });
+  if ((int64_t)hterm.size() > max_slots) hterm.resize((size_t)max_slots);
+  if (hterm.empty()) return;
+  std::vector<int32_t> hslot(V, -1);
+  for (size_t i = 0; i < hterm.size(); ++i) hslot[hterm[i]] = (int32_t)i;
+  const int64_t H = (int64_t)hterm.size();
+  if (hipMalloc(&ix.hslot, sizeof(int32_t) * V) != hipSuccess ||
+      hipMalloc(&ix.rowmask, (size_t)(slot_bytes * H)) != hipSuccess) {
+    (void)hipGetLastError();
+    hipFree(ix.hslot);
+    ix.hslot = nullptr;
+    ix.rowmask = nullptr;
+    return;
+  }
+  ix.n_heavy = H;
+  int32_t* d_hterm = c.alloc<int32_t>(H, "hipMalloc(hterm)");
+  c.upload_to(ix.hslot, hslot.data(), V, "H2D hslot");
+  c.upload_to(d_hterm, hterm.data(), H, "H2D hterm");
+  if (c.ok()) c.run(launch_build_rowmask(ix, d_hterm, h->stream), "build_rowmask launch");
+  const hipError_t es = hipStreamSynchronize(h->stream);
+  if (c.ok()) c.run(es, "build_rowmask");
+  if (c.ok()) h->device_bytes += (int64_t)sizeof(int32_t) * V + slot_bytes * H;
 }
 
 static int build_index(bm25_index* h, const std::vector<int64_t>& ip, const int32_t* indices,
@@ -656,6 +698,7 @@
           hipMalloc(&ix.tmask, sizeof(uint32_t) * n_terms * bmax_stride(ntiles)) == hipSuccess) {
         c.run(launch_build_tmask(ix, h->stream), "build_tmask launch");
         h->device_bytes += (int64_t)(sizeof(uint32_t) * n_terms * bmax_stride(ntiles));
+        if (c.ok()) build_row_masks(h, c, ip);
       } else {
         (void)hipGetLastError();
         ix.tmask = nullptr;
@@ -702,7 +745,7 @@
     for (void* x : {(void*)h->ix.indptr, (void*)h->ix.rel, (void*)h->ix.tl_ptr,
                     (void*)h->ix.tl_tile, (void*)h->ix.tl_start, (void*)h->ix.ldoc,
                     (void*)h->ix.val, (void*)h->ix.bmax, (void*)h->ix.bpool,
-                    (void*)h->ix.tmask})
+                    (void*)h->ix.tmask, (void*)h->ix.hslot, (void*)h->ix.rowmask})
       hipFree(x);
   }
   hipFree(h->ix.wbpool);
@@ -1960,7 +2003,7 @@
 
 int bm25_search_counters(bm25_index* h, int64_t* out, int32_t n) {
   if (!h || !out) return fail(BM25_EINVAL, "NULL argument");
-  if (n < 1 || n > 8) return fail(BM25_EINVAL, "n=%d must be in 1..8", n);
+  if (n < 1 || n > 10) return fail(BM25_EINVAL, "n=%d must be in 1..10", n);
   Enter in(h);
   if (in.rc) return in.rc;
   int32_t cnt[kCounters] = {};
@@ -1970,9 +2013,12 @@
   const bool counted = (h->ix.disp.kernels & kKCountSkips) != 0;
   uint64_t dpost = 0;
   std::memcpy(&dpost, cnt + 10, sizeof dpost);
-  const int64_t v[8] = {cnt[3], cnt[2], counted ? cnt[5] : -1, counted ? (int64_t)post : -1,
-                        cnt[4], h->large_fallback, counted ? cnt[8] : -1,
-                        counted ? (int64_t)dpost : -1};
+  uint64_t rpost = 0;
+  std::memcpy(&rpost, cnt + 12, sizeof rpost);
+  const int64_t v[10] = {cnt[3], cnt[2], counted ? cnt[5] : -1, counted ? (int64_t)post : -1,
+                         cnt[4], h->large_fallback, counted ? cnt[8] : -1,
+                         counted ? (int64_t)dpost : -1, counted ? cnt[9] : -1,
+                         counted ? (int64_t)rpost : -1};
   for (int i = 0; i < n; ++i) out[i] = v[i];
   return BM25_OK;
 }
diff --git a/mojo-bm25_amd/csrc/bm25mi_host.h b/mojo-bm25_amd/csrc/bm25mi_host.h
--- a/mojo-bm25_amd/csrc/bm25mi_host.h
+++ b/mojo-bm25_amd/csrc/bm25mi_host.h
@@ -109,6 +109,9 @@
 inline constexpr OptDesc kOptsMore[] = {
     {"tile_mask", "BM25_TILE_MASK", &SearchOpts::tile_mask, kOptBool, 0, 1, 0, nullptr},
     {"seg_skip", "BM25_SEG_SKIP", &SearchOpts::seg_skip, kOptBool, 0, 1, 0, nullptr},
+    {"row_skip", "BM25_ROW_SKIP", &SearchOpts::row_skip, kOptBool, 0, 1, 0, nullptr},
+    {"row_mask_kb", "BM25_ROW_MASK_KB", &SearchOpts::row_mask_kb, kOptRange, 0, 1 << 30, 2,
+     nullptr},
 };
 
 int set_opt(SearchOpts& o, const char* name, int64_t v);
diff --git a/mojo-bm25_amd/csrc/bm25mi_internal.h b/mojo-bm25_amd/csrc/bm25mi_internal.h
--- a/mojo-bm25_amd/csrc/bm25mi_internal.h
+++ b/mojo-bm25_amd/csrc/bm25mi_internal.h
@@ -57,6 +57,8 @@
   int bool_chunk = 0;
   int tile_mask = 1;
   int seg_skip = 1;
+  int row_skip = 1;
+  int row_mask_kb = 262144;
 };
 
 enum {
@@ -73,6 +75,7 @@
   kKAfter = 16384,
   kKTileSkip = 32768,
   kKSegSkip = 65536,
+  kKRowSkip = 131072,
 };
 struct Dispatch {
   uint32_t kernels = 0;
@@ -103,6 +106,9 @@
   double* val64 = nullptr;
   uint16_t* bmax = nullptr;
   uint32_t* tmask = nullptr;
+  int32_t* hslot = nullptr;
+  uint32_t* rowmask = nullptr;
+  int64_t n_heavy = 0;
   uint16_t* bpool = nullptr;
   int64_t pstride = 0;
   bool bound_weak = false;
@@ -117,7 +123,8 @@
   mutable Dispatch disp;
 };
 
-constexpr int kCounters = 12;
+constexpr int kCounters = 16;
+constexpr int kRowEntries = 16;
 
 struct LargeArena {
   char* base = nullptr;
@@ -182,7 +189,7 @@
   uint32_t* sub = nullptr;
   int32_t* sub_ipb = nullptr;
   int32_t* sub_done = nullptr;
-  uint8_t* tskip = nullptr;
+  uint16_t* tskip = nullptr;
   uint64_t* seg = nullptr;
   int64_t cap_seg = 0;
 };
@@ -212,6 +219,8 @@
                                int32_t* d_err, hipStream_t stream);
 hipError_t launch_build_bmax(const DevIndex& ix, hipStream_t stream);
 hipError_t launch_build_tmask(const DevIndex& ix, hipStream_t stream);
+hipError_t launch_heavy_terms(const DevIndex& ix, int32_t* d_heavy, hipStream_t stream);
+hipError_t launch_build_rowmask(const DevIndex& ix, const int32_t* d_hterm, hipStream_t stream);
 hipError_t launch_pool_bounds(const uint16_t* in, int64_t rows, int64_t in_stride, uint16_t* out,
                               int64_t out_stride, hipStream_t stream);
 hipError_t launch_count_tiles(const DevIndex& ix, const int32_t* d_indices, int64_t* d_cnt,
diff --git a/mojo-bm25_amd/csrc/bm25mi_kernels.hip b/mojo-bm25_amd/csrc/bm25mi_kernels.hip
--- a/mojo-bm25_amd/csrc/bm25mi_kernels.hip
+++ b/mojo-bm25_amd/csrc/bm25mi_kernels.hip
@@ -28,7 +28,7 @@
   const uint32_t* tl_start;
   const uint64_t* seg;
   int64_t seg_zero;
-  const uint8_t* tskip;
+  const uint16_t* tskip;
   int64_t tskip_stride;
 };
 
@@ -862,7 +862,18 @@
 };
 
 constexpr uint32_t kNoTile = 0xFFFFFFFFu;
-template <int TL>
+__device__ __forceinline__ uint32_t kth_set_bit16(uint32_t m, uint32_t k) {
+  uint32_t pos = 0u;
+  uint32_t c = (uint32_t)__popc(m & 0xFFu);
+  if (k >= c) { k -= c; pos = 8u; m >>= 8; }
+  c = (uint32_t)__popc(m & 0xFu);
+  if (k >= c) { k -= c; pos += 4u; m >>= 4; }
+  c = (uint32_t)__popc(m & 3u);
+  if (k >= c) { k -= c; pos += 2u; m >>= 2; }
+  if (k >= (m & 1u)) pos += 1u;
+  return pos;
+}
+template <int TL, bool RW = false>
 __device__ __forceinline__ FlatTab flat_chunk(uint32_t sb, uint32_t sl, uint32_t incl,
                                               uint32_t excl, uint32_t total, uint32_t j0,
                                               uint32_t prev, uint32_t par) {
@@ -876,10 +887,14 @@
   }
   const uint32_t e = (uint32_t)__shfl((int)excl, pos, 64);
   const uint32_t b = (uint32_t)__shfl((int)sb, pos, 64);
-  const uint32_t l = (uint32_t)__shfl((int)sl, pos, 64);
+  const uint32_t lw = (uint32_t)__shfl((int)sl, pos, 64);
+  const uint32_t l = RW ? (lw & 0xFFFFu) : lw;
   const bool in = j < total;
   FlatTab t;
-  const uint32_t k = j - e;
+  uint32_t k = j - e;
+  if constexpr (RW) {
+    if ((lw >> 16) != 0xFFFFu) k = kth_set_bit16(lw >> 16, k);
+  }
   t.base = (in && l != 0u) ? ((b & ~1u) + 128u * k) * 2u : 0u;
   const uint32_t rlo = k == 0u ? (b & 1u) : 0u;
   const uint32_t rhi = min(128u, (b & 1u) + l - 128u * k);
@@ -899,7 +914,7 @@
   return T <= 8 ? 3 : (T <= 16 ? 4 : (T <= 32 ? 5 : 6));
 }
 
-template <int S, int PH, int SM, bool SP, int TL>
+template <int S, int PH, int SM, bool SP, int TL, bool RW = false>
 __global__ __launch_bounds__(64) __attribute__((amdgpu_waves_per_eu(BM25_FLAT_WPE, BM25_FLAT_WPE))) void score_flat_kernel(
     IndexArgs a, const int32_t* __restrict__ queries, int32_t T, int32_t P, int32_t G,
     int32_t nq_host, const int32_t* __restrict__ nq_dev, const int32_t* __restrict__ qmap,
@@ -1010,7 +1025,8 @@
   auto terms_of = [&](const FlatCur& c) -> int32_t {
     return queries[(int64_t)c.qb * T + (int)min(lt, (uint32_t)(T - 1))];
   };
-  constexpr bool kBits = PH == kRest && TL == 3 && SM != kLargeM;
+  static_assert(!RW || (PH == kRest && TL == 3 && SM != kLargeM), "row words: 8-lane REST only");
+  constexpr bool kBits = RW;
   const bool skipping = PH == kRest && skeys != nullptr && G == kSampleGroup &&
                         !(kBits && a.tskip != nullptr);
   const uint32_t lgG = (uint32_t)__builtin_ctz((unsigned)G), lgP = (uint32_t)__builtin_ctz((unsigned)P);
@@ -1038,7 +1054,7 @@
     if (kBits && a.tskip != nullptr) {
       const uint32_t t32 = (uint32_t)c.b + li;
       if ((int)li < c.bw)
-        d.aux = ((uint32_t)a.tskip[(int64_t)c.q * a.tskip_stride + t32] >> lt) & 1u;
+        d.aux = a.tskip[((int64_t)c.q * a.tskip_stride + t32) * 8 + lt];
     } else if (skipping) {
       const uint32_t t32 = (uint32_t)tile;
       const int64_t si = (int64_t)(((t32 >> (lgG + lgP)) << lgG) | (t32 & (uint32_t)(G - 1)));
@@ -1055,6 +1071,7 @@
   constexpr bool kCountPost = PH == kRest && SM == 2;
   uint32_t npost = 0;
   uint32_t ndrop = 0, ndpost = 0;
+  uint32_t nrdrop = 0, nrpost = 0;
   uint32_t iSb = 0, iSl = 0, iIncl = 0, iExcl = 0;
   uint32_t iTotal = 0, iR = 0, iJ0 = 0, iPrev = kNoTile, iCur = 0;
   int32_t ctxV = 0, iPar = 0;
@@ -1072,9 +1089,9 @@
     bool skip = smp && th_pos && dN.aux < (uint32_t)(thN >> 32);
     if constexpr (PH == kRest) {
       if (kBits && a.tskip != nullptr) {
-        const bool drop = dN.aux != 0u;
+        const bool drop = dN.aux == 0u;
         if constexpr (kCountPost) {
-          const bool cut = seg_sum_u32<TL>(dN.aux) == TT;
+          const bool cut = seg_sum_u32<TL>(drop ? 1u : 0u) == TT;
           const uint32_t sl = dN.r1 - dN.r0;
           const uint32_t tp = seg_sum_u32<TL>(sl);
           const bool cnt = cut && !skip && lt == 0u && (int)li < nx.bw;
@@ -1083,6 +1100,19 @@
           const bool dcnt = drop && !cut && !skip && sl != 0u;
           ndrop += (uint32_t)__popcll(__ballot(dcnt));
           ndpost += wave_sum_u32(dcnt ? sl : 0u);
+          const uint32_t b1 = (dN.ip + dN.r0) & 1u;
+          const uint32_t nf = sl == 0u ? 0u : (b1 + sl + 127u) >> 7;
+          const bool rcnt = !drop && !skip && dN.aux != 0xFFFFu;
+          uint32_t rr = 0u, rp = 0u;
+#pragma unroll
+          for (uint32_t r = 0; r < 16u; ++r) {
+            if (rcnt && r < nf && ((dN.aux >> r) & 1u) == 0u) {
+              ++rr;
+              rp += min(128u, b1 + sl - 128u * r) - (r == 0u ? b1 : 0u);
+            }
+          }
+          nrdrop += wave_sum_u32(rr);
+          nrpost += wave_sum_u32(rp);
         }
         skip = skip || drop;
       }
@@ -1090,6 +1120,11 @@
     iSb = dN.ip + dN.r0;
     iSl = skip ? 0u : dN.r1 - dN.r0;
     uint32_t nr = iSl == 0u ? 0u : ((iSb & 1u) + iSl + 127u) >> 7;
+    if constexpr (kBits) {
+      const uint32_t rw = a.tskip != nullptr ? dN.aux : 0xFFFFu;
+      if (rw != 0xFFFFu) nr = (uint32_t)__popc(rw & ~(0xFFFFFFFFu << min(nr, 16u)));
+      iSl |= rw << 16;
+    }
     if ((PH == kAll || (PH == kRest && !th_pos)) && lt == 0u && (int)li < nx.bw)
       nr = max(nr, 1u);
     if constexpr (PH == kSample) {
@@ -1159,12 +1194,12 @@
       il = 0;
       return;
     }
-    tI = flat_chunk<TL>(iSb, iSl, iIncl, iExcl, iTotal, iJ0, iPrev, iCur);
+    tI = flat_chunk<TL, kBits>(iSb, iSl, iIncl, iExcl, iTotal, iJ0, iPrev, iCur);
     nI = min(64u, iR - iJ0);
     il = 0;
   };
   enter_item();
-  tI = flat_chunk<TL>(iSb, iSl, iIncl, iExcl, iTotal, 0u, iPrev, iCur);
+  tI = flat_chunk<TL, kBits>(iSb, iSl, iIncl, iExcl, iTotal, 0u, iPrev, iCur);
   nI = min(64u, iR);
   il = 0;
 
@@ -1342,6 +1377,11 @@
     const uint32_t ndp = ndpost;
     if (lane == 0 && ndp != 0u)
       atomicAdd(reinterpret_cast<unsigned long long*>(stats + 5), (unsigned long long)ndp);
+    const uint32_t nrd = nrdrop;
+    if (lane == 0 && nrd != 0u) atomicAdd(stats + 4, (int32_t)nrd);
+    const uint32_t nrp = nrpost;
+    if (lane == 0 && nrp != 0u)
+      atomicAdd(reinterpret_cast<unsigned long long*>(stats + 7), (unsigned long long)nrp);
   }
   finish();
 }
@@ -1543,6 +1583,56 @@
   }
 }
 
+__global__ __launch_bounds__(256) void heavy_terms_kernel(const int64_t* __restrict__ indptr,
+                                                          const uint32_t* __restrict__ rel,
+                                                          int64_t V, int64_t ntiles,
+                                                          int32_t* __restrict__ heavy) {
+  for (int64_t t = blockIdx.x; t < V; t += gridDim.x) {
+    const int64_t ip = indptr[t];
+    const uint32_t* r = rel + t * (ntiles + 1);
+    int any = 0;
+    for (int64_t j = threadIdx.x; j < ntiles; j += blockDim.x) {
+      const uint32_t l = r[j + 1] - r[j];
+      any |= (((uint32_t)(ip + r[j]) & 1u) + l + 127u) >> 7 >= 2u;
+    }
+    any = __syncthreads_or(any);
+    if (threadIdx.x == 0) heavy[t] = any;
+  }
+}
+
+__global__ __launch_bounds__(256) void build_rowmask_kernel(const int64_t* __restrict__ indptr,
+                                                            const uint32_t* __restrict__ rel,
+                                                            const uint16_t* __restrict__ ldoc,
+                                                            const int32_t* __restrict__ hterm,
+                                                            int64_t H, int64_t ntiles, int S,
+                                                            uint32_t* __restrict__ rowmask) {
+  for (int64_t h = blockIdx.x; h < H; h += gridDim.x) {
+    const int64_t t = hterm[h];
+    const int64_t ip = indptr[t];
+    const uint32_t* r = rel + t * (ntiles + 1);
+    for (int64_t j = threadIdx.x; j < ntiles; j += blockDim.x) {
+      uint32_t* out = rowmask + (h * ntiles + j) * kRowEntries;
+      const int64_t b = ip + r[j], e = ip + r[j + 1];
+      const int64_t b0 = b & ~(int64_t)1;
+      const bool wide = e > b && ((e - 1 - b0) >> 7) >= kRowEntries;
+      for (int i = 0; i < kRowEntries; ++i) out[i] = wide ? 0xFFFFFFFFu : 0u;
+      if (wide) continue;
+      int64_t cur = 0;
+      uint32_t m = 0u;
+      for (int64_t p = b; p < e; ++p) {
+        const int64_t row = (p - b0) >> 7;
+        if (row != cur) {
+          out[cur] = m;
+          m = 0u;
+          cur = row;
+        }
+        m |= 1u << ((uint32_t)ldoc[p] >> (S - 3));
+      }
+      if (e > b) out[cur] = m;
+    }
+  }
+}
+
 constexpr int kSkipNT = 256;
 constexpr int kSkipTerms = 8;
 inline int skip_npt(int64_t ntiles) {
@@ -1552,12 +1642,13 @@
 constexpr uint32_t kSkipBias = 0x80000000u - 1048472u;
 template <int N> struct alignas(2 * N) SkipB { uint16_t v[N]; };
 template <int N> struct alignas(4 * N) SkipM { uint32_t v[N]; };
-template <int N> struct alignas(N) SkipO { uint8_t v[N]; };
+struct alignas(16) SkipW { uint16_t v[kSkipTerms]; };
 template <int N>
 __global__ __launch_bounds__(kSkipNT) void tile_skip_kernel(
     const uint16_t* __restrict__ bmax, const uint32_t* __restrict__ tmask, int64_t V,
     int64_t ntiles, const int32_t* __restrict__ queries, int32_t T, int64_t Q,
-    const uint64_t* __restrict__ theta, uint8_t* __restrict__ tskip, int32_t seg) {
+    const uint64_t* __restrict__ theta, uint16_t* __restrict__ tskip, int32_t seg,
+    const int32_t* __restrict__ hslot, const uint32_t* __restrict__ rowmask) {
   const int64_t bs = bmax_stride(ntiles);
   const int64_t nch = (bs + kSkipNT * N - 1) / (kSkipNT * N);
   for (int64_t it = blockIdx.x; it < Q * nch; it += gridDim.x) {
@@ -1565,13 +1656,19 @@
     const int64_t t0 = ((it - q * nch) * kSkipNT + threadIdx.x) * N;
     if (t0 >= bs) continue;
     const uint32_t thk = (uint32_t)(theta[q] >> 32);
-    SkipO<N> out;
-#pragma unroll
-    for (int i = 0; i < N; ++i) out.v[i] = 0;
-    if (thk > score_key(0.f) && t0 < ntiles) {
+    SkipW* dst = reinterpret_cast<SkipW*>(tskip) + q * bs + t0;
+    SkipW all;
+#pragma unroll
+    for (int t = 0; t < kSkipTerms; ++t) all.v[t] = 0xFFFFu;
+    if (!(thk > score_key(0.f) && t0 < ntiles)) {
+#pragma unroll
+      for (int i = 0; i < N; ++i) dst[i] = all;
+    } else {
       SkipB<N> bb[kSkipTerms];
       SkipM<N> mm[kSkipTerms];
       uint32_t okm = 0u;
+      uint32_t hm = 0u;
+      int32_t hs[kSkipTerms];
 #pragma unroll
       for (int t = 0; t < kSkipTerms; ++t) {
 #pragma unroll
@@ -1579,20 +1676,30 @@
           bb[t].v[i] = 0;
           mm[t].v[i] = 0u;
         }
+        hs[t] = -1;
         if (t < T) {
           const int32_t term = queries[q * T + t];
           if (term >= 0 && term < V) {
             okm |= 1u << t;
             bb[t] = *reinterpret_cast<const SkipB<N>*>(bmax + term * bs + t0);
             if (tmask != nullptr) mm[t] = *reinterpret_cast<const SkipM<N>*>(tmask + term * bs + t0);
+            if (seg && rowmask != nullptr) {
+              hs[t] = __builtin_amdgcn_readfirstlane(hslot[term]);
+              if (hs[t] >= 0) hm |= 1u << t;
+            }
           }
         }
       }
+      hm = (uint32_t)__builtin_amdgcn_readfirstlane((int)hm);
       const float th = key_score(thk);
       const float K = 1048576.f / th;
 #pragma unroll
       for (int i = 0; i < N; ++i) {
-        if (t0 + i >= ntiles) break;
+        if (t0 + i >= ntiles) {
+          dst[i] = all;
+          continue;
+        }
+        SkipW out;
         float ub[kSkipTerms];
         uint32_t mk[kSkipTerms];
 #pragma unroll
@@ -1602,12 +1709,12 @@
         }
         const float sum = ((ub[0] + ub[1]) + (ub[2] + ub[3])) + ((ub[4] + ub[5]) + (ub[6] + ub[7]));
         uint32_t byte = sum * 1.0001f < th ? 0xFFu : 0u;
+        uint32_t L = 0u;
         if (byte == 0u && tmask != nullptr) {
           uint32_t c[kSkipTerms];
 #pragma unroll
           for (int t = 0; t < kSkipTerms; ++t)
             c[t] = mk[t] != 0u ? (uint32_t)ceilf(fminf(ub[t] * K, 2097152.f)) + 1u : 0u;
-          uint32_t L = 0u;
 #pragma unroll
           for (int s = 31; s >= 0; --s) {
             uint32_t acc = kSkipBias;
@@ -1622,10 +1729,30 @@
             for (int t = 0; t < kSkipTerms; ++t) byte |= (mk[t] & L) == 0u ? 1u << t : 0u;
           }
         }
-        out.v[i] = (uint8_t)byte;
-      }
-    }
-    *reinterpret_cast<SkipO<N>*>(tskip + q * bs + t0) = out;
+#pragma unroll
+        for (int t = 0; t < kSkipTerms; ++t) out.v[t] = ((byte >> t) & 1u) ? 0u : 0xFFFFu;
+        if (hm != 0u && L != 0u) {
+#pragma unroll
+          for (int t = 0; t < kSkipTerms; ++t) {
+            if (((hm >> t) & 1u) == 0u) continue;
+            if ((byte >> t) & 1u) continue;
+            const uint4* rm = reinterpret_cast<const uint4*>(
+                rowmask + ((int64_t)hs[t] * ntiles + (t0 + i)) * kRowEntries);
+            uint32_t w = 0u;
+#pragma unroll
+            for (int g = 0; g < kRowEntries / 4; ++g) {
+              const uint4 m4 = rm[g];
+              w |= ((m4.x & L) != 0u ? 1u : 0u) << (4 * g);
+              w |= ((m4.y & L) != 0u ? 2u : 0u) << (4 * g);
+              w |= ((m4.z & L) != 0u ? 4u : 0u) << (4 * g);
+              w |= ((m4.w & L) != 0u ? 8u : 0u) << (4 * g);
+            }
+            out.v[t] = (uint16_t)w;
+          }
+        }
+        dst[i] = out;
+      }
+    }
   }
 }
 
@@ -3097,6 +3224,22 @@
   return hipGetLastError();
 }
 
+hipError_t launch_heavy_terms(const DevIndex& ix, int32_t* d_heavy, hipStream_t stream) {
+  if (ix.n_terms == 0 || ix.ntiles == 0 || ix.sparse) return hipSuccess;
+  const int64_t blocks = std::min<int64_t>(ix.n_terms, 65536);
+  hipLaunchKernelGGL(heavy_terms_kernel, dim3((unsigned)blocks), dim3(256), 0, stream, ix.indptr,
+                     ix.rel, ix.n_terms, ix.ntiles, d_heavy);
+  return hipGetLastError();
+}
+
+hipError_t launch_build_rowmask(const DevIndex& ix, const int32_t* d_hterm, hipStream_t stream) {
+  if (ix.n_heavy == 0 || ix.ntiles == 0 || !ix.rowmask || ix.sparse) return hipSuccess;
+  const int64_t blocks = std::min<int64_t>(ix.n_heavy, 65536);
+  hipLaunchKernelGGL(build_rowmask_kernel, dim3((unsigned)blocks), dim3(256), 0, stream, ix.indptr,
+                     ix.rel, ix.ldoc, d_hterm, ix.n_heavy, ix.ntiles, ix.tile_shift, ix.rowmask);
+  return hipGetLastError();
+}
+
 hipError_t launch_count_tiles(const DevIndex& ix, const int32_t* d_indices, int64_t* d_cnt,
                               int32_t* d_err, hipStream_t stream) {
   if (ix.n_terms == 0) return hipSuccess;
@@ -3197,20 +3340,24 @@
   constexpr bool kSlots = PH == kRest && SM == kLargeM;
   const bool skip = PH == kRest && sg.sample_keys != nullptr && sg.M == 1 && sg.G == kSampleGroup;
   IndexArgs a = args_of(ix);
+  bool rw = false;
   if (PH == kRest && !skip && !kSlots && TL == 3 && ix.opt.tile_bound && ix.bmax != nullptr &&
       ws.tskip != nullptr) {
     a.tskip = ws.tskip;
     a.tskip_stride = tskip_stride(ix.ntiles);
+    rw = true;
     const uint32_t* tmask = ix.opt.tile_mask ? ix.tmask : (const uint32_t*)nullptr;
     const bool seg = ix.opt.seg_skip && tmask != nullptr;
-    ix.disp.kernels |= kKTileSkip | (seg ? kKSegSkip : 0);
+    const bool row = seg && ix.opt.row_skip && ix.rowmask != nullptr && ix.hslot != nullptr;
+    ix.disp.kernels |= kKTileSkip | (seg ? kKSegSkip : 0) | (row ? kKRowSkip : 0);
     auto pre = [&](auto kern, int npt) {
       const int64_t per = (int64_t)kSkipNT * npt;
       const int64_t items = sg.nq_host * ((a.tskip_stride + per - 1) / per);
       const int grid = (int)std::min<int64_t>(items, persistent_grid(kern, kSkipNT));
       hipLaunchKernelGGL(kern, dim3((unsigned)grid), dim3(kSkipNT), 0, st, ix.bmax, tmask,
                          ix.n_terms, ix.ntiles, q, (int32_t)T, (int64_t)sg.nq_host, ws.theta,
-                         ws.tskip, (int32_t)seg);
+                         ws.tskip, (int32_t)seg, ix.hslot,
+                         row ? ix.rowmask : (const uint32_t*)nullptr);
     };
     switch (skip_npt(ix.ntiles)) {
       case 4: pre(tile_skip_kernel<4>, 4); break;
@@ -3241,6 +3388,9 @@
                        PH == kRest ? ws.counters + 5 : nullptr, kSlots ? ws.slot_cnt : nullptr,
                        SM == kSplitM ? ws.sub : nullptr, SM == kSplitM ? ws.sub_ipb : nullptr);
   };
+  if constexpr (PH == kRest && TL == 3 && SM != kLargeM) {
+    if (rw) return go(score_flat_kernel<S, PH, SM, false, TL, true>);
+  }
   if (ix.sparse)
     go(score_flat_kernel<S, PH, SM, true, TL>);
   else
```

New measurement: 540,800 queries/s, median of 6. 1.1x the previous value.
